# zhenxuan00/graphical-gan

Hardware: AMD Instinct MI355X
Metric: images/sec (G+D+GP step) cifar10 32x32 bs=64 (higher is better)
Workload: dtype f32; 1 GPU; gan_inference_cifar10.py MODE=wali-gp BATCH_SIZE=64 (per GPU) 32x32x3, CRITIC_ITERS=5; parallelism=dp1, global_batch=64, hip_graph=True, minibatch_feed=device-resident ring, read in place; one graph per iteration, finite_costs=True

## Files before the change

### graphical_gan_amd/_lib.py

```python
import ctypes as C
import os

_HERE = os.path.dirname(os.path.abspath(__file__))
LIB_PATH = os.path.join(_HERE, 'libggan.so')

ACT_NONE, ACT_LRELU, ACT_RELU, ACT_TANH, ACT_SIGMOID = 0, 1, 2, 3, 4
PACK_MAX = 64
HEAD_BCE_MAX_ROWS = 2048
BCE_HEADS = 2
PACK_ARRIVE_INTS = 33 * 1024
POSTERIOR_MAX_K = 8192
MODE_K = {'CONCRETE': 0, 'STRAIGHT_THROUGHT_CONCRETE': 1, 'STRAIGHT_THROUGHT': 2}
BCE_MAX = 16
TSNE_MAX_K = 128
TSNE_MAX_SPLITS = 64
ABI_VERSION = 800


class ConvGeom(C.Structure):
    _fields_ = [(n, C.c_int) for n in ('N', 'Ci', 'H', 'W', 'Co', 'Ho', 'Wo', 'k', 'stride', 'pad_t', 'pad_l',
                                       'plan_wgs', 'plan_wgs_filter', 'plan_flags')]


PLAN_PLAIN = 1


class ProfRec(C.Structure):
    _fields_ = [('name', C.c_char * 48), ('total_ms', C.c_double), ('launches', C.c_long),
                ('flops', C.c_double), ('bytes', C.c_double), ('grid', C.c_long)]


class GganError(RuntimeError):
    pass


_P = C.c_void_p
_F = C.c_float
_I = C.c_int
_Z = C.c_size_t
_G = C.POINTER(ConvGeom)

SIGNATURES = {
    'ggan_version': (_I, []),
    'ggan_last_error': (C.c_char_p, []),
    'ggan_conv2d_workspace': (_Z, [_G]),
    'ggan_conv2d_fwd': (_I, [_G, _P, _P, _P, _P, _I, _F, _P, _Z, _P]),
    'ggan_conv2d_bwd_data': (_I, [_G, _P, _P, _P, _P, _I, _F, _P, _Z, _P]),
    'ggan_conv2d_bwd_filter': (_I, [_G, _P, _P, _P, _P, _P, _Z, _P]),
    'ggan_conv2d_bwd_data_act': (_I, [_G, _P, _P, _I, _F, _P, _P, _P, _Z, _P]),
    'ggan_conv2d_bwd_filter_act': (_I, [_G, _P, _P, _P, _I, _F, _P, _P, _P, _Z, _P]),
    'ggan_conv2d_bwd_filter_parts': (_I, [_G, _P, _P, _P, _I, _F, _I, _P, _Z, C.POINTER(_I), C.POINTER(_Z), _P]),
    'ggan_conv2d_fwd_cast_ring': (_I, [_G, _P, _I, _P, _P, _I, _P, _F, _F, _P, _P, _P, _P, _I, _F, _P]),
    'ggan_conv2d_fwd_masked': (_I, [_G, _P, _P, _P, _P, _I, _F, _P, _Z, _P]),
    'ggan_linear_bn_rows_fwd': (_I, [_P, _P, _P, _P, _P, _P, _P, _P, _P, _I, _I, _I, _F, _I, _F, _P]),
    'ggan_linear_bn_rows_bwd': (_I, [_P, _P, _P, _P, _P, _P, _P, _P, _P, _P, _P, _I, _I, _I, _I, _F, _P]),
    'ggan_deconv2d_fwd': (_I, [_G, _P, _P, _P, _P, _I, _F, _P, _Z, _P]),
    'ggan_deconv2d_bwd_data': (_I, [_G, _P, _P, _P, _P, _Z, _P]),
    'ggan_deconv2d_bwd_filter': (_I, [_G, _P, _P, _P, _P, _P, _Z, _P]),
    'ggan_gemm_workspace': (_Z, [_I, _I, _I]),
    'ggan_gemm': (_I, [_I, _I, _I, _I, _I, _P, _P, _P, _P, _I, _F, _P, _Z, _P]),
    'ggan_conv3d_out_shape': (_I, [_P, _P]),
    'ggan_im2col3d': (_I, [_P, _P, _P, _P]),
    'ggan_col2im3d': (_I, [_P, _P, _P, _P]),
    'ggan_conv3d_igemm_ok': (_I, [_P, _I]),
    'ggan_conv3d_fwd': (_I, [_P, _P, _P, _P, _P, _I, _F, _P, _Z, _P]),
    'ggan_conv3d_wgrad': (_I, [_P, _P, _P, _P, _P, _Z, _P]),
    'ggan_conv3d_dgrad': (_I, [_P, _P, _P, _P, _P]),
    'ggan_mix_rbf_mmd2_fwd': (_I, [_P, _P, _I, _I, _I, _P, _P, _I, _P, _P, _P]),
    'ggan_mix_rbf_mmd2_bwd': (_I, [_P, _P, _I, _I, _I, _P, _P, _I, _P, _P, _P, _P]),
    'ggan_mix_rbf_mmd2_unbiased_fwd': (_I, [_P, _P, _I, _I, _I, _P, _P, _I, _P, _P, _P]),
    'ggan_mix_rbf_mmd2_unbiased_bwd': (_I, [_P, _P, _I, _I, _I, _P, _P, _I, _P, _P, _P, _P]),
    'ggan_mix_rbf_sums_workspace': (_Z, [_I, _I]),
    'ggan_mix_rbf_sums': (_I, [_P, _P, _I, _I, _I, _P, _P, _I, _P, _P, _Z, _P]),
    'ggan_knn_radii_workspace': (_Z, [_I, _I]),
    'ggan_knn_radii': (_I, [_P, _I, _I, _I, _P, _P, _Z, _P]),
    'ggan_ball_counts_workspace': (_Z, [_I, _I]),
    'ggan_ball_counts': (_I, [_P, _P, _I, _I, _I, _P, _P, _P, _P, _Z, _P]),
    'ggan_noise_fill': (_I, [_P, _P, _P, _P, _P, _P, _I, _P, _P]),
    'ggan_gmm_latent_fwd': (_I, [_P, _P, _P, _P, _P, _I, _I, _I, _F, _F, _P]),
    'ggan_gmm_latent_bwd': (_I, [_P, _P, _P, _P, _P, _P, _P, _I, _I, _I, _F, _P]),
    'ggan_gmm_latent_st_fwd': (_I, [_P, _P, _P, _P, _P, _P, _I, _I, _I, _F, _F, _I, _P]),
    'ggan_gmm_latent_st_bwd': (_I, [_P, _P, _P, _P, _P, _P, _P, _I, _I, _I, _F, _I, _P]),
    'ggan_gmm_posterior_assign': (_I, [_P, _P, _F, _I, _I, _I, _I, _P, _P, _P, _P]),
    'ggan_cluster_accuracy': (_I, [_P, _P, _P, _I, _I, _P, _P]),
    'ggan_video_sheet_u8': (_I, [_P, _P, _P, _P, _I, _I, _I, _I, _I, _I, _I, _I, _I, _F, _F, _F, _P]),
    'ggan_tsne_sqnorms': (_I, [_P, _I, _I, _P, _P]),
    'ggan_tsne_neighbours': (_I, [_P, _P, _I, _I, _I, _I, _I, _P, _P, _P, _P, _Z, _P]),
    'ggan_tsne_affinities': (_I, [_P, _I, _I, _F, _I, _F, _P, _P, _P]),
    'ggan_tsne_symmetrise': (_I, [_P, _P, _I, _I, _P, _P, _P, _P, _P]),
    'ggan_tsne_gradient': (_I, [_P, _P, _P, _P, _I, _I, _P, _P, _P, _P, _P, _P]),
    'ggan_tsne_kl': (_I, [_P, _P, _P, _P, _I, _I, _P, _P, _P, _P, _P]),
    'ggan_tsne_iterate': (_I, [_P, _P, _P, _P, _P, _P, _P, _I, _I, _P, _P, _I, _I, _I, _F, _F, _F, _F, _F, _P]),
    'ggan_gemm_split': (_I, [_I, _I, _I, _I, _I, _P, _P, _I, _P, _P, _P, _P, _I, _P, _I, _F, _P, _Z, _P]),
    'ggan_gemm_colsum': (_I, [_I, _I, _I, _I, _P, _P, _P, _P, _P, _Z, _P]),
    'ggan_dyn_scan_fwd': (_I, [_I, _I, _I, _I, _I, _P, _P, _P, _P, _P, _P, _P, _P, _P, _P, _F, _P, _P, _P, _P]),
    'ggan_dyn_scan_bwd': (_I, [_I, _I, _I, _I, _I, _P, _P, _P, _P, _P, _P, _P, _P, _P, _F, _P, _P, _P, _P, _P, _P, _P]),
    'ggan_critic_head_fwd': (_I, [_I, _I, _I, _I, _P, _P, _P, _P, _P, _P, _F, _P, _P, _P, _Z, _P]),
    'ggan_critic_head_bwd': (_I, [_I, _I, _I, _I, _P, _P, _P, _P, _P, _P, _F, _P, _P, _P, _P, _P, _P, _P, _P, _Z, _P]),
    'ggan_critic_head_fwd_bce': (_I, [_I, _I, _I, _I, _P, _P, _P, _P, _P, _P, _F, _P, _P, _I, _I, _P, _P, _P, _P, _P, _P, _Z, _P]),
    'ggan_critic_head_bwd_tail': (_I, [_I, _I, _I, _I, _P, _P, _P, _P, _P, _F, _P, _P, _P, _P, _P, _P, _P, _P, _P, _I, _I, _P, _P, _P, _P, _P, _P, _Z, _P]),
    'ggan_linear_bwd_data_act': (_I, [_I, _I, _I, _P, _P, _I, _F, _P, _P, _P, _Z, _P]),
    'ggan_linear_bwd_weight_act': (_I, [_I, _I, _I, _P, _P, _P, _I, _F, _P, _P, _P, _Z, _P]),
    'ggan_colsum': (_I, [_P, _P, _I, _I, _P]),
    'ggan_reparam_fwd': (_I, [_P, _P, _P, _P, _P, _Z, _P]),
    'ggan_reparam_bwd': (_I, [_P, _P, _P, _P, _P, _P, _Z, _P]),
    'ggan_agg_div_fwd': (_I, [_I, _P, _P, _P, _P, _P, _I, _I, _I, _I, _P, _P, _P, _P, _P, _P]),
    'ggan_agg_div_bwd': (_I, [_I, _P, _P, _P, _P, _I, _I, _I, _I, _P, _P, _P, _P, _P, _P, _P, _P, _P]),
    'ggan_colsum_tall': (_I, [_P, _P, _I, _I, _P, _Z, _P]),
    'ggan_chansum': (_I, [_P, _P, _I, _I, _I, _P, _Z, _P]),
    'ggan_bn_fwd_train': (_I, [_P, _P, _P, _P, _P, _P, _I, _I, _I, _F, _I, _F, _P]),
    'ggan_bn_bwd': (_I, [_P, _P, _P, _P, _P, _P, _P, _P, _I, _I, _I, _P]),
    'ggan_bn_bwd_act': (_I, [_P, _P, _P, _I, _F, _P, _P, _P, _P, _P, _P, _P, _I, _I, _I, _P]),
    'ggan_bn_bwd_bwd': (_I, [_P, _P, _P, _I, _F, _P, _P, _P, _P, _P, _P, _P, _I, _I, _I, _P]),
    'ggan_bn_split_fwd_train': (_I, [_P, _P, _P, _P, _P, _P, _I, _I, _I, _I, _F, _I, _F, _P, _Z, _P]),
    'ggan_bn_split_bwd_act': (_I, [_P, _P, _I, _F, _P, _P, _P, _P, _P, _P, _P, _P, _I, _I, _I, _I, _I, _P, _Z, _P]),
    'ggan_bn_sync_stats': (_I, [_P, _P, _I, _I, _I, _P]),
    'ggan_bn_sync_apply': (_I, [_P, _P, _I, _P, _P, _P, _P, _P, _I, _I, _I, _F, _I, _F, _P]),
    'ggan_bn_sync_bwd_stats': (_I, [_P, _P, _P, _I, _F, _P, _P, _P, _I, _I, _I, _P]),
    'ggan_bn_sync_bwd_apply': (_I, [_P, _P, _P, _I, _F, _P, _P, _P, _P, _I, _I, _P, _P, _P, _I, _I, _I, _P]),
    'ggan_act_fwd': (_I, [_P, _P, _Z, _I, _F, _P]),
    'ggan_act_bwd': (_I, [_P, _P, _P, _Z, _I, _F, _P]),
    'ggan_act_bwd_chansum': (_I, [_P, _P, _P, _P, _I, C.POINTER(_I), _I, _I, _I, _I, _F, _P]),
    'ggan_bias_add': (_I, [_P, _P, _P, _I, _I, _I, _P]),
    'ggan_cast_scale_i32': (_I, [_P, _P, _P, _Z, _F, _F, _P]),
    'ggan_cast_scale_ring_i32': (_I, [_P, _I, _P, _P, _I, _P, _P, _Z, _F, _F, _P]),
    'ggan_axpby': (_I, [_P, _P, _P, _Z, _F, _F, _F, _P]),
    'ggan_mix_mean': (_I, [_P, _P, _P, _P, _I, _I, _I, _P]),
    'ggan_row_lerp': (_I, [_P, _P, _P, _P, _I, _I, _P]),
    'ggan_bce_logits_fwd': (_I, [_P, _F, _F, _P, _I, _I, _P]),
    'ggan_bce_logits_bwd': (_I, [_P, _F, _F, _P, _P, _I, _P]),
    'ggan_bce_logits_multi_fwd': (_I, [C.POINTER(_P), C.POINTER(_F), C.POINTER(_F), C.POINTER(_I), _I, _P, _P]),
    'ggan_bce_logits_multi_bwd': (_I, [C.POINTER(_P), C.POINTER(_F), C.POINTER(_F), C.POINTER(_I), _I, _P, C.POINTER(_P), _P]),
    'ggan_bce_logits_multi_fwd_grad': (_I, [C.POINTER(_P), C.POINTER(_F), C.POINTER(_F), C.POINTER(_I), _I, _P, C.POINTER(_P), _P]),
    'ggan_bce_head_bwd': (_I, [C.POINTER(_P), C.POINTER(_F), C.POINTER(_F), C.POINTER(_I), _I, _P, C.POINTER(_P), _I, _I, _P, _P, _F, _P, _P,
                          _P, _P]),
    'ggan_bce_heads_bwd': (_I, [C.POINTER(_P), C.POINTER(_F), C.POINTER(_F), C.POINTER(_I), _I, _P, C.POINTER(_P), _I, C.POINTER(_I),
                           C.POINTER(_I), C.POINTER(_I), C.POINTER(_P), C.POINTER(_P), C.POINTER(_F), C.POINTER(_P), C.POINTER(_P),
                           C.POINTER(_P), _P]),
    'ggan_mean_fwd': (_I, [_P, _F, _P, _I, _I, _P]),
    'ggan_mean_bwd': (_I, [_P, _F, _P, _I, _P]),
    'ggan_mean_multi_fwd_grad': (_I, [C.POINTER(_P), C.POINTER(_F), C.POINTER(_I), _I, _P, C.POINTER(_P), _P]),
    'ggan_dist_fwd': (_I, [_P, _P, _P, _Z, _I, _F, _I, _P]),
    'ggan_dist_bwd': (_I, [_P, _P, _P, _P, _P, _Z, _I, _F, _P]),
    'ggan_gp_penalty_fwd': (_I, [_P, _P, _P, _I, _I, _F, _P]),
    'ggan_gp_penalty_bwd': (_I, [_P, _P, _P, _P, _I, _I, _F, _P]),
    'ggan_gp_penalty_fwd_grad': (_I, [_P, _P, _P, _P, _P, _I, _I, _F, _P]),
    'ggan_adam_step': (_I, [_P, _P, _P, _P, _Z, _P, _F, _F, _F, _F, _F, _P]),
    'ggan_adam_advance': (_I, [_P, _P]),
    'ggan_rmsprop_step': (_I, [_P, _P, _P, _Z, _F, _F, _F, _F, _F, _F, _P]),
    'ggan_adam_step_counted': (_I, [_P, _P, _P, _P, _Z, _P, _F, _F, _F, _F, _F, _P]),
    'ggan_pack': (_I, [C.POINTER(_P), C.POINTER(_Z), C.POINTER(_Z), _I, _P, _P]),
    'ggan_pack_parts': (_I, [C.POINTER(_P), C.POINTER(_Z), C.POINTER(_Z), C.POINTER(_I), C.POINTER(_Z), _I, _P, _P, _P]),
    'ggan_pack_parts2': (_I, [C.POINTER(_P), C.POINTER(_Z), C.POINTER(_Z), C.POINTER(_I), C.POINTER(_Z), C.POINTER(_P), C.POINTER(_I),
                              C.POINTER(_Z), _I, _P, _P, _P]),
    'ggan_pack_adam': (_I, [C.POINTER(_P), C.POINTER(_Z), C.POINTER(_Z), C.POINTER(_I), C.POINTER(_Z), C.POINTER(_P), C.POINTER(_I),
                            C.POINTER(_Z), _I, _P, _P, _P, _P, _P, _P, _F, _F, _F, _F, _F, _P]),
    'ggan_prof_enable': (_I, [_I]),
    'ggan_prof_reset': (_I, []),
    'ggan_prof_report': (_I, [C.POINTER(ProfRec), _I]),
}

_lib = None


def load():
    global _lib
    if _lib is not None:
        return _lib
    if not os.path.exists(LIB_PATH):
        raise GganError('libggan.so not found at %s -- run `python -c "import __graft_entry__ as g; g.build()"` '
                        '(there is no CPU fallback)' % LIB_PATH)
    lib = C.CDLL(LIB_PATH)
    for name, (res, args) in SIGNATURES.items():
        try:
            fn = getattr(lib, name)
        except AttributeError:
            raise GganError('libggan.so does not export %s' % name)
        fn.restype = res
        fn.argtypes = args
    if lib.ggan_version() != ABI_VERSION:
        raise GganError('libggan.so speaks ABI version %d, this binding %d: a stale build -- run `python -c "import __graft_entry__ as g; g.build()"`'
                        % (lib.ggan_version(), ABI_VERSION))
    _lib = lib
    return lib


def check(rc, what):
    if rc != 0:
        msg = load().ggan_last_error()
        raise GganError('%s failed (%d): %s' % (what, rc, msg.decode() if msg else ''))


def prof_report(cap=256):
    lib = load()
    recs = (ProfRec * cap)()
    n = lib.ggan_prof_report(recs, cap)
    out = []
    for i in range(n):
        r = recs[i]
        out.append(dict(name=r.name.decode(), total_ms=r.total_ms, launches=int(r.launches),
                        flops=r.flops, bytes=r.bytes, grid=int(r.grid)))
    return out
# ... 1 lines not shown
```

### graphical_gan_amd/csrc/conv.h

```cpp
#pragma once
#include "common.h"

namespace ggan {

int conv_fwd_naive(const ggan_conv_geom& g, const float* x, const float* w, const float* bias, float* y, int act,
                   float alpha, hipStream_t s);
struct GyMask {
    const float* ref;
    int act;
    float alpha;
};
int conv_dgrad_naive(const ggan_conv_geom& g, const float* gy, GyMask m, const float* w, const float* bias, float* gx,
                     int act, float alpha, hipStream_t s);
int conv_wgrad_naive(const ggan_conv_geom& g, const float* x, const float* gy, GyMask m, float* gw, hipStream_t s);

constexpr int kTargetWgs = 200;
struct OutMask {
    const float* ref;
    int act;
    float alpha;
    bool applied;
};
int conv_fwd_mfma(const ggan_conv_geom& g, const float* x, const float* w, const float* bias, float* y, int act,
                  float alpha, void* ws, size_t ws_bytes, hipStream_t s, OutMask* mask = nullptr);
int conv_dgrad_mfma(const ggan_conv_geom& g, const float* gy, GyMask m, const float* w, const float* bias, float* gx,
                    int act, float alpha, void* ws, size_t ws_bytes, hipStream_t s);
int conv_dgrad_dg16(const ggan_conv_geom& g, const float* gy, GyMask m, const float* w, const float* bias, float* gx, int act,
                    float alpha, int target_wgs, void* ws, size_t ws_bytes, hipStream_t s);
int conv_dgrad_thin(const ggan_conv_geom& g, const float* gy, GyMask m, const float* w, const float* bias, float* gx, int act,
                    float alpha, hipStream_t s);
struct WgradParts {
    float* buf;
    size_t cap_floats;
    int with_bias;
    int n;
    size_t stride;
};
int conv_wgrad_mfma(const ggan_conv_geom& g, const float* x, const float* gy, GyMask m, float* gw, float* gbias, void* ws,
                    size_t ws_bytes, hipStream_t s, WgradParts* parts = nullptr);
struct ThinCastSrc {
    const int32_t* ring;
    const int32_t* ctr_a;
    const int32_t* ctr_b;
    const float* noise;
    float* x_out;
    int nslots, offset;
    float div, mul;
};
int conv_fwd_thin(const ggan_conv_geom& g, const float* x, const float* w, const float* bias, float* y, int act, float alpha,
                  hipStream_t s, const ThinCastSrc* cast = nullptr, const OutMask* mask = nullptr);
int conv_wgrad_thin(const ggan_conv_geom& g, const float* x, const float* gy, GyMask m, float* gw, float* gbias, void* ws,
                    size_t ws_bytes, hipStream_t s, WgradParts* parts = nullptr);
size_t conv_workspace_bytes(const ggan_conv_geom& g);
int launch_splitk_reduce(const float* partial, int SK, size_t elems, float* out, const float* bias, int C, int HW, int act,
                         float alpha, hipStream_t s, size_t slab_stride = 0, float* tail_out = nullptr, size_t tail = 0);

struct FastDiv {
    uint32_t mul, d;
};
inline FastDiv make_fastdiv(uint32_t d) {
    FastDiv f;
    f.d = d;
    f.mul = (d <= 1) ? 0u : (uint32_t)((0x100000000ull / d) + 1ull);
    return f;
}
__device__ __forceinline__ uint32_t fdiv(uint32_t n, FastDiv f) { return f.d <= 1 ? n : __umulhi(n, f.mul); }

struct FastDiv24 {
    uint32_t mul, shift;
};
inline bool make_fastdiv24(uint32_t d, uint32_t nmax, FastDiv24* out) {
    if (d <= 1) { out->mul = 1; out->shift = 0; return true; }
    for (int s = 31; s >= 1; --s) {
        const uint64_t m = ((1ull << s) + d - 1) / d;
        if (m >= (1ull << 24) || m * nmax >= (1ull << 32)) continue;
        const uint64_t err = m * d - (1ull << s);
        if ((uint64_t)nmax * err >= (1ull << s)) return false;
        out->mul = (uint32_t)m; out->shift = (uint32_t)s;
        return true;
    }
    return false;
}
__device__ __forceinline__ uint32_t fdiv24(uint32_t n, FastDiv24 f) { return __umul24(n, f.mul) >> f.shift; }

}
```

### graphical_gan_amd/csrc/conv_api.hip

```cpp
#include "common.h"
#include "conv.h"
#include <stdlib.h>
using namespace ggan;

namespace {

int check_geom(const ggan_conv_geom* g) {
    if (!g) { set_error("null geometry"); return -1; }
    if (g->N <= 0 || g->Ci <= 0 || g->Co <= 0 || g->H <= 0 || g->W <= 0 || g->Ho <= 0 || g->Wo <= 0 || g->k <= 0 ||
        g->stride <= 0 || g->pad_t < 0 || g->pad_l < 0) {
        set_error("bad conv geometry N=%d Ci=%d H=%d W=%d Co=%d Ho=%d Wo=%d k=%d s=%d pad=(%d,%d)", g->N, g->Ci, g->H,
                  g->W, g->Co, g->Ho, g->Wo, g->k, g->stride, g->pad_t, g->pad_l);
        return -1;
    }
    if ((g->plan_flags & ~GGAN_PLAN_PLAIN) || g->plan_wgs < 0 || g->plan_wgs > 65536 || g->plan_wgs_filter < 0 || g->plan_wgs_filter > 65536) {
        set_error("conv geometry: launch plan fields out of range (plan_wgs=%d plan_wgs_filter=%d plan_flags=%d): struct built against "
                  "an older ggan.h? (GGAN_ABI_VERSION %d)", g->plan_wgs, g->plan_wgs_filter, g->plan_flags, GGAN_ABI_VERSION);
        return -1;
    }
    if ((g->Ho - 1) * g->stride - g->pad_t >= g->H || (g->Wo - 1) * g->stride - g->pad_l >= g->W) {
        set_error("conv geometry: output grid larger than the input allows");
        return -1;
    }
    return 0;
}

}

extern "C" {

size_t ggan_conv2d_workspace(const ggan_conv_geom* g) { return g ? conv_workspace_bytes(*g) : 0; }

int ggan_conv2d_fwd(const ggan_conv_geom* g, const float* x, const float* w, const float* bias, float* y, int act,
                    float alpha, void* ws, size_t ws_bytes, ggan_stream_t stream) {
    if (check_geom(g)) return -1;
    GGAN_CHECK_ARG(x && w && y, "null pointer");
    hipStream_t s = (hipStream_t)stream;
    if (!(g->plan_flags & GGAN_PLAN_PLAIN) && !getenv("GGAN_NAIVE_FWD")) {
        int r = conv_fwd_thin(*g, x, w, bias, y, act, alpha, s);
        if (r <= 0) return r;
        r = conv_fwd_mfma(*g, x, w, bias, y, act, alpha, ws, ws ? ws_bytes : 0, s);
        if (r <= 0) return r;
    }
    return conv_fwd_naive(*g, x, w, bias, y, act, alpha, s);
}

int ggan_conv2d_fwd_cast_ring(const ggan_conv_geom* g, const int32_t* ring, int nslots, const int32_t* ctr_a, const int32_t* ctr_b, int offset,
                              const float* noise, float div, float mul, float* x_out, const float* w, const float* bias, float* y, int act,
                              float alpha, ggan_stream_t stream) {
    if (check_geom(g)) return -1;
    GGAN_CHECK_ARG(ring && x_out && w && y && nslots > 0, "bad argument");
    if ((g->plan_flags & GGAN_PLAN_PLAIN) || getenv("GGAN_NAIVE_FWD")) return 1;
    ThinCastSrc c;
    c.ring = ring; c.ctr_a = ctr_a; c.ctr_b = ctr_b; c.noise = noise; c.x_out = x_out; c.nslots = nslots; c.offset = offset; c.div = div; c.mul = mul;
    return conv_fwd_thin(*g, nullptr, w, bias, y, act, alpha, (hipStream_t)stream, &c);
}

static int bwd_data(const ggan_conv_geom* g, const float* gy, GyMask m, const float* w, const float* bias, float* gx, int act,
                    float alpha, void* ws, size_t ws_bytes, ggan_stream_t stream) {
    if (check_geom(g)) return -1;
    if (!(gy && w && gx)) { set_error("ggan_conv2d_bwd_data: null pointer"); return -1; }
    hipStream_t s = (hipStream_t)stream;
    if (getenv("GGAN_TRACE_CONV"))
        fprintf(stderr, "[ggan] bwd_data N=%d Ci=%d H=%d W=%d Co=%d Ho=%d Wo=%d pad=(%d,%d) mask=%d act=%d\n", g->N, g->Ci, g->H, g->W, g->Co, g->Ho,
                g->Wo, g->pad_t, g->pad_l, m.act, act);
    if (!(g->plan_flags & GGAN_PLAN_PLAIN) && !getenv("GGAN_NAIVE_DGRAD")) {
        int r = conv_dgrad_thin(*g, gy, m, w, bias, gx, act, alpha, s);
        if (r <= 0) return r;
        r = conv_dgrad_dg16(*g, gy, m, w, bias, gx, act, alpha, g->plan_wgs, ws, ws ? ws_bytes : 0, s);
        if (r <= 0) return r;
        r = conv_dgrad_mfma(*g, gy, m, w, bias, gx, act, alpha, ws, ws ? ws_bytes : 0, s);
        if (r <= 0) return r;
    }
    return conv_dgrad_naive(*g, gy, m, w, bias, gx, act, alpha, s);
}

__global__ void pad_width_k(const float* __restrict__ in, const float* __restrict__ ref, float* __restrict__ out, size_t rows,
                            int W, int Wp, int shift, int act, float alpha) {
    const size_t total = rows * (size_t)Wp;
    for (size_t i = (size_t)blockIdx.x * blockDim.x + threadIdx.x; i < total; i += (size_t)gridDim.x * blockDim.x) {
        const size_t r = i / Wp;
        const int w = (int)(i - r * Wp) - shift;
        float v = 0.f;
        if (w >= 0 && w < W) {
            v = in[r * W + w];
            if (ref) v = act_grad(v, ref[r * W + w], act, alpha);
        }
        out[i] = v;
    }
}

static int wgrad_widened(const ggan_conv_geom& g, const float* x, const float* gy, GyMask m, float* gw, float* gbias, void* ws,
                         size_t ws_bytes, hipStream_t s) {
    if (g.k != 5 || g.stride != 2 || (g.pad_l != 1 && g.pad_l != 2)) return 1;
    const int shift = g.pad_l - 1;
    int Wop = (g.Wo + 3) & ~3;
    while (2 * Wop < g.W + shift) Wop += 4;
    const int Wp = 2 * Wop;
    if (Wop > 64) return 1;
    ws = ws_scratch(ws, ws_bytes);
    const size_t xr = (size_t)g.N * g.Ci * g.H, gr = (size_t)g.N * g.Co * g.Ho;
    const size_t xb = (xr * Wp * sizeof(float) + 255) & ~(size_t)255, gb = (gr * Wop * sizeof(float) + 255) & ~(size_t)255;
    if (!ws || ws_bytes < xb + gb + (1u << 20)) return 1;
    float* xp = (float*)ws;
    float* gp = (float*)((char*)ws + xb);
    auto blocks = [](size_t n) { size_t b = (n + 255) / 256; return (int)(b > 4096 ? 4096 : (b < 1 ? 1 : b)); };
    GGAN_LAUNCH("pad_width_k", 0, 8.0 * xr * Wp, pad_width_k, dim3(blocks(xr * Wp)), dim3(256), 0, s, x, (const float*)nullptr, xp, xr,
                g.W, Wp, shift, 0, 0.f);
    GGAN_LAUNCH("pad_width_k", 0, 8.0 * gr * Wop, pad_width_k, dim3(blocks(gr * Wop)), dim3(256), 0, s, gy,
                m.act != GGAN_ACT_NONE ? m.ref : (const float*)nullptr, gp, gr, g.Wo, Wop, 0, m.act, m.alpha);
    ggan_conv_geom gp2 = g;
    gp2.W = Wp; gp2.Wo = Wop; gp2.pad_l = 1;
    void* rest = (char*)ws + xb + gb;
    const size_t rest_bytes = ws_bytes - xb - gb;
    const GyMask none{nullptr, GGAN_ACT_NONE, 0.f};
    int r = conv_wgrad_mfma(gp2, xp, gp, none, gw, gbias, rest, rest_bytes, s);
    if (r == 1 && gbias) {
        r = conv_wgrad_mfma(gp2, xp, gp, none, gw, nullptr, rest, rest_bytes, s);
        if (r == 0) r = ggan_chansum(gp, gbias, g.N, g.Co, g.Ho * Wop, rest, rest_bytes, (ggan_stream_t)s);
    }
    return r;
}

static int bwd_filter(const ggan_conv_geom* g, const float* x, const float* gy, GyMask m, float* gw, float* gbias, void* ws,
                      size_t ws_bytes, ggan_stream_t stream) {
    if (check_geom(g)) return -1;
    if (!(x && gy && gw)) { set_error("ggan_conv2d_bwd_filter: null pointer"); return -1; }
    hipStream_t s = (hipStream_t)stream;
    if (!(g->plan_flags & GGAN_PLAN_PLAIN) && !getenv("GGAN_NAIVE_WGRAD")) {
        int r = conv_wgrad_thin(*g, x, gy, m, gw, gbias, ws, ws ? ws_bytes : 0, s);
        if (r <= 0) return r;
        r = conv_wgrad_mfma(*g, x, gy, m, gw, gbias, ws, ws ? ws_bytes : 0, s);
        if (r <= 0) return r;
        r = wgrad_widened(*g, x, gy, m, gw, gbias, ws, ws ? ws_bytes : 0, s);
        if (r <= 0) return r;
    }
    if (gbias) {
        if (m.act != GGAN_ACT_NONE) return 1;
        int r = ggan_chansum(gy, gbias, g->N, g->Co, g->Ho * g->Wo, ws, ws_bytes, stream);
        if (r) return r;
    }
    if (getenv("GGAN_TRACE_NAIVE"))
        fprintf(stderr, "[ggan] plain filter-gradient kernel for N=%d Ci=%d H=%d W=%d Co=%d Ho=%d Wo=%d k=%d s=%d pad=(%d,%d)\n", g->N, g->Ci,
                g->H, g->W, g->Co, g->Ho, g->Wo, g->k, g->stride, g->pad_t, g->pad_l);
    return conv_wgrad_naive(*g, x, gy, m, gw, s);
}

int ggan_conv2d_bwd_data(const ggan_conv_geom* g, const float* gy, const float* w, const float* bias, float* gx, int act,
                         float alpha, void* ws, size_t ws_bytes, ggan_stream_t stream) {
    return bwd_data(g, gy, GyMask{nullptr, GGAN_ACT_NONE, 0.f}, w, bias, gx, act, alpha, ws, ws_bytes, stream);
}

int ggan_conv2d_bwd_filter(const ggan_conv_geom* g, const float* x, const float* gy, float* gw, float* gbias, void* ws,
                           size_t ws_bytes, ggan_stream_t stream) {
    return bwd_filter(g, x, gy, GyMask{nullptr, GGAN_ACT_NONE, 0.f}, gw, gbias, ws, ws_bytes, stream);
}

int ggan_conv2d_bwd_data_act(const ggan_conv_geom* g, const float* gy, const float* y, int y_act, float y_alpha, const float* w,
                             float* gx, void* ws, size_t ws_bytes, ggan_stream_t stream) {
    GGAN_CHECK_ARG(y || y_act == GGAN_ACT_NONE, "null activation reference");
    return bwd_data(g, gy, GyMask{y, y_act, y_alpha}, w, nullptr, gx, GGAN_ACT_NONE, 0.f, ws, ws_bytes, stream);
}

int ggan_conv2d_bwd_filter_act(const ggan_conv_geom* g, const float* x, const float* gy, const float* y, int y_act, float y_alpha,
                               float* gw, float* gbias, void* ws, size_t ws_bytes, ggan_stream_t stream) {
    GGAN_CHECK_ARG(y || y_act == GGAN_ACT_NONE, "null activation reference");
    return bwd_filter(g, x, gy, GyMask{y, y_act, y_alpha}, gw, gbias, ws, ws_bytes, stream);
}

int ggan_conv2d_bwd_filter_parts(const ggan_conv_geom* g, const float* x, const float* gy, const float* y, int y_act,
                                 float y_alpha, int with_bias, float* part, size_t part_cap, int* n_parts, size_t* stride,
                                 ggan_stream_t stream) {
    if (check_geom(g)) return -1;
    GGAN_CHECK_ARG(x && gy && part && n_parts && stride, "null pointer");
    GGAN_CHECK_ARG(y || y_act == GGAN_ACT_NONE, "null activation reference");
    if ((g->plan_flags & GGAN_PLAN_PLAIN) || getenv("GGAN_NAIVE_WGRAD")) return 1;
    WgradParts po{part, part_cap, with_bias, 0, 0};
    int r = conv_wgrad_thin(*g, x, gy, GyMask{y, y_act, y_alpha}, nullptr, nullptr, nullptr, 0, (hipStream_t)stream, &po);
    if (r == 1) r = conv_wgrad_mfma(*g, x, gy, GyMask{y, y_act, y_alpha}, nullptr, nullptr, nullptr, 0, (hipStream_t)stream, &po);
    if (r == 0) { *n_parts = po.n; *stride = po.stride; }
    return r;
}

int ggan_conv2d_fwd_masked(const ggan_conv_geom* g, const float* x, const float* w, float* y, const float* yref, int ref_act,
                           float ref_alpha, void* ws, size_t ws_bytes, ggan_stream_t stream) {
    if (check_geom(g)) return -1;
    GGAN_CHECK_ARG(x && w && y && yref, "null pointer");
    if ((g->plan_flags & GGAN_PLAN_PLAIN) || getenv("GGAN_NAIVE_FWD")) return 1;
    if ((((uintptr_t)yref) & 15) != 0) return 1;
    OutMask M{yref, ref_act, ref_alpha, false};
    if (g->Ci <= 4 && (ref_act == GGAN_ACT_LRELU || ref_act == GGAN_ACT_RELU)) {
        const int r = conv_fwd_thin(*g, x, w, nullptr, y, GGAN_ACT_NONE, 0.f, (hipStream_t)stream, nullptr, &M);
        if (r <= 0) return r;
    }
    const int rc = conv_fwd_mfma(*g, x, w, nullptr, y, GGAN_ACT_NONE, 0.f, ws, ws ? ws_bytes : 0, (hipStream_t)stream, &M);
    if (rc == 0 && !M.applied) { set_error("conv2d_fwd_masked: launch without the mask"); return -3; }
    return rc;
}

int ggan_deconv2d_fwd(const ggan_conv_geom* g, const float* x_small, const float* w, const float* bias, float* y_big,
                      int act, float alpha, void* ws, size_t ws_bytes, ggan_stream_t stream) {
    return ggan_conv2d_bwd_data(g, x_small, w, bias, y_big, act, alpha, ws, ws_bytes, stream);
}

int ggan_deconv2d_bwd_data(const ggan_conv_geom* g, const float* gy_big, const float* w, float* gx_small, void* ws,
                           size_t ws_bytes, ggan_stream_t stream) {
    return ggan_conv2d_fwd(g, gy_big, w, nullptr, gx_small, GGAN_ACT_NONE, 0.f, ws, ws_bytes, stream);
}

int ggan_deconv2d_bwd_filter(const ggan_conv_geom* g, const float* gy_big, const float* x_small, float* gw, float* gbias,
                             void* ws, size_t ws_bytes, ggan_stream_t stream) {
    if (check_geom(g)) return -1;
    if (gbias) {
        GGAN_CHECK_ARG(gy_big, "null pointer");
        int r = ggan_chansum(gy_big, gbias, g->N, g->Ci, g->H * g->W, ws, ws_bytes, stream);
        if (r) return r;
    }
    return ggan_conv2d_bwd_filter(g, gy_big, x_small, gw, nullptr, ws, ws_bytes, stream);
}

}
```

### graphical_gan_amd/csrc/conv_corr.hip

```cpp
#include "common.h"
#include "conv.h"
#include <stdlib.h>
#include <map>
#include <mutex>
#include <vector>
using namespace ggan;

namespace {

constexpr int XE_MAX = 24;
constexpr unsigned OOB = 0x7FFFFFF0u;
typedef unsigned int u32x4 __attribute__((ext_vector_type(4)));

__host__ __device__ inline int fwd_region(int data_floats, int lanes_used, int floats_per_lane) {
    const int tail = (((lanes_used + 63) & ~63) - lanes_used) * floats_per_lane;
    return (data_floats + (tail > 4 ? tail : 4) + 3) & ~3;
}

struct CorrClass {
    int Hu, Wv;
    int roff, coff;
    int or0, oc0;
    int wbase;
    int pad_;
// ... 491 lines not shown
        stamp(3);
        constexpr int NSTEP = (NT0 * PW + 1) / 2, NITEM = XE + WE;
        constexpr int IPS = (NITEM + NSTEP - 3) / (NSTEP - 2);
        for (int ck0 = ck_begin; ck0 < ck_end; ck0 += CK, buf = buf == 2 ? 0 : buf + 1) {
            const int ck2 = ck0 + 2 * CK;
            const bool more2 = ck2 < ck_end;
            const int b2 = buf == 0 ? 2 : buf - 1;
            auto hook = [&](int g) {
#pragma unroll
                for (int it = g * IPS; it < (g + 1) * IPS; ++it) {
                    if (more2 && it < XE) dma_x1(it, ck2, b2);
                    if (more2 && it >= XE && it < NITEM) dma_w1(it - XE, ck2, b2);
                }
            };
            const float* xs = smem + buf * STAGE;
            const float* ws = xs + XS_SZ;
            mma_taps<CL::th(0), CL::tw(0), DI, PW, CK, RS, 0>(xs, ws, xfrag[0], wfrag, P.CS, P.SCp, acc[0], hook);
            if (more2) wait_vm_n(ndma);
            else asm volatile("s_waitcnt vmcnt(0)" ::: "memory");
            __syncthreads();
            if (it_ < 8) stamp(4 + it_);
            ++it_;
        }
    } else if (dma) {
        asm volatile("s_waitcnt vmcnt(0)" ::: "memory");
        __syncthreads();
        stamp(3);
        constexpr int NSTEP = (NT0 * PW + 1) / 2, NITEM = XE + WE;
        constexpr int IPS = (NITEM + NSTEP - 3) / (NSTEP - 2);
        for (int ck0 = ck_begin; ck0 < ck_end; ck0 += CK, buf ^= 1) {
            const int ckn = ck0 + CK;
            const bool more = ckn < ck_end;
            auto hook = [&](int g) {
#pragma unroll
                for (int it = g * IPS; it < (g + 1) * IPS; ++it) {
                    if (more && it < XE) dma_x1(it, ckn, buf ^ 1);
                    if (more && it >= XE && it < NITEM) dma_w1(it - XE, ckn, buf ^ 1);
                }
            };
            const float* xs = smem + buf * STAGE;
            const float* ws = xs + XS_SZ;
            mma_taps<CL::th(0), CL::tw(0), DI, PW, CK, RS, 0>(xs, ws, xfrag[0], wfrag, P.CS, P.SCp, acc[0], hook);
            asm volatile("s_waitcnt vmcnt(0)" ::: "memory");
            __syncthreads();
            if (it_ < 8) stamp(4 + it_);
            ++it_;
        }
    } else if (wdma) {
        constexpr int TS = GH * NCB * WBLK;
        constexpr int WD_STEPS = (NT0 * (PW == 2 ? 2 : 1) + 1) / 2 + (NT1 * (PW == 2 ? 2 : 1) + 1) / 2 +
                                 (NT2 * (PW == 2 ? 2 : 1) + 1) / 2 + (NT3 * (PW == 2 ? 2 : 1) + 1) / 2;
        constexpr int WD_DPS = (WQ + WD_STEPS - 2) / (WD_STEPS - 1);
        constexpr int WD_S0 = (WQ + WD_DPS - 1) / WD_DPS < WD_STEPS - 1 ? (WQ + WD_DPS - 1) / WD_DPS : WD_STEPS - 1;
        constexpr int WD_SPS = (XN + WD_STEPS - WD_S0 - 1) / (WD_STEPS - WD_S0);
        prefetch(ck_begin, false);
        stage_w(ck_begin, 0);
        commit(0, false);
        if (ck_begin + CK < ck_end) prefetch(ck_begin + CK, false);
        asm volatile("s_waitcnt vmcnt(0)" ::: "memory");
        __syncthreads();
        stamp(3);
        for (int ck0 = ck_begin; ck0 < ck_end; ck0 += CK, buf ^= 1) {
            const int ckn = ck0 + CK;
            commit(buf ^ 1, false);
            const float* xs = smem + buf * STAGE;
            const float* ws = xs + XS_SZ;
            const int ck2 = ck0 + 2 * CK;
            const bool more2 = ck2 < ck_end;
            auto hook = [&](int g) {
#pragma unroll
                for (int q = g * WD_DPS; q < (g + 1) * WD_DPS; ++q)
                    if (q < WQ && (q < WQ - 1 || wso[WQ - 1] >= 0)) stage_w1(q, ckn, buf ^ 1);
#pragma unroll
                for (int j = (g - WD_S0) * WD_SPS; j < (g - WD_S0 + 1) * WD_SPS; ++j)
                    if (j >= 0 && j < XN) {
                        if constexpr (XR4) {
                            xreg4[j] = __builtin_amdgcn_raw_buffer_load_b128(rin, more2 ? xvo[j] : OOB, ck2 * HWin * 4, 0);
                            if (masked) xref4[j] = __builtin_amdgcn_raw_buffer_load_b128(rref, more2 ? xvo[j] : OOB, ck2 * HWin * 4, 0);
                        } else {
                            xreg[j] = __builtin_amdgcn_raw_buffer_load_b32(rin, more2 ? xvo[j] : OOB, ck2 * HWin * 4, 0);
                            if (masked) xref[j] = __builtin_amdgcn_raw_buffer_load_b32(rref, more2 ? xvo[j] : OOB, ck2 * HWin * 4, 0);
                        }
                    }
            };
            if constexpr (WD) {
                constexpr int S1 = (CL::th(0) * CL::tw(0) * (PW == 2 ? 2 : 1) + 1) / 2;
                constexpr int S2 = NC > 1 ? (CL::th(1) * CL::tw(1) * (PW == 2 ? 2 : 1) + 1) / 2 : 0;
                constexpr int S3 = NC > 2 ? (CL::th(2) * CL::tw(2) * (PW == 2 ? 2 : 1) + 1) / 2 : 0;
                mma_taps_wd<CL::th(0), CL::tw(0), DI, PW, TS, 0>(xs, ws, xfrag[0], wfrag_wd, P.CS, P.SCp, acc[0], hook);
                if constexpr (NC > 1) mma_taps_wd<CL::th(1), CL::tw(1), DI, PW, TS, S1>(xs, ws + NT0 * TS, xfrag[1], wfrag_wd, P.CS, P.SCp, acc[1], hook);
                if constexpr (NC > 2) mma_taps_wd<CL::th(2), CL::tw(2), DI, PW, TS, S1 + S2>(xs, ws + (NT0 + NT1) * TS, xfrag[2], wfrag_wd, P.CS, P.SCp, acc[2], hook);
                if constexpr (NC > 3) mma_taps_wd<CL::th(3), CL::tw(3), DI, PW, TS, S1 + S2 + S3>(xs, ws + (NT0 + NT1 + NT2) * TS, xfrag[3], wfrag_wd, P.CS, P.SCp, acc[3], hook);
            }
            static_assert(2 * XN < 64, "vmcnt field");
            if (masked) asm volatile("s_waitcnt vmcnt(%0)" ::"n"(2 * XN) : "memory");
            else asm volatile("s_waitcnt vmcnt(%0)" ::"n"(XN) : "memory");
            __syncthreads();
            if (it_ < 8) stamp(4 + it_);
            ++it_;
        }
    } else {
    prefetch(ck_begin);
    commit(0);
    stamp(2);
    if (ck_begin + CK < ck_end) prefetch(ck_begin + CK);
    __syncthreads();
    stamp(3);
    const bool stage_first = NTHR == 256 || wave < (NTHR / 128);
    auto stage_next = [&](int ck0) {
        if (ck0 + CK < ck_end && !(P.dbg & 1)) {
            if (!(P.dbg & 16)) commit(buf ^ 1);
            if (ck0 + 2 * CK < ck_end && !(P.dbg & 32)) prefetch(ck0 + 2 * CK);
        }
    };
    for (int ck0 = ck_begin; ck0 < ck_end; ck0 += CK, buf ^= 1) {
        if (stage_first) stage_next(ck0);
        if (fine && it_ < 4) stamp(4 + 2 * it_);
        if (!(P.dbg & 2)) {
            const float* xs = smem + ((P.dbg & 1) ? 0 : buf * STAGE);
            const float* ws = xs + XS_SZ;
            mma_taps<CL::th(0), CL::tw(0), DI, PW, CK, RS>(xs, ws, xfrag[0], wfrag, P.CS, P.SCp, acc[0]);
            if constexpr (NC > 1) mma_taps<CL::th(1), CL::tw(1), DI, PW, CK, RS>(xs, ws + NT0 * CK * RS, xfrag[1], wfrag, P.CS, P.SCp, acc[1]);
            if constexpr (NC > 2) mma_taps<CL::th(2), CL::tw(2), DI, PW, CK, RS>(xs, ws + (NT0 + NT1) * CK * RS, xfrag[2], wfrag, P.CS, P.SCp, acc[2]);
            if constexpr (NC > 3) mma_taps<CL::th(3), CL::tw(3), DI, PW, CK, RS>(xs, ws + (NT0 + NT1 + NT2) * CK * RS, xfrag[3], wfrag, P.CS, P.SCp, acc[3]);
        }
        if (fine && it_ < 4 && stage_first) stamp(5 + 2 * it_);
        if (!stage_first) stage_next(ck0);
        if (fine && it_ < 4 && !stage_first) stamp(5 + 2 * it_);
        __syncthreads();
        if (!fine && it_ < 8) stamp(4 + it_);
        ++it_;
    }
    }
    stamp(12);

    constexpr int TMW = 32 * WM;
    float* red = smem;
#pragma unroll
    for (int c = 0; c < NC; ++c)
#pragma unroll
        for (int r = 0; r < 16; ++r) {
            const int cnl = wn * 32 + (r & 3) + 8 * (r >> 2) + 4 * half;
            red[((ks * NC + c) * TNW + cnl) * TMW + wm * 32 + l31] = acc[c][r];
        }
    __syncthreads();
    stamp(13);
    if (P.dbg & 8) return;
    const bool direct = P.SK == 1;
    float* outp = direct ? P.out : P.out + (size_t)split * P.out_elems;
    const int chw = P.Hout * P.Wout;
    constexpr int GROUPS = NC == 4 ? 2 : NC;
    constexpr int UNITS = GROUPS * TNW * (TMW / 4);
    const bool quad_rows = (P.TC & 3) == 0;
    for (int u = tid; u < UNITS; u += NTHR) {
        const int p4 = u % (TMW / 4);
        const int cnl = (u / (TMW / 4)) % TNW;
        static_assert(((TMW / 4) * TNW) % 64 == 0, "store groups are whole waves");
        const int gsel = __builtin_amdgcn_readfirstlane(u / ((TMW / 4) * TNW));
        const int cn = cn0 + cnl;
        if (cn >= P.CNtot) continue;
        const int ca = NC == 4 ? 2 * gsel : gsel, cb = NC == 4 ? 2 * gsel + 1 : gsel;
        float va[4] = {0.f, 0.f, 0.f, 0.f}, vb[4] = {0.f, 0.f, 0.f, 0.f};
        float4 ta[KS], tb[KS];
#pragma unroll
        for (int k = 0; k < KS; ++k) {
            ta[k] = *reinterpret_cast<const float4*>(red + ((k * NC + ca) * TNW + cnl) * TMW + 4 * p4);
            if (NC == 4) tb[k] = *reinterpret_cast<const float4*>(red + ((k * NC + cb) * TNW + cnl) * TMW + 4 * p4);
        }
#pragma unroll
        for (int k = 0; k < KS; ++k) {
            va[0] += ta[k].x; va[1] += ta[k].y; va[2] += ta[k].z; va[3] += ta[k].w;
            if (NC == 4) { vb[0] += tb[k].x; vb[1] += tb[k].y; vb[2] += tb[k].z; vb[3] += tb[k].w; }
        }
        if (direct) {
            const float bv = P.bias ? P.bias[cn] : 0.f;
#pragma unroll
            for (int j = 0; j < 4; ++j) {
                va[j] = act_apply(va[j] + bv, P.act, P.alpha);
                if (NC == 4) vb[j] = act_apply(vb[j] + bv, P.act, P.alpha);
            }
        }
        const CorrClass& A = P.cls[CL::cls(ca)];
        const CorrClass& B = P.cls[CL::cls(cb)];
        const int p = 4 * p4;
        const int img = fdiv24(p, P.d_TRTC);
        const int rem = p - img * (P.TR * P.TC);
        const int ur = fdiv24(rem, P.d_TC);
        const int vc = rem - ur * P.TC;
        const bool img_ok = img < P.TI && (n0 + img) < P.N;
        const size_t cbase = ((size_t)(n0 + img) * P.CNtot + cn) * chw;
        bool done = false;
        if (quad_rows && img_ok && (P.Wout & 3) == 0) {
            if (NC != 4 && P.ocs == 1 && (A.Wv & 3) == 0 && (u0 + ur) < A.Hu && (v0 + vc + 3) < A.Wv) {
                const int off = (A.or0 + P.ors * (u0 + ur)) * P.Wout + A.oc0 + v0 + vc;
                if ((off & 3) == 0) {
                    if (KIND == 0 && P.out_ref) {
                        const float4 r4 = *reinterpret_cast<const float4*>(P.out_ref + cbase + off);
                        va[0] = act_grad(va[0], r4.x, P.out_act, P.out_alpha); va[1] = act_grad(va[1], r4.y, P.out_act, P.out_alpha);
                        va[2] = act_grad(va[2], r4.z, P.out_act, P.out_alpha); va[3] = act_grad(va[3], r4.w, P.out_act, P.out_alpha);
                    }
                    *reinterpret_cast<float4*>(outp + cbase + off) = make_float4(va[0], va[1], va[2], va[3]);
                    done = true;
                }
            }
            if (NC == 4 && A.Wv == B.Wv && A.Hu == B.Hu && (A.Wv & 3) == 0 && (u0 + ur) < A.Hu && (v0 + vc + 3) < A.Wv) {
                const bool a_even = A.oc0 < B.oc0;
                const int off = (A.or0 + P.ors * (u0 + ur)) * P.Wout + (a_even ? A.oc0 : B.oc0) + P.ocs * (v0 + vc);
                if ((off & 3) == 0 && P.ocs == 2) {
                    const float* e = a_even ? va : vb;
                    const float* o = a_even ? vb : va;
                    *reinterpret_cast<float4*>(outp + cbase + off) = make_float4(e[0], o[0], e[1], o[1]);
                    *reinterpret_cast<float4*>(outp + cbase + off + 4) = make_float4(e[2], o[2], e[3], o[3]);
                    done = true;
                }
            }
        }
        if (!done) {
#pragma unroll
            for (int j = 0; j < 4; ++j) {
                const int pj = p + j;
                const int im = fdiv24(pj, P.d_TRTC);
                const int rm = pj - im * (P.TR * P.TC);
                const int urj = fdiv24(rm, P.d_TC);
                const int vcj = rm - urj * P.TC;
                if (!(im < P.TI && (n0 + im) < P.N)) continue;
                const size_t cb2 = ((size_t)(n0 + im) * P.CNtot + cn) * chw;
                if ((u0 + urj) < A.Hu && (v0 + vcj) < A.Wv) {
                    const size_t oi = cb2 + (A.or0 + P.ors * (u0 + urj)) * P.Wout + A.oc0 + P.ocs * (v0 + vcj);
                    outp[oi] = (KIND == 0 && P.out_ref) ? act_grad(va[j], P.out_ref[oi], P.out_act, P.out_alpha) : va[j];
                }
                if (NC == 4 && (u0 + urj) < B.Hu && (v0 + vcj) < B.Wv)
                    outp[cb2 + (B.or0 + P.ors * (u0 + urj)) * P.Wout + B.oc0 + P.ocs * (v0 + vcj)] = vb[j];
            }
        }
    }
    stamp(14);
}

template <int MODE, int WM, int WN, int KS, int PW, bool X4 = false>
__global__ __launch_bounds__(64 * WM * WN * KS) void corr_kernel(const CorrParams P) {
    extern __shared__ __attribute__((aligned(16))) float smem[];
    warm_kernarg(P);
    const int grp = blockIdx.z / P.SK, split = blockIdx.z - grp * P.SK;
    int bx = blockIdx.x, by = blockIdx.y;
    if (P.xcd_p > 0) {
        const int lin = blockIdx.y * gridDim.x + blockIdx.x, xcd = lin & 7, slot = lin >> 3;
        const int pg = xcd % P.xcd_p, cg = xcd / P.xcd_p;
        const int npx = gridDim.x / P.xcd_p, nch = gridDim.y / (8 / P.xcd_p);
        bx = pg * npx + slot % npx;
        by = cg * nch + slot / npx;
    }
    if constexpr (MODE == 0) {
        corr_body<0, 2, 1, WM, WN, KS, PW, X4>(P, split, smem, bx, by);
    } else if constexpr (MODE == 2) {
        corr_body<3, 1, -1, WM, WN, KS, PW, X4>(P, split, smem, bx, by);
    } else if (grp == 0) {
        corr_body<1, 1, -1, WM, WN, KS, PW, X4>(P, split, smem, bx, by);
    } else {
        corr_body<2, 1, -1, WM, WN, KS, PW, X4>(P, split, smem, bx, by);
    }
}

__global__ void splitk_reduce_k(const float* __restrict__ partial, int SK, size_t elems, size_t stride, float* __restrict__ out,
                                const float* __restrict__ bias, int C, int HW, int act, float alpha, float* __restrict__ out2,
                                size_t n2) {
    for (size_t i = (size_t)blockIdx.x * blockDim.x + threadIdx.x; i < elems + n2; i += (size_t)gridDim.x * blockDim.x) {
        float s = 0.f;
#pragma unroll 8
        for (int k = 0; k < SK; ++k) s += partial[(size_t)k * stride + i];
        if (i < elems) {
            if (bias) s += bias[(i / (size_t)HW) % (size_t)C];
            out[i] = act_apply(s, act, alpha);
        } else {
            out2[i - elems] = s;
        }
    }
}

__global__ void splitk_reduce_small_k(const float* __restrict__ partial, int SK, size_t elems, size_t stride, float* __restrict__ out,
                                      const float* __restrict__ bias, int C, int HW, int act, float alpha,
                                      float* __restrict__ out2, size_t n2) {
    __shared__ float sm[4][64];
    const int o = threadIdx.x & 63, kg = threadIdx.x >> 6;
    const size_t i = (size_t)blockIdx.x * 64 + o;
    float s = 0.f;
    if (i < elems + n2)
#pragma unroll 4
        for (int k = kg; k < SK; k += 4) s += partial[(size_t)k * stride + i];
    sm[kg][o] = s;
    __syncthreads();
    if (kg == 0 && i < elems + n2) {
        float v = (sm[0][o] + sm[1][o]) + (sm[2][o] + sm[3][o]);
        if (i < elems) {
            if (bias) v += bias[(i / (size_t)HW) % (size_t)C];
            out[i] = act_apply(v, act, alpha);
        } else {
            out2[i - elems] = v;
        }
    }
}

struct WaveCfg { int WM, WN, KS, PW; };
constexpr int kNumCfgs = 9;
constexpr WaveCfg kCfgsFwd[kNumCfgs] = {{2, 2, 1, 2}, {2, 1, 2, 2}, {1, 1, 4, 1}, {1, 1, 4, 2}, {2, 1, 4, 1}, {1, 1, 8, 1}, {2, 2, 2, 1}, {2, 1, 4, 2}, {4, 1, 2, 2}};
constexpr WaveCfg kCfgsDgrad[kNumCfgs] = {{2, 2, 1, 4}, {2, 1, 2, 4}, {1, 1, 4, 2}, {1, 1, 4, 4}, {2, 1, 4, 2}, {1, 1, 8, 1}, {2, 2, 2, 2}, {1, 1, 8, 2}, {1, 1, 8, 2}};
constexpr const WaveCfg* cfgs_of(int mode) { return mode == 1 ? kCfgsDgrad : kCfgsFwd; }

#define CORR_EACH(X)                                                                                                        \
    X(0, 2, 1, 2, 2, false) X(0, 2, 1, 4, 1, false) X(0, 1, 1, 8, 1, false) X(0, 2, 2, 2, 1, false) X(0, 4, 1, 2, 2, false) \
    X(0, 2, 1, 4, 1, true) X(0, 1, 1, 8, 1, true) X(0, 2, 2, 2, 1, true) X(0, 4, 1, 2, 2, true)                             \
    X(1, 2, 1, 2, 4, false) X(1, 2, 1, 4, 2, false) X(1, 1, 1, 8, 1, false) X(1, 2, 2, 2, 2, false)                         \
    X(1, 2, 1, 4, 2, true) X(1, 1, 1, 8, 1, true)                                                                           \
    X(2, 2, 1, 2, 2, false) X(2, 1, 1, 8, 1, false) X(2, 2, 2, 2, 1, false) X(2, 2, 1, 4, 2, false)                         \
    X(2, 1, 1, 8, 1, true) X(2, 2, 2, 2, 1, true) X(2, 2, 1, 4, 2, true)
struct CorrInst { int mode; WaveCfg wc; bool x4; const char* name; void (*kernel)(const CorrParams); };
#define CORR_INST(MODE, WM, WN, KS, PW, X4) \
    {MODE, {WM, WN, KS, PW}, X4, "corr_kernel<" #MODE ", " #WM ", " #WN ", " #KS ", " #PW ", " #X4 ">", corr_kernel<MODE, WM, WN, KS, PW, X4>},
constexpr CorrInst kCorrInsts[] = {CORR_EACH(CORR_INST)};
#undef CORR_INST
#undef CORR_EACH

constexpr const CorrInst* find_inst(int mode, const WaveCfg& wc, bool x4) {
    for (const CorrInst& k : kCorrInsts)
        if (k.mode == mode && k.wc.WM == wc.WM && k.wc.WN == wc.WN && k.wc.KS == wc.KS && k.wc.PW == wc.PW && k.x4 == x4) return &k;
    return nullptr;
}
constexpr bool has_inst(int mode, int cfg, bool x4) { return find_inst(mode, cfgs_of(mode)[cfg], x4) != nullptr; }

constexpr int kOrderFwd[4] = {8, 6, 4, 5}, kOrderAll[4] = {8, 6, 7, 5};
constexpr const int* order_of(int mode) { return mode == 2 ? kOrderAll : kOrderFwd; }
constexpr int order_begin(int mode) { return mode == 0 ? 0 : 1; }
constexpr bool planner_covered(int mode) {
    for (int oi = order_begin(mode); oi < 4; ++oi)
        if (!has_inst(mode, order_of(mode)[oi], false)) return false;
    return has_inst(mode, 1, false) && has_inst(mode, 6, false);
}
static_assert(planner_covered(0) && planner_covered(1) && planner_covered(2),
              "plan_and_launch offers a wave layout that has no entry in CORR_EACH");

bool pick_tile(CorrParams& P, int Hu, int Wv, int TM, int CK, int su, int ext_r, int ext_c) {
    const int budget = (su == 2 ? XE_MAX : XE_MAX / 2) * 256;
    P.TC = Wv < TM ? Wv : TM;
    P.TR = TM / P.TC; if (P.TR < 1) P.TR = 1; if (P.TR > Hu) P.TR = Hu;
    P.TI = TM / (P.TR * P.TC); if (P.TI < 1) P.TI = 1; if (P.TI > P.N) P.TI = P.N;
    for (;;) {
        P.SR = su * (P.TR - 1) + ext_r;
        P.SCp = su * (P.TC - 1) + ext_c;
        P.CS = P.TI * P.SR * P.SCp;
        if (CK * P.CS <= budget) return true;
        if (P.TI > 1) P.TI = (P.TI + 1) / 2;
        else if (P.TR > 1) P.TR = (P.TR + 1) / 2;
        else return false;
    }
}

bool finish_tile(CorrParams& P, int Hu, int Wv) {
    const uint32_t nmax = XE_MAX * 256;
    const int xq = P.xq == 4 ? 4 : 1;
    if (!make_fastdiv24(P.CS / xq, nmax, &P.d_CS) || !make_fastdiv24(P.SR * P.SCp / xq, nmax, &P.d_SRSC) || !make_fastdiv24(P.SCp / xq, nmax, &P.d_SCp) ||
        !make_fastdiv24(P.TR * P.TC, nmax, &P.d_TRTC) || !make_fastdiv24(P.TC, nmax, &P.d_TC))
        return false;
    P.img_groups = cdiv(P.N, P.TI);
    P.tiles_r = cdiv(Hu, P.TR); P.tiles_c = cdiv(Wv, P.TC);
    return true;
}

template <int MODE>
int launch_cfg(int cfg, const CorrParams& P, dim3 grid, size_t shmem, hipStream_t s, const char* name, double fl) {
    const double ab = (double)P.in_bytes + (double)P.w_bytes + 4.0 * (double)P.out_elems;
    static std::atomic<unsigned long long> once{0};
    if (first_on_device(once))
        for (const CorrInst& k : kCorrInsts)
            (void)hipFuncSetAttribute(reinterpret_cast<const void*>(k.kernel), hipFuncAttributeMaxDynamicSharedMemorySize, 160 * 1024);
    if (shmem > 160 * 1024) { set_error("%s: LDS request %zu too large", name, shmem); return -3; }
    const CorrInst* k = cfg >= 0 && cfg < kNumCfgs ? find_inst(MODE, cfgs_of(MODE)[cfg], P.xq == 4) : nullptr;
    if (!k) { set_error("%s: no %d-byte-unit variant of wave layout %d", name, P.xq == 4 ? 16 : 4, cfg); return -3; }
    GGAN_LAUNCH(k->name, fl, ab, k->kernel, grid, dim3(64 * k->wc.WM * k->wc.WN * k->wc.KS), shmem, s, P);
    return 0;
}

std::mutex g_xtab_mu;
std::map<std::vector<int>, unsigned*> g_xtabs;

const unsigned* fwd_slab_table(const CorrParams& P, int CK, int nthr, int su, hipStream_t s) {
    int dev = 0;
    (void)hipGetDevice(&dev);
    const int xq = P.xq == 4 ? 4 : 1;
    const int XE = XE_MAX * 256 / nthr;
    const std::vector<int> key = {dev, P.CKtot, P.Hin, P.Win, P.TI, P.TR, P.TC, P.SR, P.SCp, P.CS, xq, P.row0, P.col0, CK, nthr, P.tiles_r, P.tiles_c, su};
    std::lock_guard<std::mutex> lk(g_xtab_mu);
    auto it = g_xtabs.find(key);
    if (it != g_xtabs.end()) return it->second;
    hipStreamCaptureStatus st = hipStreamCaptureStatusNone;
    if (hipStreamIsCapturing(s, &st) != hipSuccess || st != hipStreamCaptureStatusNone) { (void)hipGetLastError(); return nullptr; }
    const int CSu = P.CS / xq, SCpu = P.SCp / xq, srsc = P.SR * SCpu, xe_cnt = CK * CSu;
    const int npos = P.tiles_r * P.tiles_c;
    std::vector<unsigned> tab((size_t)npos * XE * nthr, OOB);
    for (int tr = 0; tr < P.tiles_r; ++tr)
        for (int tc = 0; tc < P.tiles_c; ++tc) {
            const int in_row0 = su * tr * P.TR + P.row0, in_col0 = su * tc * P.TC + P.col0;
            for (int j = 0; j < XE; ++j)
                for (int tid = 0; tid < nthr; ++tid) {
                    const int e = tid + j * nthr;
                    if (e >= xe_cnt) continue;
                    const int ckl = e / CSu, r1 = e - ckl * CSu;
                    const int img = r1 / srsc, r2 = r1 - img * srsc;
                    const int r = r2 / SCpu, cc = (r2 - r * SCpu) * xq;
                    const int ih = in_row0 + r, iw = in_col0 + cc;
                    if (img >= P.TI || ih < 0 || ih >= P.Hin || iw < 0 || iw >= P.Win) continue;
                    tab[((size_t)(tr * P.tiles_c + tc) * XE + j) * nthr + tid] = (unsigned)((((size_t)img * P.CKtot + ckl) * P.Hin + ih) * P.Win + iw) * 4u;
                }
        }
    unsigned* d = nullptr;
    if (hipMalloc((void**)&d, tab.size() * sizeof(unsigned)) != hipSuccess) { (void)hipGetLastError(); return nullptr; }
    if (hipMemcpy(d, tab.data(), tab.size() * sizeof(unsigned), hipMemcpyHostToDevice) != hipSuccess) { (void)hipGetLastError(); (void)hipFree(d); return nullptr; }
    g_xtabs[key] = d;
    return d;
}

template <int MODE>
int plan_and_launch(CorrParams& P, int Hu, int Wv, int su, int ext_r, int ext_c, int ntaps, int groups, float* dst,
                    const float* bias, int act, float alpha, void* ws, size_t ws_bytes, hipStream_t s, const char* name,
                    double fl, const char* sk_env, OutMask* mask = nullptr) {
    const int target = P.plan_wgs > 0 ? P.plan_wgs : kTargetWgs;
    const WaveCfg* kCfgs = cfgs_of(MODE);
    const int* order = order_of(MODE);
    int cfg = 5;
    for (int oi = order_begin(MODE); oi < 4; ++oi) {
        const int c = order[oi];
        const WaveCfg& wc = kCfgs[c];
        const int CK = 2 * wc.KS * wc.PW, TM = 32 * wc.WM, TNW = 32 * wc.WN;
        if (P.CNtot <= 32 && TNW > 32) continue;
        CorrParams T = P;
        if (!pick_tile(T, Hu, Wv, TM, CK, su, ext_r, ext_c)) continue;
        if (oi < 3 && T.TI * T.TR * T.TC * 2 <= TM && Hu * Wv * P.N >= TM) continue;
        const int wgs = cdiv(P.N, T.TI) * cdiv(Hu, T.TR) * cdiv(Wv, T.TC) * cdiv(P.CNtot, TNW) * groups;
        if (oi == 0 && wgs >= 2 * target) continue;
        if (wgs >= target || oi == 3) { cfg = c; break; }
    }
    if (P.CKtot < 8) cfg = P.CNtot <= 32 ? 1 : 6;
    const WaveCfg& wc = kCfgs[cfg];
    const int CK = 2 * wc.KS * wc.PW, TM = 32 * wc.WM, TNW = 32 * wc.WN;
    if (!pick_tile(P, Hu, Wv, TM, CK, su, ext_r, ext_c)) return 1;
    P.dbg = env_int("GGAN_DBG", 0);
    P.dma = (MODE == 0 || (CK % 16 == 0 && wc.PW <= 2)) && (P.dbg & 3) == 0;
    const int RS = TNW + (MODE != 0 ? 2 : 0);
    P.xq = 1;
    if (MODE == 0 && has_inst(MODE, cfg, true) && P.dma && (P.Win & 3) == 0 && (((uintptr_t)P.in) & 15) == 0 && ((su * P.TC) & 3) == 0) {
        const int shift = ((P.col0 % 4) + 4) % 4;
        const int scp4 = (P.SCp + shift + 3) & ~3;
        const size_t cs4 = (size_t)P.TI * P.SR * scp4;
        const int wregion = fwd_region(ntaps * CK * RS, ntaps * CK * (TNW / 4), 4);
        const size_t stage4 = 2 * ((size_t)fwd_region((int)(CK * cs4), (int)(CK * cs4 / 4), 4) + (size_t)wregion);
        const size_t stage1 = 2 * ((size_t)fwd_region(CK * P.CS, CK * P.CS, 1) + (size_t)wregion);
        const bool crosses = stage1 * sizeof(float) <= 80 * 1024 && stage4 * sizeof(float) > 80 * 1024;
        if (stage4 * sizeof(float) <= 160 * 1024 && CK * cs4 / 4 <= (size_t)XE_MAX * 256 && !crosses) {
            P.xq = 4;
            P.col0 -= shift;
            for (int c = 0; c < 4; ++c) P.cls[c].coff += shift;
            P.SCp = scp4;
            P.CS = (int)cs4;
        }
    }
    if (MODE != 0 && has_inst(MODE, cfg, true) && (P.Win & 3) == 0 && (((uintptr_t)P.in) & 15) == 0 &&
        (((uintptr_t)P.in_ref) & 15) == 0 && ((su * P.TC) & 3) == 0) {
        const int shift = ((P.col0 % 4) + 4) % 4;
        const int scp4 = (P.SCp + shift + 3) & ~3;
        const size_t cs4 = (size_t)P.TI * P.SR * scp4;
        const int nthr = 64 * wc.WM * wc.WN * wc.KS;
        const int xn = ((XE_MAX / 2) * 256 / nthr + 3) / 4 + 1;
        const size_t stage4 = 2 * ((size_t)((CK * cs4 + 1 + 3) & ~(size_t)3) + (size_t)((ntaps * CK * RS + 4 * RS + 3) & ~3));
        if (stage4 * sizeof(float) <= 160 * 1024 && CK * cs4 / 4 <= (size_t)xn * nthr) {
            P.xq = 4;
            P.col0 -= shift;
            for (int c = 0; c < 4; ++c) P.cls[c].coff += shift;
            P.SCp = scp4;
            P.CS = (int)cs4;
        }
    }
    if (!finish_tile(P, Hu, Wv)) return 1;
    if ((size_t)P.N * P.CKtot * P.Hin >= (1u << 24)) return 1;
    const int gx = P.img_groups * P.tiles_r * P.tiles_c, gy = cdiv(P.CNtot, TNW);
    int sk = env_int(sk_env, 0);
    if (sk <= 0) {
        sk = 1;
        const int base = gx * gy * groups;
        if (base < target / 2) {
            sk = target / base;
            const int max_sk = P.CKtot / (2 * CK);
            if (sk > max_sk) sk = max_sk;
            if (sk > 16) sk = 16;
        }
    }
    if (sk < 1) sk = 1;
    P.cps = cdiv(cdiv(P.CKtot, sk), CK) * CK;
    P.SK = cdiv(P.CKtot, P.cps);
    if (P.SK > 1 && (size_t)P.SK * P.out_elems * sizeof(float) > ws_bytes) {
        P.SK = 1;
        P.cps = cdiv(P.CKtot, CK) * CK;
    }
    P.out = P.SK > 1 ? (float*)ws : dst;
    P.bias = bias; P.act = act; P.alpha = alpha;
    if (mask) {
        if (MODE != 0 || P.SK != 1) return 1;
        P.out_ref = mask->ref; P.out_act = mask->act; P.out_alpha = mask->alpha;
        mask->applied = true;
    }
    if ((P.dbg & 4) && ws && ws_bytes > (64u << 20)) P.stamps = (unsigned long long*)((char*)ws + ws_bytes - (32u << 20));
    size_t stage = MODE == 0 ? 2 * ((size_t)fwd_region(CK * P.CS, CK * P.CS / P.xq, P.xq) + (size_t)fwd_region(ntaps * CK * RS, ntaps * CK * (TNW / 4), 4))
                             : 2 * ((size_t)((CK * P.CS + 1 + 3) & ~3) + (size_t)((ntaps * CK * RS + 4 * RS + 3) & ~3));
    size_t red = (size_t)wc.KS * (MODE == 2 ? 4 : (MODE == 1 ? 2 : 1)) * TNW * TM;
    P.nstg = 2;
    if (MODE == 0 && P.dma) P.xtab = fwd_slab_table(P, CK, 64 * wc.WM * wc.WN * wc.KS, su, s);
    const size_t shmem = (stage > red ? stage : red) * sizeof(float);
    {
        P.xcd_p = 0;
        if ((gx * gy) % 8 == 0) {
            double best = (gx % 8 == 0) ? (double)P.in_bytes + 8.0 * P.w_bytes : 8.0 * ((double)P.in_bytes + P.w_bytes);
            for (int p = 1; p <= 8; p *= 2) {
                if (gx % p || gy % (8 / p)) continue;
                const double cost = 8.0 * P.in_bytes / p + (double)P.w_bytes * p;
                if (cost < 0.9 * best) { best = cost; P.xcd_p = p; }
            }
        }
    }
    if (getenv("GGAN_TRACE_CONV"))
        fprintf(stderr, "[ggan] plan %s mode=%d cfg=%d tile=(%d,%d,%d) xq=%d SK=%d xcd_p=%d grid=(%d,%d,%d) %s\n", name, MODE, cfg, P.TI, P.TR,
                P.TC, P.xq, P.SK, P.xcd_p, gx, gy, groups * P.SK, P.xtab ? "table" : "no-table");
    int rc = launch_cfg<MODE>(cfg, P, dim3(gx, gy, groups * P.SK), shmem, s, name, fl);
    if (rc) return rc;
    if (P.SK > 1)
        return launch_splitk_reduce((const float*)ws, P.SK, P.out_elems, dst, bias, P.CNtot, P.Hout * P.Wout, act, alpha, s);
    return 0;
}

}

namespace ggan {

int launch_splitk_reduce(const float* partial, int SK, size_t elems, float* out, const float* bias, int C, int HW, int act,
                         float alpha, hipStream_t s, size_t slab_stride, float* tail_out, size_t tail) {
    if (slab_stride == 0) slab_stride = elems;
    if (!tail_out) tail = 0;
    if (SK >= 8 && elems + tail <= 65536) {
        GGAN_LAUNCH("splitk_reduce_small_k", 0, 4.0 * (elems + tail) * (SK + 1), splitk_reduce_small_k,
                    dim3((int)((elems + tail + 63) / 64)), dim3(256), 0, s, partial, SK, elems, slab_stride, out, bias, C, HW, act,
                    alpha, tail_out, tail);
        return 0;
    }
    size_t b = (elems + tail + 255) / 256;
    if (b > 2048) b = 2048;
    GGAN_LAUNCH("splitk_reduce_k", 0, 4.0 * (elems + tail) * (SK + 1), splitk_reduce_k, dim3((int)b), dim3(256), 0, s, partial,
                SK, elems, slab_stride, out, bias, C, HW, act, alpha, tail_out, tail);
    return 0;
}

size_t conv_workspace_bytes(const ggan_conv_geom& g) {
    size_t big = (size_t)g.N * g.Ci * g.H * g.W, small_ = (size_t)g.N * g.Co * g.Ho * g.Wo;
    size_t wsz = (size_t)g.k * g.k * g.Ci * g.Co;
    size_t m = big > small_ ? big : small_;
    size_t a = 16 * m * sizeof(float), b = 64 * wsz * sizeof(float);
    return a > b ? a : b;
}

static bool hot_geometry(const ggan_conv_geom& g) { return g.k == 5 && g.stride == 2; }
static bool fits32(size_t bytes) { return bytes < 0x7FFFFFF0ull; }

int conv_fwd_mfma(const ggan_conv_geom& g, const float* x, const float* w, const float* bias, float* y, int act,
                  float alpha, void* ws, size_t ws_bytes, hipStream_t s, OutMask* mask) {
    if (!hot_geometry(g) || (g.Co & 3)) return 1;
    ws = ws_scratch(ws, ws_bytes);
    const size_t in_bytes = (size_t)g.N * g.Ci * g.H * g.W * 4, w_bytes = (size_t)25 * g.Ci * g.Co * 4;
    if (!fits32(in_bytes) || !fits32(w_bytes) || !fits32((size_t)g.N * g.Co * g.Ho * g.Wo * 4)) return 1;
    if (((uintptr_t)w & 15) != 0) return 1;
    CorrParams P;
    memset(&P, 0, sizeof(P));
    P.in = x; P.w = w;
    P.plan_wgs = g.plan_wgs;
    P.in_bytes = (unsigned)in_bytes; P.w_bytes = (unsigned)w_bytes;
    P.N = g.N; P.CKtot = g.Ci; P.Hin = g.H; P.Win = g.W;
    P.CNtot = g.Co; P.Hout = g.Ho; P.Wout = g.Wo;
    P.ors = 1; P.ocs = 1;
    P.w_si = g.k * g.Ci * g.Co; P.w_sj = g.Ci * g.Co; P.w_sk = g.Co; P.w_sn = 1;
    P.row0 = -g.pad_t; P.col0 = -g.pad_l;
    CorrClass& c = P.cls[0];
    c.Hu = g.Ho; c.Wv = g.Wo; c.roff = 0; c.coff = 0; c.or0 = 0; c.oc0 = 0; c.wbase = 0;
    P.out_elems = (size_t)g.N * g.Co * g.Ho * g.Wo;
    const double fl = 2.0 * P.out_elems * g.Ci * 25.0;
    return plan_and_launch<0>(P, g.Ho, g.Wo, 2, 5, 5, 25, 1, y, bias, act, alpha, ws, ws_bytes, s, "conv_fwd_mfma", fl,
                              "GGAN_FWD_SK", mask);
}

int conv_dgrad_mfma(const ggan_conv_geom& g, const float* gy, GyMask m, const float* w, const float* bias, float* gx,
                    int act, float alpha, void* ws, size_t ws_bytes, hipStream_t s) {
    if (!hot_geometry(g)) return 1;
    ws = ws_scratch(ws, ws_bytes);
    if ((g.Co & 3) || ((uintptr_t)w & 15)) return 1;
    const size_t in_bytes = (size_t)g.N * g.Co * g.Ho * g.Wo * 4, w_bytes = (size_t)25 * g.Ci * g.Co * 4;
    if (!fits32(in_bytes) || !fits32(w_bytes) || !fits32((size_t)g.N * g.Ci * g.H * g.W * 4)) return 1;
    const int S = 2;
    CorrParams P;
    memset(&P, 0, sizeof(P));
    P.in = gy; P.w = w;
    P.plan_wgs = g.plan_wgs;
    if (m.act != GGAN_ACT_NONE && m.act != GGAN_ACT_LRELU && m.act != GGAN_ACT_RELU) return 1;
    if (m.act != GGAN_ACT_NONE) { P.in_ref = m.ref; P.in_act = m.act; P.in_alpha = m.alpha; }
    P.in_bytes = (unsigned)in_bytes; P.w_bytes = (unsigned)w_bytes;
    P.N = g.N; P.CKtot = g.Co; P.Hin = g.Ho; P.Win = g.Wo;
    P.CNtot = g.Ci; P.Hout = g.H; P.Wout = g.W;
    P.ors = S; P.ocs = S;
    P.w_si = S * g.k * g.Ci * g.Co; P.w_sj = S * g.Ci * g.Co; P.w_sk = 1; P.w_sn = g.Co;
    int offs[2][2], bases[2][2], cnt[2][2], th[2][2], lo[2], hi[2];
    for (int d = 0; d < 2; ++d) {
        const int pad = d == 0 ? g.pad_t : g.pad_l, L = d == 0 ? g.H : g.W;
        lo[d] = 1 << 30; hi[d] = -(1 << 30);
        for (int p = 0; p < S; ++p) {
            const int off = ((p - pad) % S + S) % S;
            offs[d][p] = off;
            bases[d][p] = (off + pad - p) / S;
            cnt[d][p] = off < L ? (L - off + S - 1) / S : 0;
            th[d][p] = (g.k - p + S - 1) / S;
            if (bases[d][p] - (th[d][p] - 1) < lo[d]) lo[d] = bases[d][p] - (th[d][p] - 1);
            if (bases[d][p] > hi[d]) hi[d] = bases[d][p];
        }
    }
    const int Hu = cnt[0][0] > cnt[0][1] ? cnt[0][0] : cnt[0][1];
    const int Wv = cnt[1][0] > cnt[1][1] ? cnt[1][0] : cnt[1][1];
    P.row0 = lo[0]; P.col0 = lo[1];
    for (int ph = 0; ph < S; ++ph)
        for (int pw = 0; pw < S; ++pw) {
            CorrClass& c = P.cls[ph * 2 + pw];
            c.Hu = cnt[0][ph]; c.Wv = cnt[1][pw];
            c.roff = bases[0][ph] - lo[0]; c.coff = bases[1][pw] - lo[1];
            c.or0 = offs[0][ph]; c.oc0 = offs[1][pw];
            c.wbase = (ph * g.k + pw) * g.Ci * g.Co;
        }
    P.out_elems = (size_t)g.N * g.Ci * g.H * g.W;
    const double fl = 2.0 * g.N * g.Co * g.Ho * g.Wo * (double)g.Ci * 25.0;
    const long wgs_all = (long)cdiv(g.N * Hu * Wv, 32) * cdiv(g.Ci, 32);
    if (wgs_all >= (g.plan_wgs > 0 ? g.plan_wgs : kTargetWgs))
        return plan_and_launch<2>(P, Hu, Wv, 1, hi[0] - lo[0] + 1, hi[1] - lo[1] + 1, 25, 1, gx, bias, act, alpha, ws, ws_bytes,
                                  s, "conv_dgrad_mfma", fl, "GGAN_DGRAD_SK");
    return plan_and_launch<1>(P, Hu, Wv, 1, hi[0] - lo[0] + 1, hi[1] - lo[1] + 1, 13, 2, gx, bias, act, alpha, ws, ws_bytes,
                              s, "conv_dgrad_mfma", fl, "GGAN_DGRAD_SK");
}

}
```

### graphical_gan_amd/csrc/conv_dg16.hip

```cpp
#include "common.h"
#include "conv.h"
#include <stdlib.h>
#include <map>
#include <mutex>
#include <tuple>
#include <vector>
using namespace ggan;

namespace {

constexpr int NTHR = 512, NWAVE = 8;
constexpr unsigned OOB = 0x7FFFFFF0u;
constexpr int XN_MAX = 3;
constexpr int WBLK = 258;
constexpr int PS = 68;
typedef unsigned int u32x4 __attribute__((ext_vector_type(4)));

struct Dg16Params {
    const float* in;
    const float* w;
    const float* bias;
    float* out;
    const float* in_ref;
    const unsigned* xtab;
    int N, CK, Hin, Win, CN;
    int lTC, lTR;
    int CS;
    int xinstr;
    int tiles_r, tiles_c;
    int nchunks;
    int ahead;
    int nstage;
    unsigned in_bytes, w_bytes;
    int xcd_p;
    int act;
    float alpha;
    float in_slope;
    int dbg;
    unsigned long long* stamps;
    int tapoff[28];
};

__host__ __device__ constexpr int tap_cls(int t) { return t < 9 ? 0 : t < 15 ? 1 : t < 21 ? 2 : 3; }
__host__ __device__ constexpr int tap_i(int t) { return t < 9 ? t / 3 : t < 15 ? (t - 9) / 2 : t < 21 ? (t - 15) / 3 : (t - 21) / 2; }
__host__ __device__ constexpr int tap_j(int t) { return t < 9 ? t % 3 : t < 15 ? (t - 9) % 2 : t < 21 ? (t - 15) % 3 : (t - 21) % 2; }
__host__ __device__ constexpr int tap_slab_off(int t, int scp) {
    const int c = tap_cls(t), ph = c >> 1, pw = c & 1;
    return (1 + (1 - ph) - tap_i(t)) * scp + 4 + (1 - pw) - tap_j(t);
}

__device__ __forceinline__ void wait_vm(int n) {
    switch (n) {
        case 0: asm volatile("s_waitcnt vmcnt(0)" ::: "memory"); break;
        case 1: asm volatile("s_waitcnt vmcnt(1)" ::: "memory"); break;
        case 2: asm volatile("s_waitcnt vmcnt(2)" ::: "memory"); break;
        case 3: asm volatile("s_waitcnt vmcnt(3)" ::: "memory"); break;
        case 4: asm volatile("s_waitcnt vmcnt(4)" ::: "memory"); break;
        case 5: asm volatile("s_waitcnt vmcnt(5)" ::: "memory"); break;
        case 6: asm volatile("s_waitcnt vmcnt(6)" ::: "memory"); break;
        case 7: asm volatile("s_waitcnt vmcnt(7)" ::: "memory"); break;
        case 8: asm volatile("s_waitcnt vmcnt(8)" ::: "memory"); break;
        case 9: asm volatile("s_waitcnt vmcnt(9)" ::: "memory"); break;
        case 10: asm volatile("s_waitcnt vmcnt(10)" ::: "memory"); break;
        default: asm volatile("s_waitcnt vmcnt(0)" ::: "memory"); break;
    }
}

template <int SCP, int KQ, bool MASKED>
__device__ __forceinline__ void dg16_body(const Dg16Params& P, float* smem) {
    constexpr int NCHT = 4 / KQ;
    constexpr int CHT = 16 * NCHT;
    constexpr int CKC = 4 * KQ;
    constexpr int TPB = 8 / KQ;
    constexpr int NOCT = 2 * NCHT;
    constexpr int NTG = (25 + TPB - 1) / TPB;
    constexpr int NBLK = NTG * NOCT;
    constexpr int WQ = (NBLK + NWAVE - 1) / NWAVE;
    constexpr int WREG = (NBLK * WBLK + 3) & ~3;
    const int tid = threadIdx.x, lane = tid & 63;
    const int wave = __builtin_amdgcn_readfirstlane(tid >> 6);
    const int kqw = wave % KQ, chh = (wave / KQ) % NCHT, pxh = wave / (KQ * NCHT);
    const int wg_lin = blockIdx.y * gridDim.x + blockIdx.x;
    const bool stamping = (P.dbg & 4) && P.stamps && tid == 0;
    auto stamp = [&](int i) { if (stamping) P.stamps[(size_t)wg_lin * 16 + i] = __builtin_readcyclecounter(); };
    stamp(0);

    const int lTC = P.lTC, lTR = P.lTR, TC = 1 << lTC, TR = 1 << lTR, TI = 64 >> (lTC + lTR);
    const int tpi = P.tiles_r * P.tiles_c;
    int bx = blockIdx.x, by = blockIdx.y;
    if (P.xcd_p > 0) {
        const int xcd = wg_lin & 7, slot = wg_lin >> 3;
        const int npx = gridDim.x / P.xcd_p, nch = gridDim.y / (8 / P.xcd_p);
        bx = (xcd % P.xcd_p) * npx + slot % npx;
        by = (xcd / P.xcd_p) * nch + slot / npx;
    }
    const int ig = bx / tpi, tpos = bx - ig * tpi;
    const int tr = tpos / P.tiles_c, tc = tpos - tr * P.tiles_c;
    const int n0 = ig * TI, u0 = tr * TR, v0 = tc * TC;
    const int cn0 = by * CHT;
    const int HWin = P.Hin * P.Win;
    const int XREG = P.xinstr * 256;
    const int STAGE = WREG + XREG;

    const auto rin = __builtin_amdgcn_make_buffer_rsrc((void*)P.in, (short)0, (int)P.in_bytes, 0x00020000);
    const auto rw = __builtin_amdgcn_make_buffer_rsrc((void*)P.w, (short)0, (int)P.w_bytes, 0x00020000);
    const auto rref = __builtin_amdgcn_make_buffer_rsrc((void*)(MASKED ? P.in_ref : P.in), (short)0, (int)P.in_bytes, 0x00020000);

    unsigned xvo[XN_MAX];
    int nx = 0;
    {
        const unsigned* tab = P.xtab + (size_t)tpos * (XN_MAX * NTHR) + tid;
#pragma unroll
        for (int j = 0; j < XN_MAX; ++j) {
            xvo[j] = OOB;
            if (wave + j * NWAVE < P.xinstr) { xvo[j] = tab[j * NTHR]; nx = j + 1; }
        }
    }
    const int l_t = lane / (KQ * 8), l_kq = (lane >> 3) % KQ, l_c8 = lane & 7;
    unsigned wvo[WQ];
    int wlds[WQ];
    int nw = 0;
#pragma unroll
    for (int q = 0; q < WQ; ++q) {
        const int b = wave + q * NWAVE;
        wvo[q] = OOB; wlds[q] = 0;
        if (b < NBLK) {
            const int tg = b / NOCT, oct = b - tg * NOCT;
            int toff = P.tapoff[tg * TPB];
#pragma unroll
            for (int i = 1; i < TPB; ++i) { const int ti = P.tapoff[tg * TPB + i]; toff = l_t == i ? ti : toff; }
            wvo[q] = toff >= 0 ? (unsigned)toff + (unsigned)(((oct * 8 + l_c8) * P.CK + l_kq * 4) * 4) : OOB;
            wlds[q] = (tg * NOCT + oct) * WBLK;
            nw = q + 1;
        }
    }
    const int w_s0 = cn0 * P.CK * 4;
    auto dma_w = [&](int q, int chunk, int stage) {
        float* dst = smem + stage * STAGE + wlds[q];
        __builtin_amdgcn_raw_ptr_buffer_load_lds(rw, (__attribute__((address_space(3))) void*)dst, 16, wvo[q], w_s0 + chunk * CKC * 4, 0, 0);
    };
    const int nch = P.nchunks;
    const int AH = P.ahead, NST = P.nstage;
#pragma unroll
    for (int q = 0; q < WQ; ++q)
        if (q < nw) dma_w(q, 0, 0);
    if (nch > 1 && AH == 2) {
#pragma unroll
        for (int q = 0; q < WQ; ++q)
            if (q < nw) dma_w(q, 1, 1);
    }
    stamp(1);

    const unsigned img_base = (unsigned)n0 * (unsigned)P.CK * (unsigned)HWin * 4u;
#pragma unroll
    for (int j = 0; j < XN_MAX; ++j) {
        const unsigned t = xvo[j];
        xvo[j] = t >= OOB ? OOB : t + img_base;
    }
    auto dma_x = [&](int j, int chunk, int stage) {
        float* dst = smem + stage * STAGE + WREG + (wave + j * NWAVE) * 256;
        __builtin_amdgcn_raw_ptr_buffer_load_lds(rin, (__attribute__((address_space(3))) void*)dst, 16, xvo[j], chunk * CKC * HWin * 4, 0, 0);
    };
    u32x4 xr[MASKED ? XN_MAX : 1], xf[MASKED ? XN_MAX : 1];
    auto load_x = [&](int j, int chunk) {
        xr[j] = __builtin_amdgcn_raw_buffer_load_b128(rin, xvo[j], chunk * CKC * HWin * 4, 0);
        xf[j] = __builtin_amdgcn_raw_buffer_load_b128(rref, xvo[j], chunk * CKC * HWin * 4, 0);
    };
    auto commit_x = [&](int stage) {
#pragma unroll
        for (int j = 0; j < XN_MAX; ++j)
            if (j < nx) {
                f32x4 v;
#pragma unroll
                for (int c = 0; c < 4; ++c) {
                    const float a = __uint_as_float(xr[j][c]);
                    v[c] = __uint_as_float(xf[j][c]) > 0.f ? a : a * P.in_slope;
                }
                *reinterpret_cast<f32x4*>(smem + stage * STAGE + WREG + (wave + j * NWAVE) * 256 + lane * 4) = v;
            }
    };

    const int l15 = lane & 15, kk = lane >> 4;
    const int afrag = (chh * 2 + (l15 >> 3)) * WBLK + (kqw * 8 + (l15 & 7)) * 4 + kk;
    int bfrag[2];
#pragma unroll
    for (int f = 0; f < 2; ++f) {
        const int p = pxh * 32 + f * 16 + l15;
        const int b = p & (TC - 1), a = (p >> lTC) & (TR - 1), img = p >> (lTC + lTR);
        bfrag[f] = WREG + (kqw * 4 + kk) * P.CS + (img * (TR + 2) + a) * SCP + b;
    }

    f32x4 acc[4][2];
#pragma unroll
    for (int c = 0; c < 4; ++c)
#pragma unroll
        for (int f = 0; f < 2; ++f) acc[c][f] = (f32x4){0.f, 0.f, 0.f, 0.f};

    if constexpr (MASKED) {
#pragma unroll
        for (int j = 0; j < XN_MAX; ++j)
            if (j < nx) load_x(j, 0);
        asm volatile("s_waitcnt vmcnt(0)" ::: "memory");
        commit_x(0);
        if (nch > 1) {
#pragma unroll
            for (int j = 0; j < XN_MAX; ++j)
                if (j < nx) load_x(j, 1);
            asm volatile("s_waitcnt vmcnt(0)" ::: "memory");
            commit_x(1);
        }
    } else {
#pragma unroll
        for (int j = 0; j < XN_MAX; ++j)
            if (j < nx) dma_x(j, 0, 0);
        if (nch > 1 && AH == 2) {
#pragma unroll
            for (int j = 0; j < XN_MAX; ++j)
                if (j < nx) dma_x(j, 1, 1);
            wait_vm(nx);
        } else {
            asm volatile("s_waitcnt vmcnt(0)" ::: "memory");
        }
    }
    __syncthreads();
    stamp(3);

    const int nxi = nx;
    int stage = 0;
    for (int c = 0; c < nch; ++c) {
        const int s1 = stage + 1 == NST ? 0 : stage + 1;
        const int s2 = AH == 2 ? (stage >= 1 ? stage - 1 : 2) : s1;
        const bool more = c + AH < nch;
        const bool more_x = MASKED ? c + 2 < nch : more;
        if constexpr (MASKED) {
            if (c >= 1 && c + 1 < nch) {
                if (AH == 2) wait_vm(nw);
                commit_x(s1);
            }
        }
        const float* sb = smem + stage * STAGE;
        float a[25], b0[25], b1[25];
        auto load = [&](int t) {
            a[t] = sb[afrag + (t / TPB) * NOCT * WBLK + (t % TPB) * KQ * 32];
            b0[t] = sb[bfrag[0] + tap_slab_off(t, SCP)];
            b1[t] = sb[bfrag[1] + tap_slab_off(t, SCP)];
        };
        auto item = [&](int it) {
            if (it < XN_MAX) {
                if (more_x && it < nxi) {
                    if constexpr (MASKED) load_x(it, c + 2); else dma_x(it, c + AH, s2);
                }
            } else if (it - XN_MAX < WQ) {
                if (more && it - XN_MAX < nw) dma_w(it - XN_MAX, c + AH, s2);
            }
        };
        load(0);
        load(1);
#pragma unroll
        for (int t = 0; t < 25; ++t) {
            if (t + 2 < 25) load(t + 2);
            acc[tap_cls(t)][0] = __builtin_amdgcn_mfma_f32_16x16x4f32(a[t], b0[t], acc[tap_cls(t)][0], 0, 0, 0);
            acc[tap_cls(t)][1] = __builtin_amdgcn_mfma_f32_16x16x4f32(a[t], b1[t], acc[tap_cls(t)][1], 0, 0, 0);
            if (t >= 1 && (t - 1) % 3 == 0) item((t - 1) / 3);
            __builtin_amdgcn_sched_group_barrier(0x100, 3, 0);
            __builtin_amdgcn_sched_group_barrier(0x008, 2, 0);
            __builtin_amdgcn_sched_group_barrier(0x030, 2, 0);
        }
        if (more && AH == 2) wait_vm(MASKED ? 2 * nxi + nw : nxi + nw);
        else asm volatile("s_waitcnt vmcnt(0)" ::: "memory");
        __syncthreads();
        if (c < 8) stamp(4 + c);
        stage = s1;
    }
    stamp(12);

    float* red = smem;
#pragma unroll
    for (int c = 0; c < 4; ++c)
#pragma unroll
        for (int f = 0; f < 2; ++f)
#pragma unroll
            for (int r = 0; r < 4; ++r)
                red[((kqw * 4 + c) * CHT + chh * 16 + kk * 4 + r) * PS + pxh * 32 + f * 16 + l15] = acc[c][f][r];
    __syncthreads();
    stamp(13);
    const int Hout = 2 * P.Hin, Wout = 2 * P.Win;
    const int lQ = lTC - 1;
    for (int u = tid; u < 64 * CHT; u += NTHR) {
        const int cq = u & ((1 << lQ) - 1);
        const int row2 = (u >> lQ) & (2 * TR - 1);
        const int ch = (u >> (lQ + lTR + 1)) & (CHT - 1);
        const int img = u >> (lQ + lTR + 1 + (NCHT == 1 ? 4 : 5));
        const int ph = 1 - (row2 & 1), arow = row2 >> 1;
        const int px = (img << (lTC + lTR)) + (arow << lTC) + 2 * cq;
        float2 e = make_float2(0.f, 0.f), o = make_float2(0.f, 0.f);
        float2 te[KQ], to[KQ];
#pragma unroll
        for (int k = 0; k < KQ; ++k) {
            te[k] = *reinterpret_cast<const float2*>(red + ((k * 4 + ph * 2 + 1) * CHT + ch) * PS + px);
            to[k] = *reinterpret_cast<const float2*>(red + ((k * 4 + ph * 2 + 0) * CHT + ch) * PS + px);
        }
#pragma unroll
        for (int k = 0; k < KQ; ++k) { e.x += te[k].x; e.y += te[k].y; o.x += to[k].x; o.y += to[k].y; }
        const float bv = P.bias ? P.bias[cn0 + ch] : 0.f;
        float4 v = make_float4(e.x + bv, o.x + bv, e.y + bv, o.y + bv);
        v.x = act_apply(v.x, P.act, P.alpha); v.y = act_apply(v.y, P.act, P.alpha);
        v.z = act_apply(v.z, P.act, P.alpha); v.w = act_apply(v.w, P.act, P.alpha);
        if (n0 + img < P.N && !(P.dbg & 8))
            *reinterpret_cast<float4*>(P.out + (((size_t)(n0 + img) * P.CN + cn0 + ch) * Hout + 2 * u0 + row2) * Wout + 2 * v0 + 4 * cq) = v;
    }
    stamp(14);
}

template <int SCP, int KQ, bool MASKED>
__global__ __launch_bounds__(NTHR) void dg16_kernel(const Dg16Params P) {
    extern __shared__ __attribute__((aligned(16))) float smem[];
    warm_kernarg(P);
    dg16_body<SCP, KQ, MASKED>(P, smem);
}

struct PlanKey {
    int CK, Hin, Win, lTC, lTR, CS, ckc;
    bool operator<(const PlanKey& o) const {
        return std::tie(CK, Hin, Win, lTC, lTR, CS, ckc) < std::tie(o.CK, o.Hin, o.Win, o.lTC, o.lTR, o.CS, o.ckc);
    }
};
std::mutex g_plan_mu;
std::map<std::pair<int, PlanKey>, unsigned*> g_plans;

int ilog2(int v) { int l = 0; while ((1 << l) < v) ++l; return l; }

int plan_cs(int TI, int TR, int TC, int SCP) {
    const int base = TI * (TR + 2) * SCP;
    const int lTC = ilog2(TC), lTR = ilog2(TR);
    for (int pad = 0; pad < 64; pad += 4) {
        const int CS = base + pad;
        bool ok = true;
        {
            int seen[32] = {0};
            for (int l = 0; l < 32 && ok; ++l) {
                const int p = l & 15, kk = l >> 4;
                const int b = p & (TC - 1), a = (p >> lTC) & (TR - 1), img = p >> (lTC + lTR);
                const int addr = kk * CS + (img * (TR + 2) + a) * SCP + b;
                if (seen[addr & 31]++) ok = false;
            }
        }
        if (ok) return CS;
    }
    return base;
}

const unsigned* get_plan(const PlanKey& k, int SCP, int xinstr, int tiles_r, int tiles_c, hipStream_t s) {
    int dev = 0;
    (void)hipGetDevice(&dev);
    std::lock_guard<std::mutex> lk(g_plan_mu);
    auto it = g_plans.find({dev, k});
    if (it != g_plans.end()) return it->second;
    hipStreamCaptureStatus st = hipStreamCaptureStatusNone;
    if (hipStreamIsCapturing(s, &st) != hipSuccess || st != hipStreamCaptureStatusNone) { (void)hipGetLastError(); return nullptr; }
    const int TC = 1 << k.lTC, TR = 1 << k.lTR, TI = 64 >> (k.lTC + k.lTR), SR = TR + 2, upr = SCP / 4;
    const int npos = tiles_r * tiles_c;
    std::vector<unsigned> tab((size_t)npos * XN_MAX * NTHR, OOB);
    for (int tr = 0; tr < tiles_r; ++tr)
        for (int tc = 0; tc < tiles_c; ++tc)
            for (int j = 0; j < XN_MAX; ++j)
                for (int tid = 0; tid < NTHR; ++tid) {
                    const int wave = tid >> 6, lane = tid & 63;
                    const int instr = wave + j * NWAVE;
                    if (instr >= xinstr) continue;
                    const int e = instr * 64 + lane;
                    const int kch = e / (k.CS / 4), rem = e - kch * (k.CS / 4);
                    if (kch >= k.ckc || rem >= TI * SR * upr) continue;
                    const int img = rem / (SR * upr), r = (rem / upr) % SR, u = rem % upr;
                    const int ih = tr * TR - 1 + r, iw = tc * TC - 4 + 4 * u;
                    if (ih < 0 || ih >= k.Hin || iw < 0 || iw + 3 >= k.Win) continue;
                    tab[((size_t)(tr * tiles_c + tc) * XN_MAX + j) * NTHR + tid] =
                        (unsigned)((((size_t)img * k.CK + kch) * k.Hin + ih) * k.Win + iw) * 4u;
                }
    unsigned* d = nullptr;
    if (hipMalloc((void**)&d, tab.size() * sizeof(unsigned)) != hipSuccess) { (void)hipGetLastError(); return nullptr; }
    if (hipMemcpy(d, tab.data(), tab.size() * sizeof(unsigned), hipMemcpyHostToDevice) != hipSuccess) { (void)hipGetLastError(); (void)hipFree(d); return nullptr; }
    g_plans[{dev, k}] = d;
    return d;
}

int launch_dg16(int scp, int kq, const Dg16Params& P, bool masked, dim3 grid, size_t shmem, hipStream_t s, double fl, double ab) {
    static std::atomic<unsigned long long> once{0};
#define DG16_EACH(X) X(12, 4) X(16, 4) X(24, 4) X(12, 2) X(16, 2) X(24, 2)
    if (first_on_device(once)) {
#define DG16_ATTR(SCP, KQ)                                                                                                                             \
        (void)hipFuncSetAttribute(reinterpret_cast<const void*>(dg16_kernel<SCP, KQ, false>), hipFuncAttributeMaxDynamicSharedMemorySize, 160 * 1024); \
        (void)hipFuncSetAttribute(reinterpret_cast<const void*>(dg16_kernel<SCP, KQ, true>), hipFuncAttributeMaxDynamicSharedMemorySize, 160 * 1024);
        DG16_EACH(DG16_ATTR)
#undef DG16_ATTR
    }
#define DG16_CASE(SCP, KQ)                                                                                                                        \
    if (scp == SCP && kq == KQ) {                                                                                                                 \
        if (masked) { GGAN_LAUNCH("dg16_kernel<" #SCP ", " #KQ ", true>", fl, ab, (dg16_kernel<SCP, KQ, true>), grid, dim3(NTHR), shmem, s, P); } \
        else { GGAN_LAUNCH("dg16_kernel<" #SCP ", " #KQ ", false>", fl, ab, (dg16_kernel<SCP, KQ, false>), grid, dim3(NTHR), shmem, s, P); }      \
        return 0;                                                                                                                                 \
    }
    DG16_EACH(DG16_CASE)
#undef DG16_CASE
#undef DG16_EACH
    return 1;
}

}

namespace ggan {

int conv_dgrad_dg16(const ggan_conv_geom& g, const float* gy, GyMask m, const float* w, const float* bias, float* gx, int act,
                    float alpha, int target_wgs, void* ws, size_t ws_bytes, hipStream_t s) {
    if (!env_int("GGAN_DG16", 1)) return 1;
    if (g.k != 5 || g.stride != 2 || g.pad_t != 1 || g.pad_l != 1) return 1;
    if ((g.H & 1) || (g.W & 1) || g.Ho * 2 != g.H || g.Wo * 2 != g.W) return 1;
    const int CK = g.Co, CN = g.Ci, Hin = g.Ho, Win = g.Wo;
    if ((CK & 15) || (CN & 15) || CK < 16) return 1;
    if (Win < 4 || (Win & (Win - 1)) || (Hin & (Hin - 1))) return 1;
    if ((((uintptr_t)gy) | ((uintptr_t)w) | ((uintptr_t)gx) | ((uintptr_t)m.ref)) & 15) return 1;
    if (m.act != GGAN_ACT_NONE && m.act != GGAN_ACT_LRELU && m.act != GGAN_ACT_RELU) return 1;
    const size_t in_bytes = (size_t)g.N * CK * Hin * Win * 4, w_bytes = (size_t)25 * CN * CK * 4;
    if (in_bytes >= 0x7FFFFFF0ull || w_bytes >= 0x7FFFFFF0ull || (size_t)g.N * CN * g.H * g.W * 4 >= 0x7FFFFFF0ull) return 1;
    const int TC = Win < 16 ? Win : 16;
    int TR = 64 / TC; if (TR > Hin) TR = Hin;
    const int TI = 64 / (TR * TC);
    if (TI * TR * TC != 64) return 1;
    const int SCP = TC + 8;
    const int tiles_r = Hin / TR, tiles_c = Win / TC, igroups = cdiv(g.N, TI);
    const int ptiles = igroups * tiles_r * tiles_c;
    if (target_wgs <= 0) target_wgs = kTargetWgs;
    int kq = env_int("GGAN_DG16_KQ", 0);
    if (kq != 2 && kq != 4) kq = ((CN & 31) == 0 && ptiles * (CN / 32) >= target_wgs) ? 2 : 4;
    if (kq == 2 && (CN & 31)) return 1;
    const int wgs = ptiles * (CN / (kq == 2 ? 32 : 16));
    if (wgs * 4 < target_wgs * 3 && !env_int("GGAN_DG16_FORCE", 0)) return 1;
    const int ckc = 4 * kq;
    if (CK % ckc) return 1;

    Dg16Params P;
    memset(&P, 0, sizeof(P));
    P.in = gy; P.w = w; P.bias = bias; P.out = gx;
    const bool masked = m.act != GGAN_ACT_NONE;
    if (masked) { P.in_ref = m.ref; P.in_slope = m.act == GGAN_ACT_LRELU ? m.alpha : 0.f; }
    P.N = g.N; P.CK = CK; P.Hin = Hin; P.Win = Win; P.CN = CN;
    P.lTC = ilog2(TC); P.lTR = ilog2(TR);
    P.CS = plan_cs(TI, TR, TC, SCP);
    P.xinstr = cdiv(ckc * P.CS / 4, 64);
    if (P.xinstr > XN_MAX * NWAVE) return 1;
    P.tiles_r = tiles_r; P.tiles_c = tiles_c;
    P.nchunks = CK / ckc;
    P.ahead = 1;
    P.nstage = masked ? 3 : 2;
    P.in_bytes = (unsigned)in_bytes; P.w_bytes = (unsigned)w_bytes;
    P.act = act; P.alpha = alpha;
    P.dbg = env_int("GGAN_DBG", 0);
    for (int t = 0; t < 28; ++t) {
        P.tapoff[t] = -1;
        if (t < 25) {
            const int c = tap_cls(t), kh = (c >> 1) + 2 * tap_i(t), kw = (c & 1) + 2 * tap_j(t);
            P.tapoff[t] = (kh * 5 + kw) * CN * CK * 4;
        }
    }
    const PlanKey key{CK, Hin, Win, P.lTC, P.lTR, P.CS, ckc};
    P.xtab = get_plan(key, SCP, P.xinstr, tiles_r, tiles_c, s);
    if (!P.xtab) return 1;
    const int nblk = (kq == 4 ? 13 * 2 : 7 * 4);
    const int wreg = (nblk * WBLK + 3) & ~3;
    const size_t stage = (size_t)wreg + (size_t)P.xinstr * 256;
    const size_t red = (size_t)kq * 4 * (kq == 4 ? 16 : 32) * PS;
    const size_t shmem = (P.nstage * stage > red ? P.nstage * stage : red) * sizeof(float);
    if (shmem > 160 * 1024) return 1;
    ws = ws_scratch(ws, ws_bytes);
    if ((P.dbg & 4) && ws && ws_bytes > (64u << 20)) P.stamps = (unsigned long long*)((char*)ws + ws_bytes - (32u << 20));
    const dim3 grid(ptiles, CN / (kq == 2 ? 32 : 16));
    {
        const int gx = (int)grid.x, gy = (int)grid.y;
        P.xcd_p = 0;
        if ((gx * gy) % 8 == 0) {
            double best = (gx % 8 == 0) ? (double)in_bytes + 8.0 * w_bytes : 8.0 * ((double)in_bytes + w_bytes);
            for (int p = 1; p <= 8; p *= 2) {
                if (gx % p || gy % (8 / p)) continue;
                const double cost = 8.0 * in_bytes / p + (double)w_bytes * p;
                if (cost < 0.9 * best) { best = cost; P.xcd_p = p; }
            }
        }
    }
    const double fl = 2.0 * g.N * g.Co * g.Ho * g.Wo * (double)g.Ci * 25.0;
    const double ab = (double)in_bytes + (double)w_bytes + 4.0 * (double)g.N * CN * g.H * g.W;
    return launch_dg16(SCP, kq, P, masked, grid, shmem, s, fl, ab);
}

}
```

### graphical_gan_amd/csrc/conv_naive.hip

```cpp
#include "common.h"
#include "conv.h"
using namespace ggan;

namespace {

__global__ void conv_fwd_naive_k(ggan_conv_geom g, const float* __restrict__ x, const float* __restrict__ w,
                                 const float* __restrict__ bias, float* __restrict__ y, int act, float alpha) {
    const size_t total = (size_t)g.N * g.Co * g.Ho * g.Wo;
    for (size_t idx = (size_t)blockIdx.x * blockDim.x + threadIdx.x; idx < total; idx += (size_t)gridDim.x * blockDim.x) {
        int ow = idx % g.Wo;
        size_t t = idx / g.Wo;
        int oh = t % g.Ho; t /= g.Ho;
        int co = t % g.Co;
        int n = t / g.Co;
        float acc = 0.f;
        for (int ci = 0; ci < g.Ci; ++ci) {
            const float* xp = x + ((size_t)n * g.Ci + ci) * g.H * g.W;
            for (int kh = 0; kh < g.k; ++kh) {
                int ih = oh * g.stride + kh - g.pad_t;
                if (ih < 0 || ih >= g.H) continue;
                for (int kw = 0; kw < g.k; ++kw) {
                    int iw = ow * g.stride + kw - g.pad_l;
                    if (iw < 0 || iw >= g.W) continue;
                    acc = fmaf(xp[ih * g.W + iw], w[(((size_t)kh * g.k + kw) * g.Ci + ci) * g.Co + co], acc);
                }
            }
        }
        if (bias) acc += bias[co];
        y[idx] = act_apply(acc, act, alpha);
    }
}

__global__ void conv_dgrad_naive_k(ggan_conv_geom g, const float* __restrict__ gy, GyMask mk, const float* __restrict__ w,
                                   const float* __restrict__ bias, float* __restrict__ gx, int act, float alpha) {
    const size_t total = (size_t)g.N * g.Ci * g.H * g.W;
    for (size_t idx = (size_t)blockIdx.x * blockDim.x + threadIdx.x; idx < total; idx += (size_t)gridDim.x * blockDim.x) {
        int iw = idx % g.W;
        size_t t = idx / g.W;
        int ih = t % g.H; t /= g.H;
        int ci = t % g.Ci;
        int n = t / g.Ci;
        float acc = 0.f;
        for (int kh = 0; kh < g.k; ++kh) {
            int th = ih + g.pad_t - kh;
            if (th < 0 || th % g.stride) continue;
            int oh = th / g.stride;
            if (oh >= g.Ho) continue;
            for (int kw = 0; kw < g.k; ++kw) {
                int tw = iw + g.pad_l - kw;
                if (tw < 0 || tw % g.stride) continue;
                int ow = tw / g.stride;
                if (ow >= g.Wo) continue;
                const float* wp = w + (((size_t)kh * g.k + kw) * g.Ci + ci) * g.Co;
                const size_t gb = (size_t)n * g.Co * g.Ho * g.Wo + (size_t)oh * g.Wo + ow;
                for (int co = 0; co < g.Co; ++co) {
                    const size_t gi = gb + (size_t)co * g.Ho * g.Wo;
                    float gv = gy[gi];
                    if (mk.act) gv = act_grad(gv, mk.ref[gi], mk.act, mk.alpha);
                    acc = fmaf(gv, wp[co], acc);
                }
            }
        }
        if (bias) acc += bias[ci];
        gx[idx] = act_apply(acc, act, alpha);
    }
}

__global__ void conv_wgrad_naive_k(ggan_conv_geom g, const float* __restrict__ x, const float* __restrict__ gy, GyMask mk,
                                   float* __restrict__ gw) {
    const size_t total = (size_t)g.k * g.k * g.Ci * g.Co;
    for (size_t idx = (size_t)blockIdx.x * blockDim.x + threadIdx.x; idx < total; idx += (size_t)gridDim.x * blockDim.x) {
        int co = idx % g.Co;
        size_t t = idx / g.Co;
        int ci = t % g.Ci; t /= g.Ci;
        int kw = t % g.k;
        int kh = t / g.k;
        float acc = 0.f;
        for (int n = 0; n < g.N; ++n) {
            const float* xp = x + ((size_t)n * g.Ci + ci) * g.H * g.W;
            const size_t gb = ((size_t)n * g.Co + co) * g.Ho * g.Wo;
            for (int oh = 0; oh < g.Ho; ++oh) {
                int ih = oh * g.stride + kh - g.pad_t;
                if (ih < 0 || ih >= g.H) continue;
                for (int ow = 0; ow < g.Wo; ++ow) {
                    int iw = ow * g.stride + kw - g.pad_l;
                    if (iw < 0 || iw >= g.W) continue;
                    float gv = gy[gb + oh * g.Wo + ow];
                    if (mk.act) gv = act_grad(gv, mk.ref[gb + oh * g.Wo + ow], mk.act, mk.alpha);
                    acc = fmaf(xp[ih * g.W + iw], gv, acc);
                }
            }
        }
        gw[idx] = acc;
    }
}

inline int grid_for(size_t n) {
    size_t b = (n + 255) / 256;
    if (b > 65535) b = 65535;
    if (b < 1) b = 1;
    return (int)b;
}

}

namespace ggan {

int conv_fwd_naive(const ggan_conv_geom& g, const float* x, const float* w, const float* bias, float* y, int act,
                   float alpha, hipStream_t s) {
    size_t total = (size_t)g.N * g.Co * g.Ho * g.Wo;
    double fl = 2.0 * total * g.Ci * g.k * g.k;
    GGAN_LAUNCH("conv_fwd_naive", fl, 0, conv_fwd_naive_k, dim3(grid_for(total)), dim3(256), 0, s, g, x, w, bias, y, act, alpha);
    return 0;
}

int conv_dgrad_naive(const ggan_conv_geom& g, const float* gy, GyMask m, const float* w, const float* bias, float* gx,
                     int act, float alpha, hipStream_t s) {
    size_t total = (size_t)g.N * g.Ci * g.H * g.W;
    double fl = 2.0 * g.N * g.Co * g.Ho * g.Wo * (double)g.Ci * g.k * g.k;
    GGAN_LAUNCH("conv_dgrad_naive", fl, 0, conv_dgrad_naive_k, dim3(grid_for(total)), dim3(256), 0, s, g, gy, m, w, bias, gx, act, alpha);
    return 0;
}

int conv_wgrad_naive(const ggan_conv_geom& g, const float* x, const float* gy, GyMask m, float* gw, hipStream_t s) {
    size_t total = (size_t)g.k * g.k * g.Ci * g.Co;
    double fl = 2.0 * g.N * g.Co * g.Ho * g.Wo * (double)g.Ci * g.k * g.k;
    GGAN_LAUNCH("conv_wgrad_naive", fl, 0, conv_wgrad_naive_k, dim3(grid_for(total)), dim3(256), 0, s, g, x, gy, m, gw);
    return 0;
}

}
```

### graphical_gan_amd/functional/conv.py

```python
import ctypes as C
import os
import torch
from torch.autograd import Function
from .._lib import ACT_NONE, ACT_LRELU, ACT_RELU, check
from ._core import (
    _L, _p, _stream, _c, _DEFER, _DATA_ONLY, _is_param, _skip_undefined, _wgrad_parts, workspace, _remembers_plan, _geom, _new_out)
from .pointwise import ActBwd


DEBUG_POISON_CHECK = bool(os.environ.get('GGAN_POISON_UNWRITTEN'))


class PendingCast(object):

    def __init__(self, x_int, noise, div, mul, slot, ring):
        self.x_int, self.noise, self.div, self.mul, self.ring = x_int, noise, float(div), float(mul), ring
        self.out = _new_out(slot, x_int.shape, x_int.device)
        self.done = False
        self.shape = tuple(x_int.shape)

    def reshape(self, *shape):
        shape = tuple(shape[0]) if len(shape) == 1 and isinstance(shape[0], (tuple, list)) else tuple(shape)
        n = self.out.numel()
        known = 1
        for d in shape:
            known *= d if d != -1 else 1
        self.shape = tuple((n // known) if d == -1 else d for d in shape)
        return self

    def materialize(self):
        if not self.done:
            rt, ca, cb, off = self.ring
            nz = _p(_c(self.noise)) if self.noise is not None else _p(None)
            check(_L().ggan_cast_scale_ring_i32(_p(rt), rt.shape[0], _p(ca), _p(cb), int(off), nz, _p(self.out), self.out.numel(), self.div,
                                                self.mul, _stream()), 'ggan_cast_scale_ring_i32')
            self.done = True
        return self.out


@_remembers_plan
@_skip_undefined
class ConvFwd(Function):

    @staticmethod
    def forward(ctx, x, w, bias, geom, act, alpha, grad_rows=None):
        N, Ci, H, W, Co, Ho, Wo = geom[:7]
        pend = x if isinstance(x, PendingCast) else None
        if pend is not None:
            x = pend.out.view(N, Ci, H, W)
            if pend.done:
                pend = None
        x, w = _c(x), _c(w)
        assert tuple(x.shape) == (N, Ci, H, W) and tuple(w.shape) == (geom[7], geom[7], Ci, Co), (x.shape, w.shape, geom)
        ctx.grad_rows = int(grad_rows) if grad_rows else None
        y = torch.empty((N, Co, Ho, Wo), dtype=torch.float32, device=x.device)
        ws = workspace(x.device)
        g = _geom(geom)
        bp = _p(_c(bias)) if bias is not None else _p(None)
        if pend is not None:
            rt, ca, cb, off = pend.ring
            nz = _p(_c(pend.noise)) if pend.noise is not None else _p(None)
            rc = _L().ggan_conv2d_fwd_cast_ring(C.byref(g), _p(rt), rt.shape[0], _p(ca), _p(cb), int(off), nz, pend.div, pend.mul,
                                                _p(x), _p(w), bp, _p(y), act, alpha, _stream())
            if rc == 1:
                pend.materialize()
                pend = None
            else:
                check(rc, 'ggan_conv2d_fwd_cast_ring')
                pend.done = True
        if pend is None:
            check(_L().ggan_conv2d_fwd(C.byref(g), _p(x), _p(w), bp, _p(y), act, alpha, _p(ws), ws.numel(), _stream()), 'ggan_conv2d_fwd')
        ctx.geom, ctx.act, ctx.alpha, ctx.has_bias = geom, act, alpha, bias is not None
        ctx.w_param, ctx.b_param = _is_param(w), _is_param(bias)
        ctx.save_for_backward(x, w, y if act != ACT_NONE else None)
        return y

    @staticmethod
    def backward(ctx, gy):
        x, w, y = ctx.saved_tensors
        if not torch.is_grad_enabled():
            r = _fused_conv_backward(ctx, gy, x, w, y)
            if r is not None:
                return r + (None,)
        want_w = ctx.needs_input_grad[1] and not (_DATA_ONLY[0] and ctx.w_param)
        want_b = ctx.has_bias and ctx.needs_input_grad[2] and not (_DATA_ONLY[0] and ctx.b_param)
        if (ctx.act in (ACT_LRELU, ACT_RELU) and torch.is_grad_enabled() and ctx.needs_input_grad[0] and not want_w and not want_b
                and not ctx.grad_rows):
            return ConvDgradMasked.apply(gy, y, w, ctx.geom, ctx.act, ctx.alpha), None, None, None, None, None, None
        if ctx.act != ACT_NONE:
            gy = ActBwd.apply(gy, y, ctx.act, ctx.alpha)
        gx = gw = gb = None
        if ctx.needs_input_grad[1] and not (_DATA_ONLY[0] and ctx.w_param):
            gw = ConvWgrad.apply(x, gy, ctx.geom)
        if ctx.has_bias and ctx.needs_input_grad[2] and not (_DATA_ONLY[0] and ctx.b_param):
            gb = ChanSum.apply(gy)
        if ctx.needs_input_grad[0]:
            gx = ConvDgrad.apply(gy, w, None, ctx.geom, ACT_NONE, 0.0)
        return gx, gw, gb, None, None, None, None


def _fused_conv_backward(ctx, gy, x, w, y):
    gy = _c(gy)
    geom = ctx.geom
    N, Ci, H, W, Co, Ho, Wo, k = geom[:8]
    g = _geom(geom)
    L = _L()
    ws = workspace(gy.device)
    act = ctx.act
    yref = _p(y) if act != ACT_NONE else _p(None)
    gx = gw = gb = None
    if ctx.needs_input_grad[1] or (ctx.has_bias and ctx.needs_input_grad[2]):
        want_b = ctx.has_bias and ctx.needs_input_grad[2]
        parts = _wgrad_parts(x, gy, y, act, ctx.alpha, geom, want_b)
        if parts is not None:
            gw, gb = parts
        else:
            gw = torch.empty((k, k, Ci, Co), dtype=torch.float32, device=gy.device)
            gb = torch.empty((Co,), dtype=torch.float32, device=gy.device) if want_b else None
            rc = L.ggan_conv2d_bwd_filter_act(C.byref(g), _p(x), _p(gy), yref, act, ctx.alpha, _p(gw), _p(gb), _p(ws), ws.numel(),
                                              _stream())
            if rc == 1:
                return None
            check(rc, 'ggan_conv2d_bwd_filter_act')
        if not ctx.needs_input_grad[1]:
            gw = None
    if ctx.needs_input_grad[0]:
        gx = torch.empty((N, Ci, H, W), dtype=torch.float32, device=gy.device)
        if ctx.grad_rows and ctx.grad_rows < N and gw is None and gb is None:
            g = _geom((ctx.grad_rows,) + tuple(geom[1:]))
            if DEBUG_POISON_CHECK:
                gx[ctx.grad_rows:].fill_(float('nan'))
        check(L.ggan_conv2d_bwd_data_act(C.byref(g), _p(gy), yref, act, ctx.alpha, _p(w), _p(gx), _p(ws), ws.numel(), _stream()),
              'ggan_conv2d_bwd_data_act')
    return gx, gw, gb, None, None, None


@_remembers_plan
@_skip_undefined
class ConvDgrad(Function):

    @staticmethod
    def forward(ctx, gy, w, bias, geom, act, alpha, slot=None):
        gy, w = _c(gy), _c(w)
        N, Ci, H, W, Co, Ho, Wo = geom[:7]
        assert tuple(gy.shape) == (N, Co, Ho, Wo) and tuple(w.shape) == (geom[7], geom[7], Ci, Co), (gy.shape, w.shape, geom)
        gx = _new_out(slot, (N, Ci, H, W), gy.device)
        ws = workspace(gy.device)
        g = _geom(geom)
        check(_L().ggan_conv2d_bwd_data(C.byref(g), _p(gy), _p(w), _p(_c(bias)) if bias is not None else _p(None),
                                        _p(gx), act, alpha, _p(ws), ws.numel(), _stream()), 'ggan_conv2d_bwd_data')
        ctx.geom, ctx.act, ctx.alpha, ctx.has_bias = geom, act, alpha, bias is not None
        ctx.save_for_backward(gy, w, gx if act != ACT_NONE else None)
        return gx

    @staticmethod
    def backward(ctx, h):
        gy, w, out = ctx.saved_tensors
        d_gy = d_w = d_b = None
        reg = _DEFER[0]
        if ctx.act != ACT_NONE and ctx.has_bias and ctx.needs_input_grad[2] and reg is not None and not torch.is_grad_enabled():
            h = _c(h)
            N, Cc = h.shape[0], h.shape[1]
            HW = h.numel() // (N * Cc)
            cap = min(64, max(1, -(-512 // Cc))) * Cc
            part = torch.empty((cap,), dtype=torch.float32, device=h.device)
            hm = torch.empty_like(h)
            n = C.c_int(0)
            check(_L().ggan_act_bwd_chansum(_p(h), _p(out), _p(hm), _p(part), cap, C.byref(n), N, Cc, HW, ctx.act, ctx.alpha, _stream()),
                  'ggan_act_bwd_chansum')
            h = hm
            d_b = part[:Cc]
            if n.value > 1:
                reg[d_b.data_ptr()] = (n.value, Cc, part)
        elif ctx.act != ACT_NONE:
            h = ActBwd.apply(h, out, ctx.act, ctx.alpha)
        if ctx.needs_input_grad[1]:
            parts = _wgrad_parts(_c(h), gy, None, ACT_NONE, 0.0, ctx.geom, False) if not torch.is_grad_enabled() else None
            d_w = parts[0] if parts is not None else ConvWgrad.apply(h, gy, ctx.geom)
        if ctx.has_bias and ctx.needs_input_grad[2] and d_b is None:
            pre = getattr(h, '_ggan_chansum', None) if not torch.is_grad_enabled() else None
            d_b = pre if (pre is not None and pre.numel() == h.shape[1]) else ChanSum.apply(h)
        if ctx.needs_input_grad[0]:
            d_gy = ConvFwd.apply(h, w, None, ctx.geom, ACT_NONE, 0.0)
        return (d_gy, d_w, d_b) + (None,) * (len(ctx.needs_input_grad) - 3)


@_remembers_plan
@_skip_undefined
class ConvDgradMasked(Function):

    @staticmethod
    def forward(ctx, gy, yref, w, geom, act, alpha):
        gy, yref, w = _c(gy), _c(yref), _c(w)
        N, Ci, H, W, Co, Ho, Wo = geom[:7]
        assert tuple(gy.shape) == (N, Co, Ho, Wo) == tuple(yref.shape), (gy.shape, yref.shape, geom)
        gx = torch.empty((N, Ci, H, W), dtype=torch.float32, device=gy.device)
        ws = workspace(gy.device)
        g = _geom(geom)
        check(_L().ggan_conv2d_bwd_data_act(C.byref(g), _p(gy), _p(yref), act, alpha, _p(w), _p(gx), _p(ws), ws.numel(), _stream()),
              'ggan_conv2d_bwd_data_act')
        ctx.geom, ctx.act, ctx.alpha = geom, act, alpha
        ctx.w_param = _is_param(w)
        ctx.save_for_backward(gy, yref, w)
        return gx

    @staticmethod
    def backward(ctx, h):
        gy, yref, w = ctx.saved_tensors
        geom = ctx.geom
        d_gy = d_w = None
        if torch.is_grad_enabled():
            gm = ActBwd.apply(gy, yref, ctx.act, ctx.alpha)
            if ctx.needs_input_grad[0]:
                d_gy = ActBwd.apply(ConvFwd.apply(h, w, None, geom, ACT_NONE, 0.0), yref, ctx.act, ctx.alpha)
            if ctx.needs_input_grad[2] and not (_DATA_ONLY[0] and ctx.w_param):
                d_w = ConvWgrad.apply(h, gm, geom)
            return d_gy, None, d_w, None, None, None
        h = _c(h)
        N, Ci, H, W, Co, Ho, Wo, k = geom[:8]
        g = _geom(geom)
        L, ws = _L(), workspace(h.device)
        if ctx.needs_input_grad[0]:
            d_gy = torch.empty((N, Co, Ho, Wo), dtype=torch.float32, device=h.device)
            rc = L.ggan_conv2d_fwd_masked(C.byref(g), _p(h), _p(w), _p(d_gy), _p(yref), ctx.act, ctx.alpha, _p(ws), ws.numel(), _stream())
            if rc == 1:
                check(L.ggan_conv2d_fwd(C.byref(g), _p(h), _p(w), _p(None), _p(d_gy), ACT_NONE, 0.0, _p(ws), ws.numel(), _stream()),
                      'ggan_conv2d_fwd')
                d_gy = ActBwd.apply(d_gy, yref, ctx.act, ctx.alpha)
            else:
                check(rc, 'ggan_conv2d_fwd_masked')
        if ctx.needs_input_grad[2] and not (_DATA_ONLY[0] and ctx.w_param):
            parts = _wgrad_parts(h, gy, yref, ctx.act, ctx.alpha, geom, False)
            if parts is not None:
                d_w = parts[0]
            else:
                d_w = torch.empty((k, k, Ci, Co), dtype=torch.float32, device=h.device)
                rc = L.ggan_conv2d_bwd_filter_act(C.byref(g), _p(h), _p(gy), _p(yref), ctx.act, ctx.alpha, _p(d_w), _p(None), _p(ws),
                                                  ws.numel(), _stream())
                if rc == 1:
                    d_w = ConvWgrad.apply(h, ActBwd.apply(gy, yref, ctx.act, ctx.alpha), geom)
                else:
                    check(rc, 'ggan_conv2d_bwd_filter_act')
        return d_gy, None, d_w, None, None, None


@_remembers_plan
@_skip_undefined
class ConvWgrad(Function):

    @staticmethod
    def forward(ctx, x, gy, geom):
        x, gy = _c(x), _c(gy)
        N, Ci, H, W, Co, Ho, Wo, k = geom[:8]
        assert tuple(x.shape) == (N, Ci, H, W) and tuple(gy.shape) == (N, Co, Ho, Wo), (x.shape, gy.shape, geom)
        gw = torch.empty((k, k, Ci, Co), dtype=torch.float32, device=x.device)
        ws = workspace(x.device)
        g = _geom(geom)
        check(_L().ggan_conv2d_bwd_filter(C.byref(g), _p(x), _p(gy), _p(gw), _p(None), _p(ws), ws.numel(), _stream()),
              'ggan_conv2d_bwd_filter')
        ctx.geom = geom
        ctx.save_for_backward(x, gy)
        return gw

    @staticmethod
    def backward(ctx, h):
        x, gy = ctx.saved_tensors
        d_x = d_gy = None
        if ctx.needs_input_grad[0]:
            d_x = ConvDgrad.apply(gy, h, None, ctx.geom, ACT_NONE, 0.0)
        if ctx.needs_input_grad[1]:
            d_gy = ConvFwd.apply(x, h, None, ctx.geom, ACT_NONE, 0.0)
        return d_x, d_gy, None


@_skip_undefined
class ChanSum(Function):

    @staticmethod
    def forward(ctx, x):
        x = _c(x)
        N, Cc = x.shape[0], x.shape[1]
        HW = x.numel() // (N * Cc)
        out = torch.empty((Cc,), dtype=torch.float32, device=x.device)
        ws = workspace(x.device)
        check(_L().ggan_chansum(_p(x), _p(out), N, Cc, HW, _p(ws), ws.numel(), _stream()), 'ggan_chansum')
        ctx.shape = tuple(x.shape)
        return out

    @staticmethod
    def backward(ctx, g):
        shp = ctx.shape
        return g.view(1, -1, *([1] * (len(shp) - 2))).expand(shp).contiguous()


TALL_ROWS = 8192


@_skip_undefined
class ColSum(Function):

    @staticmethod
    def forward(ctx, x):
        x = _c(x)
        rows, cols = x.shape
        out = torch.empty((cols,), dtype=torch.float32, device=x.device)
        if rows >= TALL_ROWS:
            ws = workspace(x.device)
            check(_L().ggan_colsum_tall(_p(x), _p(out), rows, cols, _p(ws), ws.numel(), _stream()), 'ggan_colsum_tall')
        else:
            check(_L().ggan_colsum(_p(x), _p(out), rows, cols, _stream()), 'ggan_colsum')
        ctx.rows = rows
        return out

    @staticmethod
    def backward(ctx, g):
        return g.view(1, -1).expand(ctx.rows, g.numel()).contiguous()
```

### graphical_gan_amd/models.py

```python
import contextlib
import os
import weakref

import numpy as np
import torch

from . import functional as F
from . import tflib as lib
from .tflib.ops.act import LRELU, RELU, TANH, SIGMOID

NETS_TARGET_WGS = 128
GP_TARGET_WGS = 128


class Config(object):
    def __init__(self, dataset='cifar10', batch_size=64, n_coms=0, mode=None, dim=None, dim_latent=128, bn=None,
                 temp=0.1, fuse=True, lr=None, batch_critic=True, mode_k='CONCRETE'):
        self.dataset, self.B, self.K, self.dim_latent, self.temp, self.fuse = dataset, batch_size, n_coms, dim_latent, temp, fuse
        assert mode_k in ('CONCRETE', 'STRAIGHT_THROUGHT_CONCRETE', 'STRAIGHT_THROUGHT'), mode_k
        self.mode_k = mode_k
        if dataset == 'cifar10':
            self.C, self.S, self.dim, self.nl, self.bn, self.out_act = 3, 32, 64, 3, True, 'tanh'
        elif dataset == 'svhn':
            self.C, self.S, self.dim, self.nl, self.bn, self.out_act = 3, 32, 64, 3, False, 'tanh'
        elif dataset == 'mnist':
            self.C, self.S, self.dim, self.nl, self.bn, self.out_act = 1, 28, 64, 3, True, 'sigmoid'
        elif dataset == 'face':
            self.C, self.S, self.dim, self.nl, self.bn, self.out_act = 3, 64, 32, 4, False, 'tanh'
        else:
            raise ValueError(dataset)
        if dim is not None:
            self.dim = dim
        if bn is not None:
            self.bn = bn
        self.mode = mode or ('local_ep' if n_coms else 'ali')
        assert self.mode in ('ali', 'local_ep', 'wali', 'wali-gp', 'alice', 'alice-z', 'alice-x', 'local_epce', 'vegan',
                             'vegan-wgan-gp', 'vegan-mmd', 'vegan-kl', 'vegan-ikl', 'vegan-jsd')
        self.agg = self.mode in ('vegan-kl', 'vegan-ikl', 'vegan-jsd')
        self.learn_std, self.z_samples = self.agg, 100
        self.latent_critic = self.mode in ('vegan', 'vegan-wgan-gp')
        self.lamb = 1.0
        self.no_critic = self.mode == 'vegan-mmd' or self.agg
        assert not ((self.latent_critic or self.no_critic) and n_coms)
        self.top = self.dim * 2 ** (self.nl - 1)
        self.flat = 16 * self.top
        self.output_dim = self.C * self.S * self.S
        self.critic_iters = 5 if self.mode in ('wali', 'wali-gp', 'vegan', 'vegan-wgan-gp') else 1
        if self.no_critic:
            self.critic_iters = 0
        self.lr = lr if lr is not None else {'wali-gp': 1e-4, 'wali': 5e-5}.get(self.mode, 2e-4)
        self.beta1 = 0.5
        self.batch_critic = batch_critic
        self.critic_deep = dataset == 'mnist' and not n_coms and not self.latent_critic and not self.no_critic
        if self.critic_deep and self.bn:
            self.batch_critic = False


class GraphicalGAN(object):

    def __init__(self, cfg):
        self.cfg = cfg
        self._side = None
        self._early = False
        self._pending_join = None
        self._noise_event = None
        self._gp_stream = None
        self.fork_nets = cfg.mode in ('ali', 'alice', 'alice-z', 'alice-x', 'wali', 'wali-gp', 'local_ep', 'local_epce')
        self.fork_now = False
        self.head_hint = False

    @contextlib.contextmanager
    def single_stream(self):
        saved = (self._pending_join, self._noise_event, self._early, self.fork_now, self.head_hint)
        self.fork_now, self._early, self._pending_join, self.head_hint = False, False, None, False
        try:
            yield
        finally:
            self._pending_join, self._noise_event, self._early, self.fork_now, self.head_hint = saved

    @property
    def single_contribution(self):
        return bool(self.cfg.batch_critic) and self.cfg.mode in ('ali', 'local_ep', 'wali', 'wali-gp')

    def launch_hint(self, which):
        c = self.cfg
        if c.mode == 'wali-gp' and which == 'disc' and c.batch_critic and self.fork_nets and self.fork_now:
            return GP_TARGET_WGS
        return 0

    def cut_tensors(self, nets):
        return [nets.get('q_z_src', nets['q_z'])] if self.cfg.mode in ('ali', 'local_ep', 'wali', 'wali-gp') else None

    def critic_cut(self):
        ref = getattr(self, '_critic_features', None)
        t = ref() if ref is not None else None
        if t is None or not t.requires_grad or self.cfg.mode not in ('ali', 'local_ep', 'wali') or not self.cfg.batch_critic:
            return None
        return t, self.cfg.nl

    def feed_buffers(self, device):
        c, B, feed = self.cfg, self.cfg.B, {}
        if c.dataset == 'mnist':
            feed['x_pair'] = torch.zeros(2 * B, c.output_dim, device=device)
            feed['real_x'] = feed['x_pair'][B:]
        else:
            feed['real_x_int'] = torch.zeros(B, c.output_dim, dtype=torch.int32, device=device)
        if c.dataset == 'face':
            feed['dequant_u'] = torch.zeros(B, c.output_dim, device=device)
        feed['z_pair'] = torch.zeros(2 * B, c.dim_latent, device=device)
        feed['p_z_noise'] = feed['z_pair'][:B] if not c.K else torch.zeros(B, c.dim_latent, device=device)
        if c.K:
            feed['k_pair'] = torch.zeros(2 * B, c.K, device=device)
            feed['k_onehot'] = feed['k_pair'][:B]
            if c.mode_k != 'STRAIGHT_THROUGHT':
                feed['gumbel_u'] = torch.zeros(B, c.K, device=device)
        if c.mode in ('wali-gp', 'vegan-wgan-gp'):
            feed['alpha'] = torch.zeros(B, 1, device=device)
        if c.latent_critic:
            for tag in ('f', 'r') + (('h',) if c.mode == 'vegan-wgan-gp' else ()):
                for i, w in enumerate((c.dim_latent, 1024, 512, 256)):
                    feed['dn_%s%d' % (tag, i)] = torch.zeros(B, w, device=device)
        if c.agg:
            feed['q_eps'] = torch.zeros(B, c.dim_latent, device=device)
            feed['kl_k'] = torch.zeros(c.z_samples, B, device=device)
            feed['kl_eps'] = torch.zeros(c.z_samples, c.dim_latent, device=device)
            feed['kl_zp'] = torch.zeros(c.z_samples, c.dim_latent, device=device)
        return feed

    def sample_noise(self, f):
        c = self.cfg
        if 'rng_state' not in f:
            f['rng_state'] = F.noise_state(f['p_z_noise'].device)
        specs = [(f['p_z_noise'], F.NOISE_NORMAL, 0., 1.)]
        if c.K:
            specs.append((f['k_onehot'], F.NOISE_ONEHOT, 0., 0.))
            if 'gumbel_u' in f:
                specs.append((f['gumbel_u'], F.NOISE_UNIFORM, 0., 1.))
        if 'alpha' in f:
            specs.append((f['alpha'], F.NOISE_UNIFORM, 0., 1.))
        specs += [(f[k], F.NOISE_NORMAL, 0., 1.) for k in sorted(f) if k.startswith('dn_')]
        if c.agg:
            specs += [(f['q_eps'], F.NOISE_NORMAL, 0., 1.), (f['kl_k'], F.NOISE_ONEHOT, 0., 0.), (f['kl_eps'], F.NOISE_NORMAL, 0., 1.),
                      (f['kl_zp'], F.NOISE_NORMAL, 0., 1.)]
        if c.dataset == 'face':
            specs.append((f['dequant_u'], F.NOISE_UNIFORM, 0., 1. / 128))
        F.noise_fill_(f['rng_state'], specs)

    def set_batch(self, feed, batch):
        feed['real_x' if self.cfg.dataset == 'mnist' else 'real_x_int'].copy_(batch, non_blocking=True)

    def synthetic_ring(self, device, n=8, seed=1234):
        c, rng, ring = self.cfg, np.random.default_rng(seed), []
        for _ in range(n):
            if c.dataset == 'mnist':
                b = torch.as_tensor(rng.random((c.B, c.output_dim), dtype=np.float32))
            else:
                b = torch.as_tensor(rng.integers(0, 256, size=(c.B, c.output_dim)).astype(np.int32))
            ring.append(b.to(device))
        return ring


    def _conv(self, name, cin, cout, x, act, grad_rows=None):
        if self.cfg.fuse:
            return lib.ops.conv2d.Conv2D(name, cin, cout, 5, x, stride=2, activation=act, grad_rows=grad_rows)
        return F.ActFwd.apply(lib.ops.conv2d.Conv2D(name, cin, cout, 5, x, stride=2, grad_rows=grad_rows), act, 0.2)

    def _lin(self, name, nin, nout, x, act):
        if self.cfg.fuse:
            return lib.ops.linear.Linear(name, nin, nout, x, activation=act)
        return F.ActFwd.apply(lib.ops.linear.Linear(name, nin, nout, x), act, 0.2)

    def _bn(self, name, axes, x, act):
        if self.cfg.fuse:
            return lib.ops.batchnorm.Batchnorm(name, axes, x, activation=act)
        return F.ActFwd.apply(lib.ops.batchnorm.Batchnorm(name, axes, x), act, 0.2)

    def Generator(self, noise, out_slot=None):
        c = self.cfg
        if c.bn and c.fuse:
            out = lib.ops.linear.LinearBatchnormRows('Generator.Input', c.dim_latent, c.flat, noise, 'Generator.BN1', activation=RELU)
        elif c.bn:
            out = lib.ops.linear.Linear('Generator.Input', c.dim_latent, c.flat, noise)
            out = self._bn('Generator.BN1', [0], out, RELU)
        else:
            out = self._lin('Generator.Input', c.dim_latent, c.flat, noise, RELU)
        slot = out_slot
        out = out.reshape(-1, c.top, 4, 4)
        names = ['2', '3', '4', '5'] if c.nl == 4 else ['2', '3', '5']
        ch = c.top
        for i, nm in enumerate(names):
            last = i == len(names) - 1
            cout = c.C if last else ch // 2
            final_act = TANH if c.out_act == 'tanh' else SIGMOID
            if last:
                if c.fuse:
                    out = lib.ops.deconv2d.Deconv2D('Generator.' + nm, ch, cout, 5, out, activation=final_act, out=slot)
                else:
                    out = F.ActFwd.apply(lib.ops.deconv2d.Deconv2D('Generator.' + nm, ch, cout, 5, out), final_act, 0.0)
            elif c.bn:
                out = lib.ops.deconv2d.Deconv2D('Generator.' + nm, ch, cout, 5, out)
                out = self._bn('Generator.BN' + nm, [0, 2, 3], out, RELU)
            elif c.fuse:
                out = lib.ops.deconv2d.Deconv2D('Generator.' + nm, ch, cout, 5, out, activation=RELU)
            else:
                out = F.relu(lib.ops.deconv2d.Deconv2D('Generator.' + nm, ch, cout, 5, out))
            if c.dataset == 'mnist' and nm == '2':
                out = out[:, :, :7, :7].contiguous()
            ch = cout
        return out.reshape(-1, c.output_dim)

    def Extractor(self, inputs, out_slot=None, eps=None, after_first=None):
        c = self.cfg
        out = inputs.reshape(-1, c.C, c.S, c.S)
        ch = c.C
        for i in range(c.nl):
            cout = c.dim * 2 ** i
            name = 'Extractor.%d' % (i + 1)
            if c.bn and i > 0:
                out = lib.ops.conv2d.Conv2D(name, ch, cout, 5, out, stride=2)
                out = self._bn('Extractor.BN%d' % (i + 1), [0, 2, 3], out, LRELU)
            else:
                out = self._conv(name, ch, cout, out, LRELU)
            if i == 0 and after_first is not None:
                after_first()
            ch = cout
        out = out.reshape(-1, c.flat)
        if eps is not None:
            log_std = lib.ops.linear.Linear('Extractor.Std', c.flat, c.dim_latent, out)
            mean = lib.ops.linear.Linear('Extractor.Output', c.flat, c.dim_latent, out)
            z, std = F.Reparam.apply(mean, log_std, eps)
            return z, mean, std
        return lib.ops.linear.Linear('Extractor.Output', c.flat, c.dim_latent, out, out=out_slot)

    def Discriminator(self, x, z, grad_rows=None, twice=False, before_z=None, z_out=None):
        c = self.cfg
        out = x.reshape(-1, c.C, c.S, c.S)
        ch = c.C
        for i in range(c.nl):
            cout = c.dim * 2 ** i
            name = 'Discriminator.%d' % (i + 1)
            if c.critic_deep and c.bn and i > 0:
                out = lib.ops.conv2d.Conv2D(name, ch, cout, 5, out, stride=2, grad_rows=grad_rows)
                out = self._bn('Discriminator.BN%d' % (i + 1), [0, 2, 3], out, LRELU)
            else:
                out = self._conv(name, ch, cout, out, LRELU, grad_rows)
            ch = cout
        out = out.reshape(-1, c.flat)
        self._critic_features = weakref.ref(out)
        if before_z is not None:
            before_z()
        if z_out is None:
            z_out = self._lin('Discriminator.z1', c.dim_latent, 512, z, LRELU)
        if c.critic_deep:
            z_out = self._lin('Discriminator.2', 512, 512, z_out, LRELU)
            out = self._lin('Discriminator.zx1', c.flat + 512, 512, (out, z_out), LRELU)
            if c.fuse:
                return lib.ops.linear.LinearLReLULinear('Discriminator.zx2', 512, 512, 'Discriminator.Output', out, differentiable=twice)
            out = self._lin('Discriminator.zx2', 512, 512, out, LRELU)
            return lib.ops.linear.Linear('Discriminator.Output', 512, 1, out).reshape(-1)
        if c.fuse:
            return lib.ops.linear.LinearLReLULinear('Discriminator.zx1', c.flat + 512, 512, 'Discriminator.Output', (out, z_out),
                                                    differentiable=twice)
        out = self._lin('Discriminator.zx1', c.flat + 512, 512, (out, z_out), LRELU)
        out = lib.ops.linear.Linear('Discriminator.Output', 512, 1, out)
        return out.reshape(-1)

    def LatentDiscriminator(self, z, noise):
        c = self.cfg
        out = F.Axpby.apply(z, noise[0], 1.0, 0.3, 0.0)
        for i, (nm, nin, nout) in enumerate([('Input', c.dim_latent, 1024), ('2', 1024, 512), ('3', 512, 256), ('4', 256, 256)]):
            if c.bn:
                out = lib.ops.linear.Linear('Discriminator.' + nm, nin, nout, out)
                out = self._bn('Discriminator.BN%d' % (i + 1), [0], out, LRELU)
            else:
                out = self._lin('Discriminator.' + nm, nin, nout, out, LRELU)
            if i < 3:
                out = F.Axpby.apply(out, noise[i + 1], 1.0, 0.5, 0.0)
        return lib.ops.linear.Linear('Discriminator.Output', 256, 1, out).reshape(-1)

    def _forward_latent(self, feed, which, out):
        c = self.cfg
        real_x, q_z, p_z = out['real_x'], out['q_z'], out['p_z']
        J = lib.objs.gan_inference
        J.ONLY[0] = which
        noise = lambda tag: [feed['dn_%s%d' % (tag, i)] for i in range(4)]
        det = (lambda t: t.detach()) if which == 'disc' else (lambda t: t)
        with (lib.frozen('Discriminator') if which == 'gen' else lib.frozen()):
            d_real = self.LatentDiscriminator(p_z, noise('r'))
            d_fake = self.LatentDiscriminator(det(q_z), noise('f'))
            gp = None
            if c.mode == 'vegan-wgan-gp' and which != 'gen':
                z_hat = F.RowLerp.apply(p_z, det(q_z), feed['alpha'])
                if not z_hat.requires_grad:
                    z_hat.requires_grad_(True)
                d_hat = self.LatentDiscriminator(z_hat, noise('h'))
                with F.data_grad_only():
                    (g,) = torch.autograd.grad(d_hat, [z_hat], grad_outputs=F.cached_const(1.0, d_hat.shape, d_hat.device), create_graph=True)
                gp = F.GradPenalty.apply(g, 10.0)
        rec = 1. * lib.utils.distance.distance(real_x, self.Generator(q_z), 'l2') if which != 'disc' else None
        gen_params, disc_params = self._var_lists()
        if c.mode == 'vegan':
            res = J.vegan(d_fake, d_real, rec, gen_params, disc_params, c.lamb, lr=c.lr, beta1=c.beta1)
        else:
            res = J.vegan_wgan_gp(d_fake, d_real, rec, gp, gen_params, disc_params, c.lamb, lr=c.lr, beta1=c.beta1)
        J.ONLY[0] = None
        out.update(disc_fake=d_fake, disc_real=d_real, rec_penalty=rec, gradient_penalty=gp, gen_cost=res[0], disc_cost=res[1],
                   gen_train_op=res[2], disc_train_op=res[3])
        return out

    def HyperDiscriminator(self, z, k):
        c = self.cfg
        out = self._lin('Discriminator.HyperInput', c.dim_latent + c.K, 512, (z, k), LRELU)
        out = self._lin('Discriminator.Hyper2', 512, 512, out, LRELU)
        if c.fuse:
            return lib.ops.linear.LinearLReLULinear('Discriminator.Hyper3', 512, 512, 'Discriminator.HyperOutput', out)
        out = self._lin('Discriminator.Hyper3', 512, 512, out, LRELU)
        out = lib.ops.linear.Linear('Discriminator.HyperOutput', 512, 1, out)
        return out.reshape(-1)

    def _mu(self, use=None):
        c = self.cfg
        fan = getattr(self, '_mu_fan', None)
        if fan is not None and use is not None:
            return fan[use]
        return lib.param('Generator.Hyper.Mu', np.random.normal(size=(c.K, c.dim_latent)).astype('float32'))

    def HyperGenerator(self, hyper_k, hyper_noise, out_slot=None):
        mu = self._mu(0)
        if self.cfg.fuse and F.MixMean.usable(hyper_k, mu, hyper_noise):
            return F.MixMean.apply(hyper_k, mu, hyper_noise, out_slot)
        return F.Axpby.apply(F.Gemm.apply(hyper_k, mu, None, False, False, F.ACT_NONE, 0.0), hyper_noise, 1.0, 1.0, 0.0, out_slot)

    def HyperExtractor(self, latent_z, gumbel_u, out_slot=None):
        c = self.cfg
        log_pi = float(np.log(np.float32(1.0) / np.float32(c.K)))
        if c.mode_k == 'CONCRETE':
            return F.GmmLatent.apply(latent_z, self._mu(1), gumbel_u, log_pi, c.temp, out_slot)
        return F.GmmLatentST.apply(latent_z, self._mu(1), gumbel_u, log_pi, c.temp, c.mode_k, out_slot)

    @staticmethod
    def _var_lists():
        return (lib.params_with_name('Generator') + lib.params_with_name('Extractor'),
                lib.params_with_name('Discriminator'))

    def real_x(self, feed, out_slot=None, defer=False):
        c = self.cfg
        if c.dataset == 'mnist':
            return feed['real_x']
        ring = feed.get('ring')
        defer = defer and c.fuse
        if c.dataset == 'face':
            return lib.ops.act.cast_scale(feed['real_x_int'], 256., 2., noise=feed['dequant_u'], out=out_slot, ring=ring, defer=defer)
        return lib.ops.act.cast_scale(feed['real_x_int'], 255., 2., out=out_slot, ring=ring, defer=defer)

    def begin_nets(self, feed):
        c = self.cfg
        self._early = False
        if not (self.fork_nets and self.fork_now) or c.agg or c.dataset == 'mnist':
            return
        dev = feed['p_z_noise'].device
        if dev.type != 'cuda' or not (c.batch_critic and 'z_pair' in feed):
            return
        if self._side is None:
            self._side = F.shared_stream(dev, 'side')
        self._side.wait_stream(torch.cuda.current_stream(dev))
        self._early = True

    def join_side(self, x_only=False):
        pj = self._pending_join
        if pj is None:
            return
        cur, ev_x, ev_end = pj
        if x_only:
            if ev_x is not None:
                cur.wait_event(ev_x)
                pj[1] = None
            return
        cur.wait_event(ev_end)
        self._pending_join = None

    def forward_nets(self, feed):
        c, B = self.cfg, self.cfg.B
        xs = zs = [None, None]
        if c.batch_critic and 'z_pair' in feed:
            xp = feed['x_pair'] if 'x_pair' in feed else torch.empty((2 * B, c.output_dim), dtype=torch.float32,
                                                                     device=feed['z_pair'].device)
            xs = [F.RowSlot(xp, 0, B), F.RowSlot(xp, B, 2 * B)]
            zs = [F.RowSlot(feed['z_pair'], 0, B), F.RowSlot(feed['z_pair'], B, 2 * B)]
        self._mu_fan = F.fanout(self._mu(), 2) if (c.K and c.fuse) else None
        try:
            return self._forward_nets_k(feed, c, B, xs, zs)
        finally:
            self._mu_fan = None

    def _forward_nets_k(self, feed, c, B, xs, zs):
        p_z = self.HyperGenerator(feed['k_onehot'], feed['p_z_noise'], zs[0]) if c.K else feed['p_z_noise']
        fork = self.fork_nets and self.fork_now and p_z.is_cuda
        if fork:
# ... 216 lines not shown
```

### graphical_gan_amd/tflib/ops/conv2d.py

```python
import numpy as np

from ... import functional as F
from .. import param as _param
from .. import tap as _tap
from .. import initial_values_needed as _draw

_default_weightnorm = False


def enable_default_weightnorm():
    global _default_weightnorm
    _default_weightnorm = True


_weights_stdev = None


def set_weights_stdev(weights_stdev):
    global _weights_stdev
    _weights_stdev = weights_stdev


def unset_weights_stdev():
    global _weights_stdev
    _weights_stdev = None


def _uniform(stdev, size):
    return np.random.uniform(low=-stdev * np.sqrt(3), high=stdev * np.sqrt(3), size=size).astype('float32')


def _mask(mask_type, filter_size, input_dim, output_dim):
    mask_type, mask_n_channels = mask_type
    mask = np.ones((filter_size, filter_size, input_dim, output_dim), dtype='float32')
    center = filter_size // 2
    mask[center + 1:, :, :, :] = 0.
    mask[center, center + 1:, :, :] = 0.
    for i in range(mask_n_channels):
        for j in range(mask_n_channels):
            if (mask_type == 'a' and i >= j) or (mask_type == 'b' and i > j):
                mask[center, center, i::mask_n_channels, j::mask_n_channels] = 0.
    return mask


def Conv2D(name, input_dim, output_dim, filter_size, inputs, he_init=True, mask_type=None, stride=1, weightnorm=None,
           biases=True, gain=1., padding='SAME', activation=None, alpha=0.2, grad_rows=None):
    fan_in = input_dim * filter_size ** 2
    fan_out = output_dim * filter_size ** 2 / (stride ** 2)
    if mask_type is not None:
        fan_in /= 2.
        fan_out /= 2.
    filters_stdev = np.sqrt(4. / (fan_in + fan_out)) if he_init else np.sqrt(2. / (fan_in + fan_out))
    shape = (filter_size, filter_size, input_dim, output_dim)
    if _draw(name + '.Filters'):
        filter_values = _uniform(_weights_stdev if _weights_stdev is not None else filters_stdev, shape)
        filter_values *= gain
    else:
        filter_values = None
    filters = _param(name + '.Filters', filter_values)
    if weightnorm is None:
        weightnorm = _default_weightnorm
    if weightnorm:
        norm_values = np.sqrt(np.sum(np.square(filter_values), axis=(0, 1, 2))) if filter_values is not None else None
        target_norms = _param(name + '.g', norm_values)
        norms = (filters * filters).sum(dim=(0, 1, 2)).sqrt()
        filters = filters * (target_norms / norms)
    if mask_type is not None:
        import torch
        filters = filters * torch.as_tensor(_mask(mask_type, filter_size, input_dim, output_dim), device=filters.device)
    b = _param(name + '.Biases', np.zeros(output_dim, dtype='float32')) if biases else None
    N, C, H, W = inputs.shape
    assert C == input_dim, (name, inputs.shape, input_dim)
    geom = F.conv_geom(N, input_dim, H, W, output_dim, filter_size, stride, padding)
    act = F.ACT_NONE if activation is None else activation
    out = F.ConvFwd.apply(inputs, filters, b, geom, act, float(alpha), grad_rows)
    return _tap(name, out) if act in (F.ACT_LRELU, F.ACT_RELU) else out
```

### include/ggan.h

```cpp
#ifndef GGAN_H
#define GGAN_H
#include <stddef.h>
#include <stdint.h>

#ifdef __cplusplus
extern "C" {
#endif

typedef void* ggan_stream_t;
#define GGAN_WS_RESERVED 16384

enum { GGAN_ACT_NONE = 0, GGAN_ACT_LRELU = 1, GGAN_ACT_RELU = 2, GGAN_ACT_TANH = 3, GGAN_ACT_SIGMOID = 4 };

#define GGAN_ABI_VERSION 800
int ggan_version(void);
const char* ggan_last_error(void);
typedef struct {
    int N, Ci, H, W;
    int Co, Ho, Wo;
    int k, stride, pad_t, pad_l;
    int plan_wgs, plan_wgs_filter, plan_flags;
} ggan_conv_geom;
#define GGAN_PLAN_PLAIN 1

size_t ggan_conv2d_workspace(const ggan_conv_geom* g);
int ggan_conv2d_fwd(const ggan_conv_geom* g, const float* x, const float* w, const float* bias,
                    float* y, int act, float alpha, void* ws, size_t ws_bytes, ggan_stream_t stream);
int ggan_conv2d_bwd_data(const ggan_conv_geom* g, const float* gy, const float* w, const float* bias,
                         float* gx, int act, float alpha, void* ws, size_t ws_bytes, ggan_stream_t stream);
int ggan_conv2d_bwd_filter(const ggan_conv_geom* g, const float* x, const float* gy, float* gw,
                           float* gbias, void* ws, size_t ws_bytes, ggan_stream_t stream);
int ggan_conv2d_bwd_data_act(const ggan_conv_geom* g, const float* gy, const float* y, int y_act, float y_alpha,
                             const float* w, float* gx, void* ws, size_t ws_bytes, ggan_stream_t stream);
int ggan_conv2d_bwd_filter_act(const ggan_conv_geom* g, const float* x, const float* gy, const float* y, int y_act,
                               float y_alpha, float* gw, float* gbias, void* ws, size_t ws_bytes, ggan_stream_t stream);
int ggan_conv2d_bwd_filter_parts(const ggan_conv_geom* g, const float* x, const float* gy, const float* y, int y_act,
                                 float y_alpha, int with_bias, float* part, size_t part_cap, int* n_parts,
                                 size_t* stride, ggan_stream_t stream);

int ggan_deconv2d_fwd(const ggan_conv_geom* g, const float* x_small, const float* w, const float* bias,
                      float* y_big, int act, float alpha, void* ws, size_t ws_bytes, ggan_stream_t stream);
int ggan_deconv2d_bwd_data(const ggan_conv_geom* g, const float* gy_big, const float* w, float* gx_small,
                           void* ws, size_t ws_bytes, ggan_stream_t stream);
int ggan_deconv2d_bwd_filter(const ggan_conv_geom* g, const float* gy_big, const float* x_small, float* gw,
                             float* gbias , void* ws, size_t ws_bytes,
                             ggan_stream_t stream);

int ggan_linear_bwd_data_act(int M, int N, int K, const float* g, const float* y, int y_act, float y_alpha,
                             const float* w, float* dx, void* ws, size_t ws_bytes, ggan_stream_t stream);
int ggan_linear_bwd_weight_act(int M, int N, int K, const float* x, const float* g, const float* y, int y_act,
                               float y_alpha, float* dw, float* db, void* ws, size_t ws_bytes, ggan_stream_t stream);

int ggan_gemm_split(int ta, int tb, int M, int N, int K, const float* A, const float* A2, int a_split, const float* B,
                    const float* bias, float* C, float* C2, int c_split, float* colsum_b, int act, float alpha, void* ws,
                    size_t ws_bytes, ggan_stream_t stream);

int ggan_dyn_scan_fwd(int B, int T, int dl, int dt, int H, const float* z0, const float* eps, const float* w_in, const float* b_in,
                      const float* w_1, const float* b_1, const float* w_out, const float* b_out, const float* zw, const float* b_zw,
                      float alpha, float* zs, float* h1, float* h2, ggan_stream_t stream);
int ggan_dyn_scan_bwd(int B, int T, int dl, int dt, int H, const float* g_zs, const float* zs, const float* eps, const float* h1,
                      const float* h2, const float* w_in, const float* w_1, const float* w_out, const float* zw, float alpha, float* G1,
                      float* G2, float* Go, float* Xin, float* d_z0, float* d_eps, ggan_stream_t stream);

int ggan_critic_head_fwd(int M, int K1, int K2, int H, const float* a1, const float* a2, const float* w, const float* b,
                         const float* w_out, const float* b_out, float alpha, float* h, float* logits, void* ws, size_t ws_bytes,
                         ggan_stream_t stream);
int ggan_critic_head_bwd(int M, int K1, int K2, int H, const float* g, const float* a1, const float* a2, const float* w, const float* h,
                         const float* w_out, float alpha, float* gh, float* d_a1, float* d_a2, float* d_w, float* d_b, float* d_wout,
                         float* d_bout, void* ws, size_t ws_bytes, ggan_stream_t stream);

int ggan_critic_head_fwd_bce(int M, int K1, int K2, int H, const float* a1, const float* a2, const float* w, const float* b,
                             const float* w_out, const float* b_out, float alpha, float* h, float* logits, int kind, int nterms,
                             const int* term_rows, const float* labels, const float* weights, float* g, float* gh, void* ws,
                             size_t ws_bytes, ggan_stream_t stream);
int ggan_critic_head_bwd_tail(int M, int K1, int K2, int H, const float* a1, const float* a2, const float* w, const float* h,
                              const float* w_out, float alpha, const float* gh, float* d_a1, float* d_a2, float* d_w, float* d_b,
                              float* d_wout, float* d_bout, const float* logits, const float* g, int kind, int nterms, const int* term_rows,
                              const float* labels, const float* weights, const float* const* ext, float* loss, void* ws, size_t ws_bytes,
                              ggan_stream_t stream);

size_t ggan_gemm_workspace(int M, int N, int K);
int ggan_gemm(int ta, int tb, int M, int N, int K, const float* A, const float* B, const float* bias,
              float* C, int act, float alpha, void* ws, size_t ws_bytes, ggan_stream_t stream);
int ggan_gemm_colsum(int ta, int M, int N, int K, const float* A, const float* B, float* C, float* colsum_b,
                     void* ws, size_t ws_bytes, ggan_stream_t stream);
int ggan_colsum(const float* x, float* out, int rows, int cols, ggan_stream_t stream);
int ggan_colsum_tall(const float* x, float* out, int rows, int cols, void* ws, size_t ws_bytes, ggan_stream_t stream);
int ggan_chansum(const float* x, float* out, int N, int C, int HW, void* ws, size_t ws_bytes, ggan_stream_t stream);

int ggan_bn_fwd_train(const float* x, const float* scale, const float* offset, float* y,
                      float* save_mean, float* save_invstd, int N, int C, int HW, float eps,
                      int act, float alpha, ggan_stream_t stream);
int ggan_bn_bwd(const float* x, const float* gy, const float* scale, const float* save_mean,
                const float* save_invstd, float* gx, float* gscale, float* goffset,
                int N, int C, int HW, ggan_stream_t stream);
int ggan_bn_bwd_act(const float* x, const float* gy, const float* y, int y_act, float y_alpha, const float* scale,
                    const float* save_mean, const float* save_invstd, float* gx, float* gscale, float* goffset,
                    float* gx_chansum, int N, int C, int HW, ggan_stream_t stream);

int ggan_conv2d_fwd_masked(const ggan_conv_geom* g, const float* x, const float* w, float* y, const float* yref, int ref_act,
                           float ref_alpha, void* ws, size_t ws_bytes, ggan_stream_t stream);

int ggan_linear_bn_rows_fwd(const float* x, const float* w, const float* b, const float* scale, const float* offset, float* h,
                            float* y, float* save_mean, float* save_invstd, int M, int K, int N, float eps, int act,
                            float alpha, ggan_stream_t stream);
int ggan_linear_bn_rows_bwd(const float* x, const float* gy, const float* h, const float* y, const float* scale, const float* save_mean,
                            const float* save_invstd, float* dw, float* db, float* dscale, float* doffset, int M, int K, int N, int act,
                            float alpha, ggan_stream_t stream);

int ggan_bn_bwd_bwd(const float* x, const float* gy, const float* y, int y_act, float y_alpha, const float* h, const float* scale,
                    const float* save_mean, const float* save_invstd, float* ggy, float* gx2, float* gscale2, int N, int C, int HW,
                    ggan_stream_t stream);

int ggan_bn_split_fwd_train(const float* x, const float* scale, const float* offset, float* y, float* save_mean, float* save_invstd,
                            int N, int C, int HW, int groups, float eps, int act, float alpha, void* ws, size_t ws_bytes,
                            ggan_stream_t stream);
int ggan_bn_split_bwd_act(const float* x, const float* gy, int act, float alpha, const float* scale, const float* offset,
                          const float* save_mean, const float* save_invstd, float* gx, float* gscale, float* goffset,
                          float* gx_chansum, int N, int C, int HW, int groups, int gx_groups, void* ws, size_t ws_bytes,
                          ggan_stream_t stream);

int ggan_bn_sync_stats(const float* x, float* stats, int N, int C, int HW, ggan_stream_t stream);
int ggan_bn_sync_apply(const float* x, const float* stats, int world, const float* scale, const float* offset, float* y,
                       float* save_mean, float* save_invstd, int N, int C, int HW, float eps, int act, float alpha,
                       ggan_stream_t stream);
int ggan_bn_sync_bwd_stats(const float* x, const float* gy, const float* y, int y_act, float y_alpha, const float* save_mean,
                           const float* save_invstd, float* sums, int N, int C, int HW, ggan_stream_t stream);
int ggan_bn_sync_bwd_apply(const float* x, const float* gy, const float* y, int y_act, float y_alpha, const float* scale,
                           const float* save_mean, const float* save_invstd, const float* sums, int world, int rank, float* gx,
                           float* gscale, float* goffset, int N, int C, int HW, ggan_stream_t stream);

int ggan_act_fwd(const float* x, float* y, size_t n, int act, float alpha, ggan_stream_t stream);
int ggan_act_bwd(const float* gy, const float* ref, float* gx, size_t n, int act, float alpha,
                 ggan_stream_t stream);
int ggan_act_bwd_chansum(const float* gy, const float* ref, float* gx, float* parts, int parts_cap, int* n_parts, int N, int C, int HW,
                         int act, float alpha, ggan_stream_t stream);
int ggan_bias_add(const float* x, const float* bias, float* y, int N, int C, int HW, ggan_stream_t stream);
int ggan_cast_scale_i32(const int32_t* x, const float* noise , float* y, size_t n,
                        float div, float mul, ggan_stream_t stream);
int ggan_cast_scale_ring_i32(const int32_t* ring, int nslots, const int32_t* ctr_a, const int32_t* ctr_b, int offset,
                             const float* noise , float* y, size_t n, float div, float mul, ggan_stream_t stream);
int ggan_conv2d_fwd_cast_ring(const ggan_conv_geom* g, const int32_t* ring, int nslots, const int32_t* ctr_a, const int32_t* ctr_b, int offset,
                              const float* noise , float div, float mul, float* x_out, const float* w,
                              const float* bias , float* y, int act, float alpha, ggan_stream_t stream);
int ggan_mix_mean(const float* k, const float* mu, const float* noise, float* out, int B, int K, int D, ggan_stream_t stream);
int ggan_axpby(const float* x, const float* y, float* out, size_t n, float a, float b, float c,
               ggan_stream_t stream);
int ggan_row_lerp(const float* x, const float* y, const float* alpha, float* out, int rows, int cols,
                  ggan_stream_t stream);

int ggan_bce_logits_fwd(const float* x, float label, float weight, float* loss, int n, int accumulate,
                        ggan_stream_t stream);
int ggan_bce_logits_bwd(const float* x, float label, float weight, const float* gloss, float* gx, int n,
                        ggan_stream_t stream);
#define GGAN_BCE_MAX 16
int ggan_bce_logits_multi_fwd(const float* const* xs, const float* labels, const float* weights, const int* ns,
                              int count, float* loss, ggan_stream_t stream);
#define GGAN_HEAD_BCE_MAX_ROWS 2048
int ggan_bce_head_bwd(const float* const* xs, const float* labels, const float* weights, const int* ns, int count, float* loss,
                      float* const* gxs, int M, int H, const float* h, const float* w_out, float alpha, float* gh, float* d_wout,
                      float* d_bout, ggan_stream_t stream);
#define GGAN_BCE_HEADS 2
int ggan_bce_heads_bwd(const float* const* xs, const float* labels, const float* weights, const int* ns, int count, float* loss,
                       float* const* gxs, int nheads, const int* head_terms, const int* Ms, const int* Hs, const float* const* hs,
                       const float* const* w_outs, const float* alphas, float* const* ghs, float* const* d_wouts ,
                       float* const* d_bouts , ggan_stream_t stream);
int ggan_bce_logits_multi_bwd(const float* const* xs, const float* labels, const float* weights, const int* ns,
                              int count, const float* gloss, float* const* gxs, ggan_stream_t stream);
int ggan_bce_logits_multi_fwd_grad(const float* const* xs, const float* labels, const float* weights, const int* ns,
                                   int count, float* loss, float* const* gxs, ggan_stream_t stream);
int ggan_mean_fwd(const float* x, float weight, float* loss, int n, int accumulate, ggan_stream_t stream);
int ggan_mean_bwd(const float* gloss, float weight, float* gx, int n, ggan_stream_t stream);
int ggan_mean_multi_fwd_grad(const float* const* xs, const float* weights, const int* ns, int count, float* loss,
                             float* const* gxs , ggan_stream_t stream);

int ggan_conv3d_out_shape(const int* dims10, int* lo_ho_wo);
int ggan_im2col3d(const int* dims10, const float* x, float* col, ggan_stream_t stream);
int ggan_col2im3d(const int* dims10, const float* col, float* gx, ggan_stream_t stream);
int ggan_conv3d_igemm_ok(const int* dims10, int kind);
int ggan_conv3d_fwd(const int* dims10, const float* x, const float* w, const float* bias , float* y, int act,
                    float alpha, void* ws, size_t ws_bytes, ggan_stream_t stream);
int ggan_conv3d_wgrad(const int* dims10, const float* x, const float* gy, float* gw, void* ws, size_t ws_bytes,
                      ggan_stream_t stream);
int ggan_conv3d_dgrad(const int* dims10, const float* gy, const float* w, float* gx, ggan_stream_t stream);

int ggan_mix_rbf_mmd2_fwd(const float* X, const float* Y, int m, int n, int d, const float* sigmas, const float* wts, int ns,
// ... 109 lines not shown
```

Measured before the change: 17370 images/sec.

## Fuse previous layer's activation-gradient mask into conv dgrad epilogue

Adds a bwd_data_act_out entry point that applies the input-producing layer's LReLU/ReLU derivative mask inside the dgrad kernels' store epilogue (dg16, mfma corr, naive). The resulting gradient is tagged as premasked, so the downstream conv backward and wgrad skip re-applying the mask. This removes a separate read-modify pass over the activation gradient for each discriminator conv layer. It adds bookkeeping for premasked tensors, an extra reference read in the epilogue, and fallback paths when the geometry or alignment is unsupported.

```diff
diff --git a/graphical_gan_amd/_lib.py b/graphical_gan_amd/_lib.py
--- a/graphical_gan_amd/_lib.py
+++ b/graphical_gan_amd/_lib.py
@@ -48,6 +48,7 @@
     'ggan_conv2d_bwd_data': (_I, [_G, _P, _P, _P, _P, _I, _F, _P, _Z, _P]),
     'ggan_conv2d_bwd_filter': (_I, [_G, _P, _P, _P, _P, _P, _Z, _P]),
     'ggan_conv2d_bwd_data_act': (_I, [_G, _P, _P, _I, _F, _P, _P, _P, _Z, _P]),
+    'ggan_conv2d_bwd_data_act_out': (_I, [_G, _P, _P, _I, _F, _P, _P, _P, _I, _F, _P, _Z, _P]),
     'ggan_conv2d_bwd_filter_act': (_I, [_G, _P, _P, _P, _I, _F, _P, _P, _P, _Z, _P]),
     'ggan_conv2d_bwd_filter_parts': (_I, [_G, _P, _P, _P, _I, _F, _I, _P, _Z, C.POINTER(_I), C.POINTER(_Z), _P]),
     'ggan_conv2d_fwd_cast_ring': (_I, [_G, _P, _I, _P, _P, _I, _P, _F, _F, _P, _P, _P, _P, _I, _F, _P]),
diff --git a/graphical_gan_amd/csrc/conv.h b/graphical_gan_amd/csrc/conv.h
--- a/graphical_gan_amd/csrc/conv.h
+++ b/graphical_gan_amd/csrc/conv.h
@@ -10,8 +10,9 @@
     int act;
     float alpha;
 };
+struct OutMask;
 int conv_dgrad_naive(const ggan_conv_geom& g, const float* gy, GyMask m, const float* w, const float* bias, float* gx,
-                     int act, float alpha, hipStream_t s);
+                     int act, float alpha, hipStream_t s, OutMask* om = nullptr);
 int conv_wgrad_naive(const ggan_conv_geom& g, const float* x, const float* gy, GyMask m, float* gw, hipStream_t s);
 
 constexpr int kTargetWgs = 200;
@@ -24,9 +25,9 @@
 int conv_fwd_mfma(const ggan_conv_geom& g, const float* x, const float* w, const float* bias, float* y, int act,
                   float alpha, void* ws, size_t ws_bytes, hipStream_t s, OutMask* mask = nullptr);
 int conv_dgrad_mfma(const ggan_conv_geom& g, const float* gy, GyMask m, const float* w, const float* bias, float* gx,
-                    int act, float alpha, void* ws, size_t ws_bytes, hipStream_t s);
+                    int act, float alpha, void* ws, size_t ws_bytes, hipStream_t s, OutMask* om = nullptr);
 int conv_dgrad_dg16(const ggan_conv_geom& g, const float* gy, GyMask m, const float* w, const float* bias, float* gx, int act,
-                    float alpha, int target_wgs, void* ws, size_t ws_bytes, hipStream_t s);
+                    float alpha, int target_wgs, void* ws, size_t ws_bytes, hipStream_t s, OutMask* om = nullptr);
 int conv_dgrad_thin(const ggan_conv_geom& g, const float* gy, GyMask m, const float* w, const float* bias, float* gx, int act,
                     float alpha, hipStream_t s);
 struct WgradParts {
diff --git a/graphical_gan_amd/csrc/conv_api.hip b/graphical_gan_amd/csrc/conv_api.hip
--- a/graphical_gan_amd/csrc/conv_api.hip
+++ b/graphical_gan_amd/csrc/conv_api.hip
@@ -57,22 +57,27 @@
 }
 
 static int bwd_data(const ggan_conv_geom* g, const float* gy, GyMask m, const float* w, const float* bias, float* gx, int act,
-                    float alpha, void* ws, size_t ws_bytes, ggan_stream_t stream) {
+                    float alpha, void* ws, size_t ws_bytes, ggan_stream_t stream, OutMask* om = nullptr) {
     if (check_geom(g)) return -1;
     if (!(gy && w && gx)) { set_error("ggan_conv2d_bwd_data: null pointer"); return -1; }
+    if (om) {
+        if (om->act != GGAN_ACT_LRELU && om->act != GGAN_ACT_RELU) { set_error("ggan_conv2d_bwd_data_act_out: output mask must be lrelu or relu"); return -1; }
+        if (g->Ci <= 4 && !(g->plan_flags & GGAN_PLAN_PLAIN)) return 1;
+    }
     hipStream_t s = (hipStream_t)stream;
     if (getenv("GGAN_TRACE_CONV"))
         fprintf(stderr, "[ggan] bwd_data N=%d Ci=%d H=%d W=%d Co=%d Ho=%d Wo=%d pad=(%d,%d) mask=%d act=%d\n", g->N, g->Ci, g->H, g->W, g->Co, g->Ho,
                 g->Wo, g->pad_t, g->pad_l, m.act, act);
     if (!(g->plan_flags & GGAN_PLAN_PLAIN) && !getenv("GGAN_NAIVE_DGRAD")) {
-        int r = conv_dgrad_thin(*g, gy, m, w, bias, gx, act, alpha, s);
-        if (r <= 0) return r;
-        r = conv_dgrad_dg16(*g, gy, m, w, bias, gx, act, alpha, g->plan_wgs, ws, ws ? ws_bytes : 0, s);
-        if (r <= 0) return r;
-        r = conv_dgrad_mfma(*g, gy, m, w, bias, gx, act, alpha, ws, ws ? ws_bytes : 0, s);
-        if (r <= 0) return r;
-    }
-    return conv_dgrad_naive(*g, gy, m, w, bias, gx, act, alpha, s);
+        int r = om ? 1 : conv_dgrad_thin(*g, gy, m, w, bias, gx, act, alpha, s);
+        if (r <= 0) return r;
+        r = conv_dgrad_dg16(*g, gy, m, w, bias, gx, act, alpha, g->plan_wgs, ws, ws ? ws_bytes : 0, s, om);
+        if (r <= 0) return r;
+        r = conv_dgrad_mfma(*g, gy, m, w, bias, gx, act, alpha, ws, ws ? ws_bytes : 0, s, om);
+        if (r <= 0) return r;
+        if (om && g->k == 5 && g->stride == 2) return 1;
+    }
+    return conv_dgrad_naive(*g, gy, m, w, bias, gx, act, alpha, s, om);
 }
 
 __global__ void pad_width_k(const float* __restrict__ in, const float* __restrict__ ref, float* __restrict__ out, size_t rows,
@@ -162,6 +167,17 @@
     return bwd_data(g, gy, GyMask{y, y_act, y_alpha}, w, nullptr, gx, GGAN_ACT_NONE, 0.f, ws, ws_bytes, stream);
 }
 
+int ggan_conv2d_bwd_data_act_out(const ggan_conv_geom* g, const float* gy, const float* y, int y_act, float y_alpha, const float* w,
+                                 float* gx, const float* out_ref, int out_act, float out_alpha, void* ws, size_t ws_bytes,
+                                 ggan_stream_t stream) {
+    GGAN_CHECK_ARG(y || y_act == GGAN_ACT_NONE, "null activation reference");
+    GGAN_CHECK_ARG(out_ref, "null output reference");
+    OutMask om{out_ref, out_act, out_alpha, false};
+    const int rc = bwd_data(g, gy, GyMask{y, y_act, y_alpha}, w, nullptr, gx, GGAN_ACT_NONE, 0.f, ws, ws_bytes, stream, &om);
+    if (rc == 0 && !om.applied) { set_error("conv2d_bwd_data_act_out: launch without the mask"); return -3; }
+    return rc;
+}
+
 int ggan_conv2d_bwd_filter_act(const ggan_conv_geom* g, const float* x, const float* gy, const float* y, int y_act, float y_alpha,
                                float* gw, float* gbias, void* ws, size_t ws_bytes, ggan_stream_t stream) {
     GGAN_CHECK_ARG(y || y_act == GGAN_ACT_NONE, "null activation reference");
diff --git a/graphical_gan_amd/csrc/conv_corr.hip b/graphical_gan_amd/csrc/conv_corr.hip
--- a/graphical_gan_amd/csrc/conv_corr.hip
+++ b/graphical_gan_amd/csrc/conv_corr.hip
@@ -667,6 +667,8 @@
     constexpr int GROUPS = NC == 4 ? 2 : NC;
     constexpr int UNITS = GROUPS * TNW * (TMW / 4);
     const bool quad_rows = (P.TC & 3) == 0;
+    const float oslope = P.out_act == GGAN_ACT_LRELU ? P.out_alpha : 0.f;
+    auto omask = [&](float v, float r) { return KIND == 0 ? act_grad(v, r, P.out_act, P.out_alpha) : (r > 0.f ? v : v * oslope); };
     for (int u = tid; u < UNITS; u += NTHR) {
         const int p4 = u % (TMW / 4);
         const int cnl = (u / (TMW / 4)) % TNW;
@@ -709,10 +711,9 @@
             if (NC != 4 && P.ocs == 1 && (A.Wv & 3) == 0 && (u0 + ur) < A.Hu && (v0 + vc + 3) < A.Wv) {
                 const int off = (A.or0 + P.ors * (u0 + ur)) * P.Wout + A.oc0 + v0 + vc;
                 if ((off & 3) == 0) {
-                    if (KIND == 0 && P.out_ref) {
+                    if (P.out_ref) {
                         const float4 r4 = *reinterpret_cast<const float4*>(P.out_ref + cbase + off);
-                        va[0] = act_grad(va[0], r4.x, P.out_act, P.out_alpha); va[1] = act_grad(va[1], r4.y, P.out_act, P.out_alpha);
-                        va[2] = act_grad(va[2], r4.z, P.out_act, P.out_alpha); va[3] = act_grad(va[3], r4.w, P.out_act, P.out_alpha);
+                        va[0] = omask(va[0], r4.x); va[1] = omask(va[1], r4.y); va[2] = omask(va[2], r4.z); va[3] = omask(va[3], r4.w);
                     }
                     *reinterpret_cast<float4*>(outp + cbase + off) = make_float4(va[0], va[1], va[2], va[3]);
                     done = true;
@@ -724,8 +725,15 @@
                 if ((off & 3) == 0 && P.ocs == 2) {
                     const float* e = a_even ? va : vb;
                     const float* o = a_even ? vb : va;
-                    *reinterpret_cast<float4*>(outp + cbase + off) = make_float4(e[0], o[0], e[1], o[1]);
-                    *reinterpret_cast<float4*>(outp + cbase + off + 4) = make_float4(e[2], o[2], e[3], o[3]);
+                    float4 s0 = make_float4(e[0], o[0], e[1], o[1]), s1 = make_float4(e[2], o[2], e[3], o[3]);
+                    if (P.out_ref) {
+                        const float4 r0 = *reinterpret_cast<const float4*>(P.out_ref + cbase + off);
+                        const float4 r1 = *reinterpret_cast<const float4*>(P.out_ref + cbase + off + 4);
+                        s0 = make_float4(omask(s0.x, r0.x), omask(s0.y, r0.y), omask(s0.z, r0.z), omask(s0.w, r0.w));
+                        s1 = make_float4(omask(s1.x, r1.x), omask(s1.y, r1.y), omask(s1.z, r1.z), omask(s1.w, r1.w));
+                    }
+                    *reinterpret_cast<float4*>(outp + cbase + off) = s0;
+                    *reinterpret_cast<float4*>(outp + cbase + off + 4) = s1;
                     done = true;
                 }
             }
@@ -742,10 +750,12 @@
                 const size_t cb2 = ((size_t)(n0 + im) * P.CNtot + cn) * chw;
                 if ((u0 + urj) < A.Hu && (v0 + vcj) < A.Wv) {
                     const size_t oi = cb2 + (A.or0 + P.ors * (u0 + urj)) * P.Wout + A.oc0 + P.ocs * (v0 + vcj);
-                    outp[oi] = (KIND == 0 && P.out_ref) ? act_grad(va[j], P.out_ref[oi], P.out_act, P.out_alpha) : va[j];
+                    outp[oi] = P.out_ref ? omask(va[j], P.out_ref[oi]) : va[j];
                 }
-                if (NC == 4 && (u0 + urj) < B.Hu && (v0 + vcj) < B.Wv)
-                    outp[cb2 + (B.or0 + P.ors * (u0 + urj)) * P.Wout + B.oc0 + P.ocs * (v0 + vcj)] = vb[j];
+                if (NC == 4 && (u0 + urj) < B.Hu && (v0 + vcj) < B.Wv) {
+                    const size_t oi = cb2 + (B.or0 + P.ors * (u0 + urj)) * P.Wout + B.oc0 + P.ocs * (v0 + vcj);
+                    outp[oi] = P.out_ref ? omask(vb[j], P.out_ref[oi]) : vb[j];
+                }
             }
         }
     }
@@ -1017,7 +1027,8 @@
     P.out = P.SK > 1 ? (float*)ws : dst;
     P.bias = bias; P.act = act; P.alpha = alpha;
     if (mask) {
-        if (MODE != 0 || P.SK != 1) return 1;
+        if (P.SK != 1) return 1;
+        if (MODE != 0 && (bias || act != GGAN_ACT_NONE || (mask->act != GGAN_ACT_LRELU && mask->act != GGAN_ACT_RELU))) return 1;
         P.out_ref = mask->ref; P.out_act = mask->act; P.out_alpha = mask->alpha;
         mask->applied = true;
     }
@@ -1107,8 +1118,9 @@
 }
 
 int conv_dgrad_mfma(const ggan_conv_geom& g, const float* gy, GyMask m, const float* w, const float* bias, float* gx,
-                    int act, float alpha, void* ws, size_t ws_bytes, hipStream_t s) {
+                    int act, float alpha, void* ws, size_t ws_bytes, hipStream_t s, OutMask* om) {
     if (!hot_geometry(g)) return 1;
+    if (om && (!om->ref || (((uintptr_t)om->ref) & 15))) return 1;
     ws = ws_scratch(ws, ws_bytes);
     if ((g.Co & 3) || ((uintptr_t)w & 15)) return 1;
     const size_t in_bytes = (size_t)g.N * g.Co * g.Ho * g.Wo * 4, w_bytes = (size_t)25 * g.Ci * g.Co * 4;
@@ -1155,9 +1167,9 @@
     const long wgs_all = (long)cdiv(g.N * Hu * Wv, 32) * cdiv(g.Ci, 32);
     if (wgs_all >= (g.plan_wgs > 0 ? g.plan_wgs : kTargetWgs))
         return plan_and_launch<2>(P, Hu, Wv, 1, hi[0] - lo[0] + 1, hi[1] - lo[1] + 1, 25, 1, gx, bias, act, alpha, ws, ws_bytes,
-                                  s, "conv_dgrad_mfma", fl, "GGAN_DGRAD_SK");
+                                  s, "conv_dgrad_mfma", fl, "GGAN_DGRAD_SK", om);
     return plan_and_launch<1>(P, Hu, Wv, 1, hi[0] - lo[0] + 1, hi[1] - lo[1] + 1, 13, 2, gx, bias, act, alpha, ws, ws_bytes,
-                              s, "conv_dgrad_mfma", fl, "GGAN_DGRAD_SK");
-}
-
-}
+                              s, "conv_dgrad_mfma", fl, "GGAN_DGRAD_SK", om);
+}
+
+}
diff --git a/graphical_gan_amd/csrc/conv_dg16.hip b/graphical_gan_amd/csrc/conv_dg16.hip
--- a/graphical_gan_amd/csrc/conv_dg16.hip
+++ b/graphical_gan_amd/csrc/conv_dg16.hip
@@ -22,6 +22,7 @@
     const float* bias;
     float* out;
     const float* in_ref;
+    const float* out_ref;
     const unsigned* xtab;
     int N, CK, Hin, Win, CN;
     int lTC, lTR;
@@ -36,6 +37,8 @@
     int act;
     float alpha;
     float in_slope;
+    int out_act;
+    float out_alpha;
     int dbg;
     unsigned long long* stamps;
     int tapoff[28];
@@ -293,6 +296,10 @@
         const int img = u >> (lQ + lTR + 1 + (NCHT == 1 ? 4 : 5));
         const int ph = 1 - (row2 & 1), arow = row2 >> 1;
         const int px = (img << (lTC + lTR)) + (arow << lTC) + 2 * cq;
+        const bool live = n0 + img < P.N;
+        const size_t oi = (((size_t)(n0 + img) * P.CN + cn0 + ch) * Hout + 2 * u0 + row2) * Wout + 2 * v0 + 4 * cq;
+        float4 rf = make_float4(1.f, 1.f, 1.f, 1.f);
+        if (P.out_ref && live) rf = *reinterpret_cast<const float4*>(P.out_ref + oi);
         float2 e = make_float2(0.f, 0.f), o = make_float2(0.f, 0.f);
         float2 te[KQ], to[KQ];
 #pragma unroll
@@ -306,8 +313,12 @@
         float4 v = make_float4(e.x + bv, o.x + bv, e.y + bv, o.y + bv);
         v.x = act_apply(v.x, P.act, P.alpha); v.y = act_apply(v.y, P.act, P.alpha);
         v.z = act_apply(v.z, P.act, P.alpha); v.w = act_apply(v.w, P.act, P.alpha);
-        if (n0 + img < P.N && !(P.dbg & 8))
-            *reinterpret_cast<float4*>(P.out + (((size_t)(n0 + img) * P.CN + cn0 + ch) * Hout + 2 * u0 + row2) * Wout + 2 * v0 + 4 * cq) = v;
+        if (P.out_ref) {
+            const float os = P.out_act == GGAN_ACT_LRELU ? P.out_alpha : 0.f;
+            v.x = rf.x > 0.f ? v.x : v.x * os; v.y = rf.y > 0.f ? v.y : v.y * os;
+            v.z = rf.z > 0.f ? v.z : v.z * os; v.w = rf.w > 0.f ? v.w : v.w * os;
+        }
+        if (live && !(P.dbg & 8)) *reinterpret_cast<float4*>(P.out + oi) = v;
     }
     stamp(14);
 }
@@ -411,8 +422,11 @@
 namespace ggan {
 
 int conv_dgrad_dg16(const ggan_conv_geom& g, const float* gy, GyMask m, const float* w, const float* bias, float* gx, int act,
-                    float alpha, int target_wgs, void* ws, size_t ws_bytes, hipStream_t s) {
+                    float alpha, int target_wgs, void* ws, size_t ws_bytes, hipStream_t s, OutMask* om) {
     if (!env_int("GGAN_DG16", 1)) return 1;
+    if (om && ((om->act != GGAN_ACT_LRELU && om->act != GGAN_ACT_RELU) || !om->ref || (((uintptr_t)om->ref) & 15) || bias ||
+               act != GGAN_ACT_NONE))
+        return 1;
     if (g.k != 5 || g.stride != 2 || g.pad_t != 1 || g.pad_l != 1) return 1;
     if ((g.H & 1) || (g.W & 1) || g.Ho * 2 != g.H || g.Wo * 2 != g.W) return 1;
     const int CK = g.Co, CN = g.Ci, Hin = g.Ho, Win = g.Wo;
@@ -454,6 +468,7 @@
     P.nstage = masked ? 3 : 2;
     P.in_bytes = (unsigned)in_bytes; P.w_bytes = (unsigned)w_bytes;
     P.act = act; P.alpha = alpha;
+    if (om) { P.out_ref = om->ref; P.out_act = om->act; P.out_alpha = om->alpha; }
     P.dbg = env_int("GGAN_DBG", 0);
     for (int t = 0; t < 28; ++t) {
         P.tapoff[t] = -1;
@@ -469,7 +484,8 @@
     const int wreg = (nblk * WBLK + 3) & ~3;
     const size_t stage = (size_t)wreg + (size_t)P.xinstr * 256;
     const size_t red = (size_t)kq * 4 * (kq == 4 ? 16 : 32) * PS;
-    const size_t shmem = (P.nstage * stage > red ? P.nstage * stage : red) * sizeof(float);
+    const int nfoot = (!masked && m.ref) ? 3 : P.nstage;
+    const size_t shmem = (nfoot * stage > red ? nfoot * stage : red) * sizeof(float);
     if (shmem > 160 * 1024) return 1;
     ws = ws_scratch(ws, ws_bytes);
     if ((P.dbg & 4) && ws && ws_bytes > (64u << 20)) P.stamps = (unsigned long long*)((char*)ws + ws_bytes - (32u << 20));
@@ -488,7 +504,9 @@
     }
     const double fl = 2.0 * g.N * g.Co * g.Ho * g.Wo * (double)g.Ci * 25.0;
     const double ab = (double)in_bytes + (double)w_bytes + 4.0 * (double)g.N * CN * g.H * g.W;
-    return launch_dg16(SCP, kq, P, masked, grid, shmem, s, fl, ab);
-}
-
-}
+    const int rc = launch_dg16(SCP, kq, P, masked, grid, shmem, s, fl, ab);
+    if (rc == 0 && om) om->applied = true;
+    return rc;
+}
+
+}
diff --git a/graphical_gan_amd/csrc/conv_naive.hip b/graphical_gan_amd/csrc/conv_naive.hip
--- a/graphical_gan_amd/csrc/conv_naive.hip
+++ b/graphical_gan_amd/csrc/conv_naive.hip
@@ -32,7 +32,8 @@
 }
 
 __global__ void conv_dgrad_naive_k(ggan_conv_geom g, const float* __restrict__ gy, GyMask mk, const float* __restrict__ w,
-                                   const float* __restrict__ bias, float* __restrict__ gx, int act, float alpha) {
+                                   const float* __restrict__ bias, float* __restrict__ gx, int act, float alpha,
+                                   const float* __restrict__ out_ref, float out_slope) {
     const size_t total = (size_t)g.N * g.Ci * g.H * g.W;
     for (size_t idx = (size_t)blockIdx.x * blockDim.x + threadIdx.x; idx < total; idx += (size_t)gridDim.x * blockDim.x) {
         int iw = idx % g.W;
@@ -62,7 +63,9 @@
             }
         }
         if (bias) acc += bias[ci];
-        gx[idx] = act_apply(acc, act, alpha);
+        acc = act_apply(acc, act, alpha);
+        if (out_ref) acc = out_ref[idx] > 0.f ? acc : acc * out_slope;
+        gx[idx] = acc;
     }
 }
 
@@ -115,10 +118,15 @@
 }
 
 int conv_dgrad_naive(const ggan_conv_geom& g, const float* gy, GyMask m, const float* w, const float* bias, float* gx,
-                     int act, float alpha, hipStream_t s) {
+                     int act, float alpha, hipStream_t s, OutMask* om) {
+    if (om && ((om->act != GGAN_ACT_LRELU && om->act != GGAN_ACT_RELU) || !om->ref || bias || act != GGAN_ACT_NONE)) return 1;
     size_t total = (size_t)g.N * g.Ci * g.H * g.W;
     double fl = 2.0 * g.N * g.Co * g.Ho * g.Wo * (double)g.Ci * g.k * g.k;
-    GGAN_LAUNCH("conv_dgrad_naive", fl, 0, conv_dgrad_naive_k, dim3(grid_for(total)), dim3(256), 0, s, g, gy, m, w, bias, gx, act, alpha);
+    const float* out_ref = om ? om->ref : nullptr;
+    const float out_slope = om && om->act == GGAN_ACT_LRELU ? om->alpha : 0.f;
+    GGAN_LAUNCH("conv_dgrad_naive", fl, 0, conv_dgrad_naive_k, dim3(grid_for(total)), dim3(256), 0, s, g, gy, m, w, bias, gx, act, alpha,
+                out_ref, out_slope);
+    if (om) om->applied = true;
     return 0;
 }
 
diff --git a/graphical_gan_amd/functional/conv.py b/graphical_gan_amd/functional/conv.py
--- a/graphical_gan_amd/functional/conv.py
+++ b/graphical_gan_amd/functional/conv.py
@@ -38,12 +38,30 @@
         return self.out
 
 
+def _premask_on():
+    return not os.environ.get('GGAN_NO_PREMASK')
+
+
+def _premasked_ref(y):
+    return _p(None) if os.environ.get('GGAN_PREMASK_NARROW_LDS') else _p(y)
+
+
+def _mark_premasked(gx, ref, rows, act, alpha):
+    gx._ggan_premask = (ref.data_ptr(), int(rows), int(act), float(alpha))
+
+
+def _is_premasked(gy, y, rows, act, alpha):
+    m = getattr(gy, '_ggan_premask', None)
+    return (m is not None and y is not None and m[0] == y.data_ptr() and m[1] >= int(rows) and m[2] == int(act)
+            and m[3] == float(alpha))
+
+
 @_remembers_plan
 @_skip_undefined
 class ConvFwd(Function):
 
     @staticmethod
-    def forward(ctx, x, w, bias, geom, act, alpha, grad_rows=None):
+    def forward(ctx, x, w, bias, geom, act, alpha, grad_rows=None, in_act=None):
         N, Ci, H, W, Co, Ho, Wo = geom[:7]
         pend = x if isinstance(x, PendingCast) else None
         if pend is not None:
@@ -53,6 +71,7 @@
         x, w = _c(x), _c(w)
         assert tuple(x.shape) == (N, Ci, H, W) and tuple(w.shape) == (geom[7], geom[7], Ci, Co), (x.shape, w.shape, geom)
         ctx.grad_rows = int(grad_rows) if grad_rows else None
+        ctx.in_act = (int(in_act[0]), float(in_act[1])) if (in_act and in_act[0] in (ACT_LRELU, ACT_RELU) and pend is None) else None
         y = torch.empty((N, Co, Ho, Wo), dtype=torch.float32, device=x.device)
         ws = workspace(x.device)
         g = _geom(geom)
@@ -81,13 +100,14 @@
         if not torch.is_grad_enabled():
             r = _fused_conv_backward(ctx, gy, x, w, y)
             if r is not None:
-                return r + (None,)
+                return r + (None, None)
         want_w = ctx.needs_input_grad[1] and not (_DATA_ONLY[0] and ctx.w_param)
         want_b = ctx.has_bias and ctx.needs_input_grad[2] and not (_DATA_ONLY[0] and ctx.b_param)
         if (ctx.act in (ACT_LRELU, ACT_RELU) and torch.is_grad_enabled() and ctx.needs_input_grad[0] and not want_w and not want_b
                 and not ctx.grad_rows):
-            return ConvDgradMasked.apply(gy, y, w, ctx.geom, ctx.act, ctx.alpha), None, None, None, None, None, None
-        if ctx.act != ACT_NONE:
+            xref = x if (ctx.in_act is not None and _premask_on()) else None
+            return (ConvDgradMasked.apply(gy, y, w, ctx.geom, ctx.act, ctx.alpha, xref, ctx.in_act),) + (None,) * 7
+        if ctx.act != ACT_NONE and not _is_premasked(gy, y, ctx.geom[0], ctx.act, ctx.alpha):
             gy = ActBwd.apply(gy, y, ctx.act, ctx.alpha)
         gx = gw = gb = None
         if ctx.needs_input_grad[1] and not (_DATA_ONLY[0] and ctx.w_param):
@@ -96,18 +116,21 @@
             gb = ChanSum.apply(gy)
         if ctx.needs_input_grad[0]:
             gx = ConvDgrad.apply(gy, w, None, ctx.geom, ACT_NONE, 0.0)
-        return gx, gw, gb, None, None, None, None
+        return gx, gw, gb, None, None, None, None, None
 
 
 def _fused_conv_backward(ctx, gy, x, w, y):
-    gy = _c(gy)
     geom = ctx.geom
     N, Ci, H, W, Co, Ho, Wo, k = geom[:8]
+    act = ctx.act
+    if act != ACT_NONE and _is_premasked(gy, y, ctx.grad_rows if (ctx.grad_rows and ctx.grad_rows < N) else N, act, ctx.alpha):
+        act = ACT_NONE
+    gy = _c(gy)
     g = _geom(geom)
     L = _L()
     ws = workspace(gy.device)
-    act = ctx.act
     yref = _p(y) if act != ACT_NONE else _p(None)
+    dref = _premasked_ref(y) if (act == ACT_NONE and ctx.act != ACT_NONE) else yref
     gx = gw = gb = None
     if ctx.needs_input_grad[1] or (ctx.has_bias and ctx.needs_input_grad[2]):
         want_b = ctx.has_bias and ctx.needs_input_grad[2]
@@ -130,8 +153,17 @@
             g = _geom((ctx.grad_rows,) + tuple(geom[1:]))
             if DEBUG_POISON_CHECK:
                 gx[ctx.grad_rows:].fill_(float('nan'))
-        check(L.ggan_conv2d_bwd_data_act(C.byref(g), _p(gy), yref, act, ctx.alpha, _p(w), _p(gx), _p(ws), ws.numel(), _stream()),
-              'ggan_conv2d_bwd_data_act')
+        rc = 1
+        if ctx.in_act is not None and _premask_on():
+            rc = L.ggan_conv2d_bwd_data_act_out(C.byref(g), _p(gy), dref, act, ctx.alpha, _p(w), _p(gx), _p(x), ctx.in_act[0], ctx.in_act[1],
+                                                _p(ws), ws.numel(), _stream())
+            if rc == 0:
+                _mark_premasked(gx, x, g.N, *ctx.in_act)
+            elif rc != 1:
+                check(rc, 'ggan_conv2d_bwd_data_act_out')
+        if rc == 1:
+            check(L.ggan_conv2d_bwd_data_act(C.byref(g), _p(gy), dref, act, ctx.alpha, _p(w), _p(gx), _p(ws), ws.numel(), _stream()),
+                  'ggan_conv2d_bwd_data_act')
     return gx, gw, gb, None, None, None
 
 
@@ -190,15 +222,28 @@
 class ConvDgradMasked(Function):
 
     @staticmethod
-    def forward(ctx, gy, yref, w, geom, act, alpha):
+    def forward(ctx, gy, yref, w, geom, act, alpha, xref=None, x_act=None):
+        pre = _is_premasked(gy, yref, geom[0], act, alpha)
         gy, yref, w = _c(gy), _c(yref), _c(w)
         N, Ci, H, W, Co, Ho, Wo = geom[:7]
         assert tuple(gy.shape) == (N, Co, Ho, Wo) == tuple(yref.shape), (gy.shape, yref.shape, geom)
         gx = torch.empty((N, Ci, H, W), dtype=torch.float32, device=gy.device)
         ws = workspace(gy.device)
         g = _geom(geom)
-        check(_L().ggan_conv2d_bwd_data_act(C.byref(g), _p(gy), _p(yref), act, alpha, _p(w), _p(gx), _p(ws), ws.numel(), _stream()),
-              'ggan_conv2d_bwd_data_act')
+        yp, ya = (_premasked_ref(yref), ACT_NONE) if pre else (_p(yref), act)
+        rc = 1
+        if xref is not None and x_act is not None:
+            xref = _c(xref)
+            rc = _L().ggan_conv2d_bwd_data_act_out(C.byref(g), _p(gy), yp, ya, alpha, _p(w), _p(gx), _p(xref), x_act[0], x_act[1], _p(ws),
+                                                   ws.numel(), _stream())
+            if rc == 0:
+                _mark_premasked(gx, xref, N, *x_act)
+            elif rc != 1:
+                check(rc, 'ggan_conv2d_bwd_data_act_out')
+        if rc == 1:
+            check(_L().ggan_conv2d_bwd_data_act(C.byref(g), _p(gy), yp, ya, alpha, _p(w), _p(gx), _p(ws), ws.numel(), _stream()),
+                  'ggan_conv2d_bwd_data_act')
+        ctx.pre = pre
         ctx.geom, ctx.act, ctx.alpha = geom, act, alpha
         ctx.w_param = _is_param(w)
         ctx.save_for_backward(gy, yref, w)
@@ -209,13 +254,14 @@
         gy, yref, w = ctx.saved_tensors
         geom = ctx.geom
         d_gy = d_w = None
+        n_in = len(ctx.needs_input_grad)
         if torch.is_grad_enabled():
-            gm = ActBwd.apply(gy, yref, ctx.act, ctx.alpha)
+            gm = gy if ctx.pre else ActBwd.apply(gy, yref, ctx.act, ctx.alpha)
             if ctx.needs_input_grad[0]:
                 d_gy = ActBwd.apply(ConvFwd.apply(h, w, None, geom, ACT_NONE, 0.0), yref, ctx.act, ctx.alpha)
             if ctx.needs_input_grad[2] and not (_DATA_ONLY[0] and ctx.w_param):
                 d_w = ConvWgrad.apply(h, gm, geom)
-            return d_gy, None, d_w, None, None, None
+            return (d_gy, None, d_w) + (None,) * (n_in - 3)
         h = _c(h)
         N, Ci, H, W, Co, Ho, Wo, k = geom[:8]
         g = _geom(geom)
@@ -230,18 +276,19 @@
             else:
                 check(rc, 'ggan_conv2d_fwd_masked')
         if ctx.needs_input_grad[2] and not (_DATA_ONLY[0] and ctx.w_param):
-            parts = _wgrad_parts(h, gy, yref, ctx.act, ctx.alpha, geom, False)
+            m_act = ACT_NONE if ctx.pre else ctx.act
+            parts = _wgrad_parts(h, gy, yref, m_act, ctx.alpha, geom, False)
             if parts is not None:
                 d_w = parts[0]
             else:
                 d_w = torch.empty((k, k, Ci, Co), dtype=torch.float32, device=h.device)
-                rc = L.ggan_conv2d_bwd_filter_act(C.byref(g), _p(h), _p(gy), _p(yref), ctx.act, ctx.alpha, _p(d_w), _p(None), _p(ws),
-                                                  ws.numel(), _stream())
+                rc = L.ggan_conv2d_bwd_filter_act(C.byref(g), _p(h), _p(gy), _p(yref) if m_act != ACT_NONE else _p(None), m_act, ctx.alpha,
+                                                  _p(d_w), _p(None), _p(ws), ws.numel(), _stream())
                 if rc == 1:
-                    d_w = ConvWgrad.apply(h, ActBwd.apply(gy, yref, ctx.act, ctx.alpha), geom)
+                    d_w = ConvWgrad.apply(h, gy if ctx.pre else ActBwd.apply(gy, yref, ctx.act, ctx.alpha), geom)
                 else:
                     check(rc, 'ggan_conv2d_bwd_filter_act')
-        return d_gy, None, d_w, None, None, None
+        return (d_gy, None, d_w) + (None,) * (n_in - 3)
 
 
 @_remembers_plan
diff --git a/graphical_gan_amd/models.py b/graphical_gan_amd/models.py
--- a/graphical_gan_amd/models.py
+++ b/graphical_gan_amd/models.py
@@ -160,9 +160,10 @@
         return ring
 
 
-    def _conv(self, name, cin, cout, x, act, grad_rows=None):
+    def _conv(self, name, cin, cout, x, act, grad_rows=None, owns_input=False):
         if self.cfg.fuse:
-            return lib.ops.conv2d.Conv2D(name, cin, cout, 5, x, stride=2, activation=act, grad_rows=grad_rows)
+            return lib.ops.conv2d.Conv2D(name, cin, cout, 5, x, stride=2, activation=act, grad_rows=grad_rows,
+                                         in_act=(act, 0.2) if owns_input else None)
         return F.ActFwd.apply(lib.ops.conv2d.Conv2D(name, cin, cout, 5, x, stride=2, grad_rows=grad_rows), act, 0.2)
 
     def _lin(self, name, nin, nout, x, act):
@@ -243,7 +244,7 @@
                 out = lib.ops.conv2d.Conv2D(name, ch, cout, 5, out, stride=2, grad_rows=grad_rows)
                 out = self._bn('Discriminator.BN%d' % (i + 1), [0, 2, 3], out, LRELU)
             else:
-                out = self._conv(name, ch, cout, out, LRELU, grad_rows)
+                out = self._conv(name, ch, cout, out, LRELU, grad_rows, owns_input=i > 0 and not (c.critic_deep and c.bn))
             ch = cout
         out = out.reshape(-1, c.flat)
         self._critic_features = weakref.ref(out)
diff --git a/graphical_gan_amd/tflib/ops/conv2d.py b/graphical_gan_amd/tflib/ops/conv2d.py
--- a/graphical_gan_amd/tflib/ops/conv2d.py
+++ b/graphical_gan_amd/tflib/ops/conv2d.py
@@ -44,7 +44,7 @@
 
 
 def Conv2D(name, input_dim, output_dim, filter_size, inputs, he_init=True, mask_type=None, stride=1, weightnorm=None,
-           biases=True, gain=1., padding='SAME', activation=None, alpha=0.2, grad_rows=None):
+           biases=True, gain=1., padding='SAME', activation=None, alpha=0.2, grad_rows=None, in_act=None):
     fan_in = input_dim * filter_size ** 2
     fan_out = output_dim * filter_size ** 2 / (stride ** 2)
     if mask_type is not None:
@@ -73,5 +73,5 @@
     assert C == input_dim, (name, inputs.shape, input_dim)
     geom = F.conv_geom(N, input_dim, H, W, output_dim, filter_size, stride, padding)
     act = F.ACT_NONE if activation is None else activation
-    out = F.ConvFwd.apply(inputs, filters, b, geom, act, float(alpha), grad_rows)
+    out = F.ConvFwd.apply(inputs, filters, b, geom, act, float(alpha), grad_rows, in_act)
     return _tap(name, out) if act in (F.ACT_LRELU, F.ACT_RELU) else out
diff --git a/include/ggan.h b/include/ggan.h
--- a/include/ggan.h
+++ b/include/ggan.h
@@ -32,6 +32,9 @@
                            float* gbias, void* ws, size_t ws_bytes, ggan_stream_t stream);
 int ggan_conv2d_bwd_data_act(const ggan_conv_geom* g, const float* gy, const float* y, int y_act, float y_alpha,
                              const float* w, float* gx, void* ws, size_t ws_bytes, ggan_stream_t stream);
+int ggan_conv2d_bwd_data_act_out(const ggan_conv_geom* g, const float* gy, const float* y, int y_act, float y_alpha,
+                                 const float* w, float* gx, const float* out_ref, int out_act, float out_alpha, void* ws,
+                                 size_t ws_bytes, ggan_stream_t stream);
 int ggan_conv2d_bwd_filter_act(const ggan_conv_geom* g, const float* x, const float* gy, const float* y, int y_act,
                                float y_alpha, float* gw, float* gbias, void* ws, size_t ws_bytes, ggan_stream_t stream);
 int ggan_conv2d_bwd_filter_parts(const ggan_conv_geom* g, const float* x, const float* gy, const float* y, int y_act,
```

Measured after the change: 17320 images/sec (median of 2 runs). Within noise of the previous version (-0.3%).
